# CaptainEven/DenseBox

Measured on AMD Instinct MI355X. Metric: training patches/sec (240x240), higher is better.
Workload: dtype f16; 1 GPU; full training step (fwd + fused dense loss w/ hard-negative mining + bwd + grad all-reduce + SGD) of DenseBoxLMLOC on 240x240 patches; net=DenseBoxLMLOC, batch_per_gpu=64, global_batch=64, patch=240x240, parallelism=dp1, half_neg=11, grad_finite=True

## Files before the change

densebox_amd/_lib.py:

```python
import ctypes as C
import os

_HERE = os.path.dirname(os.path.abspath(__file__))
LIB_PATH = os.environ.get('DBX_LIB') or os.path.join(_HERE, 'csrc', 'libdensebox_hip.so')

F16, BF16, F32 = 0, 1, 2
DTYPE_ID = {'f16': F16, 'bf16': BF16, 'f32': F32}
ESIZE = {F16: 2, BF16: 2, F32: 4}

EPI_BIAS, EPI_RELU, EPI_GATE, EPI_DROPMASK, EPI_ACCUM, EPI_F32_NCHW, EPI_DROPHASH = 1, 2, 4, 8, 16, 32, 64
CONV_WFRAG = 128
K_IGEMM, K_DMA, K_BAND, K_C64, K_C8, K_WS, K_P8 = 1, 2, 3, 4, 5, 6, 7


class View(C.Structure):
    _fields_ = [('ptr', C.c_void_p), ('n', C.c_int32), ('h', C.c_int32), ('w', C.c_int32),
                ('pad', C.c_int32), ('ld', C.c_int32), ('c_off', C.c_int32), ('c', C.c_int32)]


class ConvDesc(C.Structure):
    _fields_ = [('dtype', C.c_int32), ('kh', C.c_int32), ('kw', C.c_int32), ('cpad', C.c_int32),
                ('cin_pad', C.c_int32), ('cout_pad', C.c_int32), ('epilogue', C.c_int32), ('drop_seed', C.c_uint32)]


# ... 40 lines not shown


class CropFrame(C.Structure):
    _fields_ = [('src', C.c_void_p), ('sh', C.c_int32), ('sw', C.c_int32)]


class EvalRecord(C.Structure):
    _fields_ = [('score', C.c_double), ('lm_err', C.c_double), ('status', C.c_int32), ('frame', C.c_int32)]


class Track(C.Structure):
    _fields_ = [('box', C.c_double * 4), ('vel', C.c_double * 4), ('score', C.c_double), ('best_score', C.c_double), ('id', C.c_int32),
                ('hits', C.c_int32), ('age', C.c_int32), ('first_frame', C.c_int32), ('last_frame', C.c_int32), ('best_frame', C.c_int32)]


class TrackRecord(C.Structure):
    _fields_ = [('stream', C.c_int32), ('reserved', C.c_int32), ('t', Track)]


class Shot(C.Structure):
    _fields_ = [('key', C.c_double), ('score', C.c_double), ('sharpness', C.c_int64), ('id', C.c_int32), ('frame', C.c_int32),
                ('shots', C.c_int32), ('reserved', C.c_int32)]


class ShotRecord(C.Structure):
    _fields_ = [('stream', C.c_int32), ('slot', C.c_int32), ('shot', Shot)]


class OverlayFrame(C.Structure):
    _fields_ = [('src', C.c_void_p), ('dst', C.c_void_p), ('h', C.c_int32), ('w', C.c_int32)]


class OverlayStyle(C.Structure):
    _fields_ = [('box_color', C.c_uint8 * 4), ('text_color', C.c_uint8 * 4), ('mark_color', C.c_uint8 * 4), ('thickness', C.c_int32),
                ('radius', C.c_int32), ('font_scale', C.c_int32), ('inset_scale', C.c_int32)]


class RedactStyle(C.Structure):
    _fields_ = [('color', C.c_uint8 * 4), ('method', C.c_int32), ('shape', C.c_int32), ('cell', C.c_int32), ('radius', C.c_int32),
                ('grow', C.c_int32), ('grow_pct', C.c_int32), ('coast', C.c_int32), ('min_score', C.c_double)]


class ResizeJob(C.Structure):
    _fields_ = [('src', C.c_void_p), ('sh', C.c_int32), ('sw', C.c_int32), ('cx0', C.c_int32), ('cy0', C.c_int32),
                ('cw', C.c_int32), ('ch', C.c_int32), ('pad_l', C.c_int32), ('pad_t', C.c_int32), ('pad_r', C.c_int32),
                ('pad_b', C.c_int32), ('pad_value', C.c_int32), ('dh', C.c_int32), ('dw', C.c_int32), ('dst_off', C.c_int64)]


class Nv12Frame(C.Structure):
    _fields_ = [('y', C.c_void_p), ('uv', C.c_void_p), ('rgb', C.c_void_p), ('h', C.c_int32), ('w', C.c_int32), ('pitch_y', C.c_int32),
                ('pitch_uv', C.c_int32), ('pitch_rgb', C.c_int32), ('reserved', C.c_int32)]


class Nv12Params(C.Structure):
    _fields_ = [('standard', C.c_int32), ('range', C.c_int32), ('order', C.c_int32), ('reserved', C.c_int32)]


class ResizeJobNv12(C.Structure):
    _fields_ = [('y', C.c_void_p), ('uv', C.c_void_p), ('pitch_y', C.c_int32), ('pitch_uv', C.c_int32), ('sh', C.c_int32),
                ('sw', C.c_int32), ('cx0', C.c_int32), ('cy0', C.c_int32), ('cw', C.c_int32), ('ch', C.c_int32), ('pad_l', C.c_int32),
                ('pad_t', C.c_int32), ('pad_r', C.c_int32), ('pad_b', C.c_int32), ('pad_value', C.c_int32), ('dh', C.c_int32),
                ('dw', C.c_int32), ('dst_off', C.c_int64)]


class PatchJob(C.Structure):
    _fields_ = [('src', C.c_void_p), ('dst', C.c_void_p), ('scale_x', C.c_double), ('scale_y', C.c_double), ('row_bytes', C.c_int32),
                ('cx0', C.c_int32), ('cy0', C.c_int32), ('cw', C.c_int32), ('ch', C.c_int32), ('pad_l', C.c_int32), ('pad_t', C.c_int32),
                ('vw', C.c_int32), ('vh', C.c_int32), ('dh', C.c_int32), ('dw', C.c_int32), ('pad_value', C.c_int32),
                ('tiles_x', C.c_int32), ('frame', C.c_int32), ('kind', C.c_int32), ('reserved', C.c_int32)]


class PatchGeom(C.Structure):
    _fields_ = [('status', C.c_int32), ('x0', C.c_int32), ('y0', C.c_int32), ('x1', C.c_int32), ('y1', C.c_int32),
                ('labels', C.c_int32 * 12), ('reserved', C.c_int32)]


class PatchPlanIO(C.Structure):
    _fields_ = [(k, C.c_void_p) for k in (
        'frames', 'plates', 'plate0', 'cand', 'draws', 'state', 'jobs', 'labels', 'bbox', 'vertices', 'label', 'count', 'tally',
        'status', 'slot', 'cand_out', 'draws_out')]


class PatchAug(C.Structure):
    _fields_ = [('flags', C.c_int32), ('blur', C.c_int32), ('box_len', C.c_int32), ('sat', C.c_int32), ('contrast', C.c_int32),
                ('brightness', C.c_int32), ('curve', C.c_int32), ('noise_amp', C.c_int32), ('key_lo', C.c_int32), ('key_hi', C.c_int32),
                ('gain', C.c_int32 * 3), ('reserved', C.c_int32 * 3)]


class PatchAugCfg(C.Structure):
    _fields_ = [('p_flip', C.c_double), ('p_blur', C.c_double), ('p_curve', C.c_double), ('p_noise', C.c_double), ('kind_w', C.c_int32 * 3),
                ('box_lo', C.c_int32), ('box_hi', C.c_int32), ('sat_lo', C.c_int32), ('sat_hi', C.c_int32), ('contrast_lo', C.c_int32),
                ('contrast_hi', C.c_int32), ('brightness_lo', C.c_int32), ('brightness_hi', C.c_int32), ('gain_lo', C.c_int32),
                ('gain_hi', C.c_int32), ('noise_lo', C.c_int32), ('noise_hi', C.c_int32), ('curve_lo', C.c_int32), ('curve_hi', C.c_int32),
                ('G', C.c_int32), ('reserved', C.c_int32 * 2)]


class PatchAugIO(C.Structure):
    _fields_ = [(k, C.c_void_p) for k in ('labels_in', 'count', 'params_in', 'state', 'params', 'labels', 'bbox', 'vertices', 'label')]


class PatchWarpRec(C.Structure):
    _fields_ = [('flags', C.c_int32), ('border', C.c_int32), ('fill', C.c_int32), ('rot', C.c_int32), ('quad', C.c_int32 * 8),
                ('scale', C.c_int32), ('aspect', C.c_int32), ('shear', C.c_int32), ('reserved', C.c_int32)]


class PatchWarpCfg(C.Structure):
    _fields_ = [('p_warp', C.c_double), ('rot_lo', C.c_int32), ('rot_hi', C.c_int32), ('scale_lo', C.c_int32), ('scale_hi', C.c_int32),
                ('aspect_lo', C.c_int32), ('aspect_hi', C.c_int32), ('shear_lo', C.c_int32), ('shear_hi', C.c_int32), ('tx', C.c_int32),
                ('ty', C.c_int32), ('jitter', C.c_int32), ('margin', C.c_int32), ('border', C.c_int32), ('fill', C.c_int32), ('R', C.c_int32),
                ('reserved', C.c_int32)]


class PatchWarpIO(C.Structure):
    _fields_ = [(k, C.c_void_p) for k in ('labels_in', 'count', 'params_in', 'state', 'rot', 'params', 'labels', 'bbox', 'vertices', 'label',
                                          'fwd', 'inv')]


class MergeXform(C.Structure):
    _fields_ = [('scale', C.c_double), ('off_x', C.c_double), ('off_y', C.c_double)]


_VP, _I32, _I64, _F, _D = C.c_void_p, C.c_int32, C.c_int64, C.c_float, C.c_double
_PV, _PC = C.POINTER(View), C.POINTER(ConvDesc)

SIGNATURES = {
    'dbx_last_error': (C.c_char_p, []),
    'dbx_version': (C.c_int, []),
    'dbx_device_arch': (C.c_int, [C.c_int]),
    'dbx_conv_packed_elems': (_I64, [_PC]),
    'dbx_conv_forward': (C.c_int, [_PC, _PV, _VP, _VP, _PV, _PV, _VP, _I32, _VP]),
    'dbx_conv_plan': (C.c_int, [_PC, _PV, _PV, C.POINTER(ConvPlan)]),
    'dbx_conv_forward_split': (C.c_int, [_PC, _PV, _VP, _VP, _PV, _PV, _PV, _PV, _I32, _I32, _VP]),
    'dbx_heads_forward_fusable': (C.c_int, [_PC, _PV, _PV, C.POINTER(C.c_int32), _I32]),
    'dbx_heads_forward_fused_scratch_bytes': (_I64, [_I32, _I64]),
    'dbx_heads_forward_fused': (C.c_int, [_PC, _PV, _VP, _VP, _PV, _VP, _VP, C.POINTER(C.c_int32), _I32, _VP, _VP, _VP]),
    'dbx_heads_forward_fused_heads': (C.c_int, [_PC, _PV, _VP, _VP, _PV, _VP, _VP, C.POINTER(C.c_int32), _I32, C.POINTER(C.c_void_p), _VP, _VP]),
    'dbx_dp_unique_id': (C.c_int, [_VP]),
    'dbx_dp_init': (C.c_int, [_VP, _I32, _I32, C.POINTER(C.c_void_p)]),
    'dbx_dp_allreduce_sum_f32': (C.c_int, [_VP, _VP, _I64, _VP]),
    'dbx_dp_destroy': (C.c_int, [_VP]),
    'dbx_conv_dgrad_wgrad1_scratch_bytes': (_I64, []),
    'dbx_conv_dgrad_wgrad1_fusable': (C.c_int, [_PC, _PV, _PV, _PV]),
    'dbx_conv_dgrad_wgrad1': (C.c_int, [_PC, _PV, _VP, _PV, _PV, _I32, _VP, _VP, _VP, _I32, _VP]),
    'dbx_conv_pool_fusable': (C.c_int, [_PC, _PV, _PV]),
    'dbx_conv_forward_pool': (C.c_int, [_PC, _PV, _VP, _VP, _PV, _PV, _I32, _VP]),
    'dbx_conv_forward_pool_idx': (C.c_int, [_PC, _PV, _VP, _VP, _PV, _PV, _I32, _VP, _VP]),
    'dbx_pack_weight': (C.c_int, [_I32, _I32, _VP, _I32, _I32, _I32, _I32, _VP, _I32, _I32, _I32, _I32, _VP]),
    'dbx_fold_heads': (C.c_int, [_VP, _VP, _VP, _VP, _I32, _VP, _VP, _VP]),
    'dbx_fold_refine': (C.c_int, [_VP, _VP, _VP, _VP, _VP, _VP, _I32, _I32, _VP, _VP, _VP, _VP]),
    'dbx_refine_eval': (C.c_int, [_VP, _VP, _I32, _I32, _I32, _VP, _VP, _VP, _VP]),
    'dbx_refine_backward_scratch_bytes': (C.c_int64, [_I32, _I32, _I32]),
    'dbx_refine_backward': (C.c_int, [_VP, _VP, _VP, _I32, _I32, _I32, _VP, _VP, _VP, _VP, _VP, _VP, _I32, _VP, _VP, _VP, _VP, _VP, _VP, _VP, _VP, _VP, _VP, _VP, _VP, _VP, _VP]),
    'dbx_upsample_bilinear_nchw_f32': (C.c_int, [_VP, _I32, _I32, _I32, _VP, _I32, _I32, _VP]),
    'dbx_pack_multi': (C.c_int, [_I32, _VP, _I32, _I64, _VP]),
    'dbx_sgd_pack_step': (C.c_int, [_I32, _VP, _I32, _I64, _VP, _F, _F, _F, _I32, _VP]),
    'dbx_head2_dgrad': (C.c_int, [_I32, _PV, C.POINTER(C.c_void_p), C.POINTER(C.c_int32), _I32, _PV, _VP, _I32, _I32, C.c_uint32, _VP]),
    'dbx_head2_wgrad_scratch_bytes': (_I64, [_I32, _I32]),
    'dbx_head2_wgrad': (C.c_int, [_I32, _PV, _PV, C.POINTER(C.c_int32), _I32, C.POINTER(C.c_void_p), C.POINTER(C.c_void_p), _VP, _VP]),
    'dbx_head2_backward': (C.c_int, [_I32, _PV, _PV, C.POINTER(C.c_void_p), C.POINTER(C.c_int32), _I32, _PV, _VP, _I32, _I32, C.c_uint32,
                                     C.POINTER(C.c_void_p), C.POINTER(C.c_void_p), _VP, _VP]),
    'dbx_head2_backward_up': (C.c_int, [_I32, _PV, _PV, C.POINTER(C.c_void_p), C.POINTER(C.c_int32), _I32, _PV, _VP, _I32, _I32, C.c_uint32,
                                        C.POINTER(C.c_void_p), C.POINTER(C.c_void_p), _VP, _PV, _VP]),
    'dbx_perspective_matrix': (C.c_int, [_VP, _VP, _VP]),
    'dbx_warp_perspective_u8': (C.c_int, [_VP, _I32, _I32, _I32, _VP, _VP, _I32, _I32, _VP]),
    'dbx_warp_batch_workspace_bytes': (_I64, [_I32]),
    'dbx_warp_perspective_batch_u8': (C.c_int, [C.POINTER(WarpJob), _I32, _I32, _VP, _VP, _VP]),
    'dbx_plate_crops_batch': (C.c_int, [_VP, _I32, _I32, _VP, _I64, _I64, _VP, _I32, _I32, _I32, _VP, _VP, _VP, _VP]),
    'dbx_match_gt_batch': (C.c_int, [_VP, _I32, _I64, _VP, _VP, _I32, _I32, _VP, _I32, _VP, _VP, _I32, _D, _VP, _VP, _VP, _VP, _VP, _VP]),
    'dbx_eval_append': (C.c_int, [_VP, _I32, _I64, _VP, _VP, _I32, _I32, _VP, _VP, _VP, _VP, _I64, _VP, _VP]),
    'dbx_track_update_batch': (C.c_int, [_VP, _I32, _I64, _VP, _VP, _I32, _I32, _VP, _VP, _I32, _I32, _I32, _D, _I32, _D, _D, _D, _VP, _VP, _VP,
                                         _VP, _VP, _VP]),
    'dbx_track_append': (C.c_int, [_VP, _VP, _I32, _I32, _I32, _VP, _I64, _VP, _VP]),
    'dbx_crop_sharpness': (C.c_int, [_VP, _I64, _I32, _I32, _I32, _VP, _VP]),
    'dbx_track_gallery_update': (C.c_int, [_VP, _VP, _VP, _VP, _VP, _VP, _VP, _VP, _VP, _VP, _VP, _VP, _VP, _I32, _I32, _I32, _I32, _I32, _I32,
                                           _I32, _I32, _I64, _I32, _D, _I32, _VP]),
    'dbx_draw_overlay_batch': (C.c_int, [_VP, _I32, _I32, _I32, _I32, _VP, _I32, _I64, _VP, _VP, _I32, _VP, _VP, _VP, _I32, _I32,
                                         C.POINTER(OverlayStyle), _VP]),
    'dbx_overlay_font': (C.c_int, [_VP]),
    'dbx_overlay_label': (C.c_int, [_D, _I32, C.c_char_p, _I32]),
    'dbx_redact_batch': (C.c_int, [_VP, _I32, _I32, _I32, _I32, _VP, _I32, _I64, _VP, _VP, _I32, _VP, _I32, _I32, _I32,
                                   C.POINTER(RedactStyle), _VP]),
    'dbx_redact_host': (C.c_int, [_VP, _VP, _I32, _I32, _I32, _VP, _I32, _I32, _VP, _I32, _VP, _I32, C.POINTER(RedactStyle)]),
    'dbx_resize_batch_workspace_bytes': (_I64, [_I32]),
    'dbx_resize_cubic_batch_u8': (C.c_int, [C.POINTER(ResizeJob), _I32, _I32, _VP, _VP, _VP]),
    'dbx_nv12_to_rgb_batch': (C.c_int, [_VP, _I32, _I32, _I32, C.POINTER(Nv12Params), _VP]),
    'dbx_rgb_to_nv12_batch': (C.c_int, [_VP, _I32, _I32, _I32, C.POINTER(Nv12Params), _VP]),
    'dbx_nv12_host': (C.c_int, [C.POINTER(Nv12Frame), C.POINTER(Nv12Params), _I32]),
    'dbx_resize_batch_nv12_workspace_bytes': (_I64, [_I32]),
    'dbx_resize_cubic_batch_nv12': (C.c_int, [C.POINTER(ResizeJobNv12), _I32, C.POINTER(Nv12Params), _VP, _VP, _VP]),
    'dbx_patch_plan': (C.c_int, [C.POINTER(PatchPlanIO), _I32, _I32, _I32, _I32, _I32, _D, _D, _I32, _VP]),
    'dbx_patch_cut': (C.c_int, [_VP, _VP, _I32, _I32, _VP, _VP]),
    'dbx_patch_plan_host': (C.c_int, [_I32, _I32, _I32, _VP, _I32, _D, _D, _D, _I32, C.POINTER(PatchGeom)]),
    'dbx_patch_draw': (C.c_int, [_I64, _I64, _I32, _I32, _VP]),
    'dbx_patch_check_tables': (C.c_int, [_VP, _I32, _VP, _I32, _VP, _I32]),
    'dbx_patch_aug_plan': (C.c_int, [C.POINTER(PatchAugIO), C.POINTER(PatchAugCfg), _I32, _VP]),
    'dbx_patch_augment': (C.c_int, [_VP, _VP, _VP, _VP, _I32, _I32, _I32, _VP, _VP]),
    'dbx_patch_aug_params_host': (C.c_int, [C.POINTER(PatchAugCfg), _I64, _I64, _VP, _VP, _I32, _VP, _VP, _VP, _VP, _VP]),
    'dbx_patch_augment_host': (C.c_int, [_VP, _VP, _VP, _I32, _I32, _VP]),
    'dbx_patch_warp_plan': (C.c_int, [C.POINTER(PatchWarpIO), C.POINTER(PatchWarpCfg), _I32, _VP]),
    'dbx_patch_warp': (C.c_int, [_VP, _VP, _VP, _VP, _I32, _I32, _VP, _VP]),
    'dbx_patch_warp_params_host': (C.c_int, [C.POINTER(PatchWarpCfg), _I64, _I64, _VP, _VP, _VP, _I32, _VP, _VP, _VP, _VP, _VP, _VP, _VP]),
    'dbx_patch_warp_host': (C.c_int, [_VP, _VP, _VP, _I32, _VP]),
    'dbx_conv_wgrad_scratch_bytes': (_I64, [_I32, _PV, _PV, _I32, _I32]),
    'dbx_conv_wgrad': (C.c_int, [_I32, _PV, _PV, _I32, _I32, _I32, _I32, _I32, _VP, _VP, _VP, _I32, _VP]),
    'dbx_conv_wgrad_slice': (C.c_int, [_I32, _PV, _PV, _I32, _I32, _I32, _I32, _I32, _VP, _I32, _I32, _VP, _VP, _I32, _VP]),
    'dbx_conv_wgrad_pool_dz_ok': (C.c_int, [_I32, _PV, _PV, _I32, _I32]),
    'dbx_conv_wgrad_pool_dz': (C.c_int, [_I32, _PV, _VP, _I32, _PV, _PV, _I32, _I32, _I32, _I32, _I32, _VP, _VP, _VP, _I32, _I32, _VP]),
    'dbx_head2_backward_up_fused': (C.c_int, [_I32, _PV, _PV]),
    'dbx_head2_backward_up_plan': (C.c_int, [_I32, _PV, _PV, C.POINTER(C.c_int32), _I32, C.POINTER(Head2UpPlan)]),
    'dbx_heads1_wgrad_gen_ok': (C.c_int, [_I32, _PV, _I32]),
    'dbx_heads1_dgrad_gen': (C.c_int, [_I32, _PV, C.POINTER(C.c_void_p), C.POINTER(C.c_int32), _I32, _I32, C.c_uint32, _VP, _PV, _PV, _VP]),
    'dbx_heads1_wgrad_gen': (C.c_int, [_I32, _PV, _PV, C.POINTER(C.c_void_p), C.POINTER(C.c_int32), _I32, _I32, C.c_uint32, _I32, _VP, _I32, _I32,
                             _VP, _VP, _VP]),
    'dbx_conv_wgrad_plan': (C.c_int, [_I32, _PV, _PV, _I32, _I32, C.c_char_p, _I32, C.POINTER(C.c_int32)]),
    'dbx_nchw_to_framed': (C.c_int, [_I32, _VP, _I32, _PV, _VP]),
    'dbx_u8hwc_to_framed': (C.c_int, [_I32, _VP, _PV, C.POINTER(C.c_float), C.POINTER(C.c_float), _VP]),
    'dbx_nchw_to_framed_ch': (C.c_int, [_I32, _VP, _I32, _PV, _I32, _VP]),
    'dbx_nchw_to_framed_slots': (C.c_int, [_I32, _VP, _VP, _I32, _I32, _PV, _VP]),
    'dbx_framed_to_nchw_f32': (C.c_int, [_I32, _PV, _VP, _VP]),
    'dbx_framed_add_ch': (C.c_int, [_I32, _PV, _I32, _I32, _PV, _I32, _VP]),
    'dbx_maxpool2x2': (C.c_int, [_I32, _PV, _PV, _VP]),
    'dbx_maxpool2x2_bwd': (C.c_int, [_I32, _PV, _PV, _PV, _I32, _I32, _VP]),
    'dbx_maxpool_idx_bytes': (C.c_int64, [_I32, _I32, _I32, _I32]),
    'dbx_maxpool2x2_idx': (C.c_int, [_I32, _PV, _PV, _VP, _VP]),
    'dbx_maxpool2x2_bwd_idx': (C.c_int, [_I32, _VP, _PV, _PV, _I32, _I32, _VP]),
    'dbx_upsample_bilinear': (C.c_int, [_I32, _PV, _PV, _VP]),
    'dbx_upsample_bilinear_bwd': (C.c_int, [_I32, _PV, _PV, _PV, _VP]),
    'dbx_upsample_bilinear_bwd_plan': (C.c_int, [_I32, _PV, _PV, C.POINTER(UpsampleBwdPlan)]),
    'dbx_loss_scratch_bytes': (C.c_int64, [_I32]),
    'dbx_loss_forward_backward': (C.c_int, [C.POINTER(LossDesc), C.POINTER(LossIO), _VP, _VP]),
    'dbx_count_positives': (C.c_int, [_VP, _VP, _I32, _VP, _VP]),
    'dbx_init_score_map': (C.c_int, [_VP, _VP, _I32, _VP, _VP]),
    'dbx_init_offset_map': (C.c_int, [_VP, _VP, _I32, _I32, _VP, _VP]),
    'dbx_init_lm_heatmap': (C.c_int, [_VP, _VP, _I32, _I32, _VP, _VP]),
    'dbx_mask_by_sel': (C.c_int, [_VP, _I32, _VP, _I64, _VP, _I32, _VP]),
    'dbx_mask_gray_zone_cls': (C.c_int, [_VP, _VP, _VP, _I32, _VP]),
    'dbx_mask_gray_zone_lm': (C.c_int, [_VP, _I32, _VP, _I64, _VP]),
    'dbx_sgd_step': (C.c_int, [_VP, _VP, _I32, _I64, _F, _F, _F, _I32, _VP]),
    'dbx_grad_guard': (C.c_int, [_VP, _I64, _VP, _I32, _VP]),
    'dbx_sgd_step_guarded': (C.c_int, [_VP, _VP, _I32, _I64, _F, _F, _F, _I32, _VP, _I32, _VP]),
    'dbx_sgd_pack_step_guarded': (C.c_int, [_I32, _VP, _I32, _I64, _VP, _F, _F, _F, _I32, _VP, _I32, _VP]),
    'dbx_detect_scratch_bytes': (_I64, [_I32, _I32, _I32]),
    'dbx_detect': (C.c_int, [_VP, _VP, _VP, _VP, _I32, _I32, _I32, _D, _VP, _I32, _VP, _VP, _VP, _VP]),
    'dbx_detect_batch_scratch_bytes': (_I64, [_I32, _I32, _I32, _I32]),
    'dbx_detect_batch': (C.c_int, [_VP, _VP, _VP, _VP, _I32, _I32, _I32, _I32, _D, _VP, _I32, _VP, _VP, _VP, _VP]),
    'dbx_nms': (C.c_int, [_VP, _I32, _I32, _D, _VP, _VP, _VP]),
    'dbx_detect_thresh_batch_scratch_bytes': (_I64, [_I32, _I32, _I32, _I32]),
    'dbx_detect_thresh_batch': (C.c_int, [_VP, _VP, _VP, _VP, _I32, _I32, _I32, _F, _I32, _D, _VP, _I32, _VP, _VP, _VP, _VP, _VP]),
    'dbx_thresh_rows_batch_scratch_bytes': (_I64, [_I32, _I32, _I32, _I32]),
    'dbx_thresh_rows_batch': (C.c_int, [_VP, _VP, _VP, _VP, _I32, _I32, _I32, _F, _I32, _VP, _I32, _VP, _VP, _VP, _VP]),
    'dbx_nms_large_scratch_bytes': (_I64, [_I32]),
    'dbx_nms_large': (C.c_int, [_VP, _I32, _I32, _D, _VP, _VP, _VP]),
    'dbx_merge_nms_batch_workspace_bytes': (_I64, [_I32, _I32, _I32]),
    'dbx_merge_nms_batch': (C.c_int, [C.POINTER(C.c_void_p), C.POINTER(MergeXform), _I32, _I32, _I32, _I32, _D, _VP, _VP, _VP, _VP]),
    'dbx_merge_nms_thresh_batch_workspace_bytes': (_I64, [_I32, _I32, _I32]),
    'dbx_merge_nms_thresh_batch': (C.c_int, [C.POINTER(C.c_void_p), C.POINTER(C.c_void_p), C.POINTER(MergeXform), _I32, _I32, _I32, _I32, _D,
                                             _VP, _VP, _VP, _VP, _VP]),
}

ABI_VERSION = 13
_lib = None
MISSING = []


def lib():
    global _lib
    if _lib is None:
        if not os.path.exists(LIB_PATH):
            raise RuntimeError('libdensebox_hip.so is not built (%s). Run `python -c "import __graft_entry__ as g; '
                               'g.build()"`; densebox_amd has no fallback path.' % LIB_PATH)
        L = C.CDLL(LIB_PATH)
        for name, (res, args) in SIGNATURES.items():
            try:
                fn = getattr(L, name)
            except AttributeError:
                MISSING.append(name)
                continue
            fn.restype = res
            fn.argtypes = args
        if 'dbx_version' not in MISSING and L.dbx_version() != ABI_VERSION:
            raise RuntimeError('libdensebox_hip.so at %s has ABI version %d, this binding needs %d (struct layouts / scratch '
                               'contracts differ): rebuild it' % (LIB_PATH, L.dbx_version(), ABI_VERSION))
        _lib = L
    return _lib


def check(rc):
    if rc != 0:
        raise RuntimeError('libdensebox_hip: %s (status %d)' % (lib().dbx_last_error().decode(), rc))


def ptr(t):
    return C.c_void_p(t.data_ptr()) if t is not None else None


def stream_ptr():
    import torch
    return C.c_void_p(torch.cuda.current_stream().cuda_stream)
```

densebox_amd/csrc/aux_ops.hip:

```cpp
#include "common.hpp"
#include <mutex>

static thread_local char g_err[512] = "";
void dbx_set_error(const char* fmt, ...) {
    va_list ap;
    va_start(ap, fmt);
    vsnprintf(g_err, sizeof(g_err), fmt, ap);
    va_end(ap);
}
extern "C" const char* dbx_last_error(void) { return g_err; }
extern "C" int dbx_version(void) { return DBX_ABI_VERSION; }
extern "C" int dbx_device_arch(int device) {
    hipDeviceProp_t p;
    if (hipGetDeviceProperties(&p, device) != hipSuccess) { dbx_set_error("hipGetDeviceProperties failed"); return DBX_ERR_HIP; }
    int arch = 0;
    const char* s = p.gcnArchName;
    if (s[0] == 'g' && s[1] == 'f' && s[2] == 'x') arch = (int)strtol(s + 3, nullptr, 16) == 0x950 ? 950 : (int)strtol(s + 3, nullptr, 10);
    return arch;
}

template <typename T> struct Vec { static constexpr int N = 16 / sizeof(T); };

template <typename T> __device__ __forceinline__ void load_vec(const T* p, float (&v)[16 / sizeof(T)]) {
    const u32x4 raw = *(const u32x4*)p;
// ... 1671 lines not shown

__global__ void fold_heads_kernel(const float* __restrict__ w2, const float* __restrict__ b2, const float* __restrict__ w1,
                                  const float* __restrict__ b1, int k, float* __restrict__ w, float* __restrict__ b) {
    const int j = blockIdx.x;
    for (int c = threadIdx.x; c < 768; c += blockDim.x) {
        float acc = 0.f;
        for (int h = 0; h < 512; ++h) acc = fmaf(w2[j * 512 + h], w1[h * 768 + c], acc);
        w[j * 768 + c] = acc;
    }
    if (threadIdx.x == 0) {
        float acc = b2[j];
        for (int h = 0; h < 512; ++h) acc = fmaf(w2[j * 512 + h], b1[h], acc);
        b[j] = acc;
    }
}
extern "C" int dbx_fold_heads(const float* w2, const float* b2, const float* w1, const float* b1, int32_t k, float* w_out,
                              float* b_out, void* stream) {
    DBX_REQUIRE(w2 && b2 && w1 && b1 && w_out && b_out && k >= 1, "fold_heads: bad arguments");
    hipLaunchKernelGGL(fold_heads_kernel, dim3(k), dim3(256), 0, (hipStream_t)stream, w2, b2, w1, b1, k, w_out, b_out);
    DBX_LAUNCH_CHECK();
    return DBX_OK;
}

__global__ __launch_bounds__(256) void fold_refine_v_kernel(const float* __restrict__ w2, const float* __restrict__ w3, int cm, float* __restrict__ V) {
    const int e = blockIdx.x * 32 + (threadIdx.x >> 3), part = threadIdx.x & 7;
    float acc = 0.f;
    if (e < cm * 25) {
        const int m = e / 25, ab = e % 25;
        for (int n = part; n < cm; n += 8) acc = fmaf(w3[n], w2[((size_t)n * cm + m) * 25 + ab], acc);
    }
    acc += __shfl_xor(acc, 1); acc += __shfl_xor(acc, 2); acc += __shfl_xor(acc, 4);
    if (part == 0 && e < cm * 25) V[e] = acc;
}
__global__ __launch_bounds__(256) void fold_refine_w_kernel(const float* __restrict__ w1, const float* __restrict__ b1, const float* __restrict__ b2,
                                                            const float* __restrict__ w3, const float* __restrict__ b3, const float* __restrict__ Vg,
                                                            int ci, int cm, float* __restrict__ w, float* __restrict__ b) {
    __shared__ float V[64 * 25];
    __shared__ float w1s[64 * 9];
    __shared__ float red[5][49];
    __shared__ float bred[256];
    const int tid = threadIdx.x, c = blockIdx.x;
    for (int e = tid; e < cm * 25; e += 256) V[e] = Vg[e];
    for (int e = tid; e < cm * 9; e += 256) w1s[e] = w1[((size_t)(e / 9) * ci + c) * 9 + e % 9];
    __syncthreads();
    if (tid < 245) {
        const int uv = tid % 49, ch = tid / 49, u = uv / 7, v = uv % 7;
        const int per = (cm + 4) / 5, m0 = ch * per, m1 = m0 + per < cm ? m0 + per : cm;
        float acc = 0.f;
        for (int m = m0; m < m1; ++m)
            for (int i = 0; i < 3; ++i)
                for (int j = 0; j < 3; ++j) {
                    const int a2 = u - i, b2i = v - j;
                    if (a2 >= 0 && a2 < 5 && b2i >= 0 && b2i < 5) acc = fmaf(V[m * 25 + a2 * 5 + b2i], w1s[m * 9 + i * 3 + j], acc);
                }
        red[ch][uv] = acc;
    }
    __syncthreads();
    if (tid < 49) w[c * 49 + tid] = (((red[0][tid] + red[1][tid]) + red[2][tid]) + red[3][tid]) + red[4][tid];
    if (c == 0) {
        float part = 0.f;
        for (int m = tid; m < cm; m += 256) {
            float sv = 0.f;
            for (int ab = 0; ab < 25; ++ab) sv += V[m * 25 + ab];
            part += sv * b1[m] + w3[m] * b2[m];
        }
        bred[tid] = part;
        __syncthreads();
        if (tid == 0) {
            float acc = b3[0];
            for (int t = 0; t < 256; ++t) acc += bred[t];
            b[0] = acc;
        }
    }
}
extern "C" int dbx_fold_refine(const float* w1, const float* b1, const float* w2, const float* b2, const float* w3, const float* b3,
                               int32_t ci, int32_t cm, float* w_out, float* b_out, float* v_out, void* stream) {
    DBX_REQUIRE(w1 && b1 && w2 && b2 && w3 && b3 && w_out && b_out && v_out && ci >= 1 && cm >= 1 && cm <= 64, "fold_refine: bad arguments (mid channels <= 64)");
    hipLaunchKernelGGL(fold_refine_v_kernel, dim3((cm * 25 + 31) / 32), dim3(256), 0, (hipStream_t)stream, w2, w3, cm, v_out);
    DBX_LAUNCH_CHECK();
    hipLaunchKernelGGL(fold_refine_w_kernel, dim3(ci), dim3(256), 0, (hipStream_t)stream, w1, b1, b2, w3, b3, v_out, ci, cm, w_out, b_out);
    DBX_LAUNCH_CHECK();
    return DBX_OK;
}

__global__ __launch_bounds__(256) void refine_eval_kernel(const float* __restrict__ lm, const float* __restrict__ sc, int h, int w,
                                                          const float* __restrict__ wf, const float* __restrict__ bf, float* __restrict__ out) {
    constexpr int T = 16, PT = T + 6, CI = 5;
    __shared__ float tile[CI][PT][PT + 1];
    __shared__ float wsm[CI * 49];
    const int ph = h / 2, pw = w / 2, oh = ph - 6, ow = pw - 6;
    const int n = blockIdx.z, oy0 = blockIdx.y * T, ox0 = blockIdx.x * T;
    const int tid = threadIdx.x;
    for (int e = tid; e < CI * 49; e += 256) wsm[e] = wf[e];
    for (int e = tid; e < CI * PT * PT; e += 256) {
        const int c = e / (PT * PT), r = e % (PT * PT), py = oy0 + r / PT, px = ox0 + r % PT;
        float v = 0.f;
        if (py < ph && px < pw) {
            const float* p = (c < 4 ? lm + ((size_t)n * 4 + c) * h * w : sc + (size_t)n * h * w) + (size_t)(2 * py) * w + 2 * px;
            v = fmaxf(fmaxf(p[0], p[1]), fmaxf(p[w], p[w + 1]));
        }
        tile[c][r / PT][r % PT] = v;
    }
    __syncthreads();
    const int ty = tid / T, tx = tid % T, oy = oy0 + ty, ox = ox0 + tx;
    if (oy < oh && ox < ow) {
        float acc = bf[0];
        for (int c = 0; c < CI; ++c)
#pragma unroll
            for (int u = 0; u < 7; ++u)
#pragma unroll
                for (int v = 0; v < 7; ++v) acc = fmaf(wsm[(c * 7 + u) * 7 + v], tile[c][ty + u][tx + v], acc);
        out[((size_t)n * oh + oy) * ow + ox] = acc;
    }
}
extern "C" int dbx_refine_eval(const float* landmark_nchw, const float* score_nchw, int32_t n, int32_t h, int32_t w, const float* w_fold,
                               const float* b_fold, float* out_small, void* stream) {
    DBX_REQUIRE(landmark_nchw && score_nchw && w_fold && b_fold && out_small && n >= 1 && h / 2 >= 7 && w / 2 >= 7, "refine_eval: bad arguments (H/2, W/2 >= 7)");
    const int oh = h / 2 - 6, ow = w / 2 - 6;
    hipLaunchKernelGGL(refine_eval_kernel, dim3((ow + 15) / 16, (oh + 15) / 16, n), dim3(256), 0, (hipStream_t)stream, landmark_nchw, score_nchw, h, w,
                       w_fold, b_fold, out_small);
    DBX_LAUNCH_CHECK();
    return DBX_OK;
}

__global__ void upsample_nchw_f32_kernel(const float* __restrict__ x, int planes, int hi, int wi, float* __restrict__ y, int ho, int wo,
                                         float sy, float sx) {
    const int64_t total = (int64_t)planes * ho * wo;
    for (int64_t i = blockIdx.x * (int64_t)blockDim.x + threadIdx.x; i < total; i += (int64_t)gridDim.x * blockDim.x) {
        const int px = (int)(i % wo), py = (int)((i / wo) % ho);
        const int64_t pl = i / ((int64_t)wo * ho);
        int y0, y1, x0, x1;
        float ly0, ly1, lx0, lx1;
        bilin_coef(py, sy, hi, y0, y1, ly0, ly1);
        bilin_coef(px, sx, wi, x0, x1, lx0, lx1);
        const float* p = x + pl * hi * wi;
        {
#pragma clang fp contract(off)
            const float top = lx0 * p[y0 * wi + x0] + lx1 * p[y0 * wi + x1];
            const float bot = lx0 * p[y1 * wi + x0] + lx1 * p[y1 * wi + x1];
            y[i] = ly0 * top + ly1 * bot;
        }
    }
}
extern "C" int dbx_upsample_bilinear_nchw_f32(const float* x, int32_t planes, int32_t hi, int32_t wi, float* y, int32_t ho, int32_t wo,
                                              void* stream) {
    DBX_REQUIRE(x && y && planes >= 1 && hi >= 1 && wi >= 1 && ho >= 1 && wo >= 1, "upsample_nchw: bad arguments");
    const int64_t total = (int64_t)planes * ho * wo;
    hipLaunchKernelGGL(upsample_nchw_f32_kernel, dim3(grid_for(total)), dim3(256), 0, (hipStream_t)stream, x, planes, hi, wi, y, ho, wo,
                       ac_scale(hi, ho), ac_scale(wi, wo));
    DBX_LAUNCH_CHECK();
    return DBX_OK;
}

template <typename T>
__global__ void u8hwc_to_framed_kernel(const unsigned char* __restrict__ x, FrameGeo y, float m0, float m1, float m2, float s0,
                                       float s1, float s2) {
    constexpr int V = Vec<T>::N;
    const int cg = y.c / V;
    const int64_t total = (int64_t)y.n * y.h * y.w;
    for (int64_t i = blockIdx.x * (int64_t)blockDim.x + threadIdx.x; i < total; i += (int64_t)gridDim.x * blockDim.x) {
        const int px = (int)(i % y.w);
        const int py = (int)((i / y.w) % y.h);
        const int n = (int)(i / ((int64_t)y.w * y.h));
        const unsigned char* p = x + i * 3;
        float v[3];
        v[0] = ((float)p[0] / 255.0f - m0) / s0;
        v[1] = ((float)p[1] / 255.0f - m1) / s1;
        v[2] = ((float)p[2] / 255.0f - m2) / s2;
        T* dst = (T*)y.base + geo_pix(y, n, py, px);
        for (int g = 0; g < cg; ++g) {
            float o[V];
#pragma unroll
            for (int j = 0; j < V; ++j) { const int c = g * V + j; o[j] = c < 3 ? v[c] : 0.f; }
            store_vec<T>(dst + g * V, o);
        }
    }
}
template <typename T> static int u8hwc_to_framed_t(const uint8_t* x, const dbx_view* y, const float* mean, const float* stdv, hipStream_t s) {
    VIEW_VEC_CHECK(T, y, "u8hwc_to_framed");
    DBX_REQUIRE(y->c >= 3 && mean && stdv, "u8hwc_to_framed: need >= 3 channels and mean/std");
    const int64_t total = (int64_t)y->n * y->h * y->w;
    hipLaunchKernelGGL(u8hwc_to_framed_kernel<T>, dim3(grid_for(total)), dim3(256), 0, s, x, make_geo<T>(y), mean[0], mean[1], mean[2],
                       stdv[0], stdv[1], stdv[2]);
    DBX_LAUNCH_CHECK();
    return DBX_OK;
}
extern "C" int dbx_u8hwc_to_framed(int32_t dtype, const uint8_t* x_nhwc, const dbx_view* y, const float* mean3, const float* std3,
                                   void* stream) {
    DBX_DISPATCH_DTYPE(dtype, u8hwc_to_framed_t, x_nhwc, y, mean3, std3, (hipStream_t)stream);
}
```

densebox_amd/csrc/common.hpp:

```cpp
#pragma once
#include <hip/hip_runtime.h>
#include <stdint.h>
#include <stdio.h>
#include <stdarg.h>
#include <atomic>

#include "../../include/densebox_hip.h"

typedef float f32x4 __attribute__((ext_vector_type(4)));
typedef _Float16 f16x8 __attribute__((ext_vector_type(8)));
typedef _Float16 f16x4 __attribute__((ext_vector_type(4)));
typedef __bf16 bf16x8 __attribute__((ext_vector_type(8)));
typedef __bf16 bf16x4 __attribute__((ext_vector_type(4)));
typedef unsigned int u32x4 __attribute__((ext_vector_type(4)));
typedef unsigned int u32x2 __attribute__((ext_vector_type(2)));

void dbx_set_error(const char* fmt, ...);

#define DBX_HIP(call)                                                                         \
    do {                                                                                      \
        hipError_t e_ = (call);                                                               \
        if (e_ != hipSuccess) {                                                               \
            dbx_set_error("%s failed: %s (%s:%d)", #call, hipGetErrorString(e_), __FILE__, __LINE__); \
            return DBX_ERR_HIP;                                                               \
        }                                                                                     \
    } while (0)

#define DBX_LAUNCH_CHECK()                                                                    \
    do {                                                                                      \
        hipError_t e_ = hipGetLastError();                                                    \
        if (e_ != hipSuccess) {                                                               \
            dbx_set_error("kernel launch failed: %s (%s:%d)", hipGetErrorString(e_), __FILE__, __LINE__); \
            return DBX_ERR_HIP;                                                               \
        }                                                                                     \
    } while (0)

#define DBX_REQUIRE(cond, ...)                                                                \
    do {                                                                                      \
        if (!(cond)) {                                                                        \
            dbx_set_error(__VA_ARGS__);                                                       \
            return DBX_ERR_ARG;                                                               \
        }                                                                                     \
    } while (0)

struct DbxDevOnce {
    std::atomic<uint64_t> done{0};
    bool pending(int* dev_out) {
        int dev = 0;
        if (hipGetDevice(&dev) != hipSuccess) dev = 0;
        *dev_out = dev;
        return !((done.load(std::memory_order_acquire) >> (dev & 63)) & 1ull);
    }
    void mark(int dev) { done.fetch_or(1ull << (dev & 63), std::memory_order_release); }
};

namespace pipe { template <int N> struct IC { static constexpr int value = N; }; }

static inline int dbx_esize(int dtype) { return dtype == DBX_F32 ? 4 : 2; }

template <typename T> struct DType;
template <> struct DType<_Float16> { static constexpr int id = DBX_F16; };
template <> struct DType<__bf16> { static constexpr int id = DBX_BF16; };
template <> struct DType<float> { static constexpr int id = DBX_F32; };

template <typename T> __device__ __forceinline__ float to_f32(T v) { return (float)v; }
template <typename T> __device__ __forceinline__ T from_f32(float v) { return (T)v; }

struct FrameGeo {
    char* base;
    int n, h, w, pad;
    int hp, wp;
    int ld;
    int c;
};

template <typename T>
static inline FrameGeo make_geo(const dbx_view* v) {
    FrameGeo g;
    g.base = (char*)v->ptr + (size_t)v->c_off * sizeof(T);
    g.n = v->n; g.h = v->h; g.w = v->w; g.pad = v->pad;
    g.hp = v->h + 2 * v->pad; g.wp = v->w + 2 * v->pad;
    g.ld = v->ld; g.c = v->c;
    return g;
}

__device__ __forceinline__ size_t geo_pix(const FrameGeo& g, int n, int y, int x) {
    return ((size_t)(n * g.hp + y + g.pad) * g.wp + (x + g.pad)) * (size_t)g.ld;
}

__device__ __forceinline__ unsigned dbx_drop_hash32(unsigned seed, unsigned m, unsigned c32) {
    unsigned x = seed ^ (m * 0x9E3779B1u) ^ (c32 * 0x85EBCA77u);
    x ^= x >> 16; x *= 0x7FEB352Du; x ^= x >> 15; x *= 0x846CA68Bu; x ^= x >> 16;
    return x;
}
__device__ __forceinline__ unsigned dbx_drop_bits4(unsigned seed, unsigned m, unsigned c4) {
    return (dbx_drop_hash32(seed, m, c4 >> 3) >> ((c4 & 7u) * 4u)) & 15u;
}

typedef float f32x16 __attribute__((ext_vector_type(16)));

template <typename T> struct Mma32;
template <> struct Mma32<_Float16> {
    static __device__ __forceinline__ void run(const u32x4& a, const u32x4& b, f32x16& c) {
        c = __builtin_amdgcn_mfma_f32_32x32x16_f16(__builtin_bit_cast(f16x8, a), __builtin_bit_cast(f16x8, b), c, 0, 0, 0);
    }
};
template <> struct Mma32<__bf16> {
    static __device__ __forceinline__ void run(const u32x4& a, const u32x4& b, f32x16& c) {
        c = __builtin_amdgcn_mfma_f32_32x32x16_bf16(__builtin_bit_cast(bf16x8, a), __builtin_bit_cast(bf16x8, b), c, 0, 0, 0);
    }
};

struct GenHid {
    const char* dout;
    const float* w2[4];
    int k[4];
    int ld, slot, nh;
    int H, W, pad;
    unsigned seed; int use_hash;
};
template <typename T>
__device__ __forceinline__ u32x4 genhid_wfrag(const GenHid& gh, int hd, int ch, int lane) {
    const float* wp = gh.w2[0];
    int k = gh.k[0];
#pragma unroll
    for (int hh = 1; hh < 4; ++hh)
        if (hd == hh && gh.w2[hh]) { wp = gh.w2[hh]; k = gh.k[hh]; }
    const float sc = gh.use_hash ? 2.f : 1.f;
    u32x4 raw;
    T* e = (T*)&raw;
#pragma unroll
    for (int j = 0; j < 8; ++j) {
        const int row = j < k ? j : (k > 0 ? k - 1 : 0);
        const float v = wp[(size_t)row * 512 + ch];
        e[j] = from_f32<T>((lane < 32 && j < k) ? v * sc : 0.f);
    }
    return raw;
}
__device__ __forceinline__ int genhid_pixel(const GenHid& gh, int img, int q_in_img, int wp, float inv_wp) {
    const int fy = (int)(((float)q_in_img + 0.5f) * inv_wp);
    const int fx = q_in_img - fy * wp;
    const int y = fy - gh.pad, x = fx - gh.pad;
    return ((unsigned)y < (unsigned)gh.H && (unsigned)x < (unsigned)gh.W) ? (img * gh.H + y) * gh.W + x : -1;
}
__device__ __forceinline__ u32x4 genhid_load_dout(const GenHid& gh, int hd, int m) {
    const int mm = m < 0 ? 0 : m;
    return *(const u32x4*)(gh.dout + ((size_t)mm * gh.ld + hd * gh.slot) * 2);
}
__device__ __forceinline__ u32x4 genhid_bfrag(const u32x4& raw, int m, int lane) {
    return (m < 0 || lane >= 32) ? (u32x4){0u, 0u, 0u, 0u} : raw;
}

__host__ __device__ inline size_t dbx_frag_index(int row, int tap, int k, int cin_pad, int rows_pad, int taps) {
    const int bn = rows_pad % 256 == 0 ? 256 : 128;
    int period, step, nstep, nper;
    if (taps == 9) {
        const int KC = cin_pad / 64, ky = tap / 3, kx = tap - 3 * ky;
        period = 3 * (k / 64) + ky; step = kx * 4 + (k % 64) / 16; nstep = 12; nper = 3 * KC;
    } else {
        period = k / 128; step = (k % 128) / 16; nstep = 8; nper = cin_pad / 128;
    }
    const int lane = 32 * ((k % 16) / 8) + row % 32;
    const size_t blk = (((size_t)(row / bn) * nper + period) * nstep + step) * (bn / 32) + (row % bn) / 32;
    return (blk * 64 + lane) * 8 + k % 8;
}

__device__ __forceinline__ float dbx_sgd_update(float pv, float gr, float* buf, float lr, float mu, float wd, int first) {
#pragma clang fp contract(off)
    const float gv = gr + wd * pv;
    const float bv = first ? gv : mu * *buf + gv;
    *buf = bv;
    return pv - lr * bv;
}

#define DBX_DISPATCH_DTYPE(dtype, FN, ...)                          \
    switch (dtype) {                                                \
        case DBX_F16: return FN<_Float16>(__VA_ARGS__);             \
        case DBX_BF16: return FN<__bf16>(__VA_ARGS__);              \
        case DBX_F32: return FN<float>(__VA_ARGS__);                \
        default: dbx_set_error("bad dtype %d", (int)(dtype)); return DBX_ERR_DTYPE; \
    }
```

densebox_amd/csrc/loss.hip:

```cpp
#include "common.hpp"

#define HWD 60
#define NPIX 3600
#define LOSS_THREADS 1024

__device__ __forceinline__ int norm_idx(int v) {
    if (v < 0) { v += HWD; if (v < 0) v = 0; }
    else if (v > HWD) v = HWD;
    return v;
}
struct Span { int a, b; };
__device__ __forceinline__ Span py_slice(int start, int stop) {
    Span s; s.a = norm_idx(start); s.b = norm_idx(stop); if (s.b < s.a) s.b = s.a; return s;
}
__device__ __forceinline__ void rect_axis(float c0, float c2, double border, int& org, int& end) {
    const double centre = (double)(c0 + c2) * 0.5;
    const float w = c2 - c0;
    const float rw = 0.3f * w;
    const float half = rw * 0.5f;
    if (border == 0.0) {
        org = (int)(centre - (double)half + 0.5);
        end = (int)((double)org + (double)rw + 0.5);
    } else {
        org = (int)(centre - (double)half - border + 0.5);
        end = (int)((double)org + (double)rw + border * 2.0 + 0.5);
    }
}
struct Box { Span py, px, gzy, gzx, coy, cox; int valid; };
__device__ __forceinline__ Box make_box(const float* bb, int valid) {
    Box b; b.valid = valid;
    int ox, ex, oy, ey;
    rect_axis(bb[0], bb[2], 0.0, ox, ex); rect_axis(bb[1], bb[3], 0.0, oy, ey);
    b.px = py_slice(ox, ex + 1); b.py = py_slice(oy, ey + 1);
    rect_axis(bb[0], bb[2], 2.0, ox, ex); rect_axis(bb[1], bb[3], 2.0, oy, ey);
    b.gzx = py_slice(ox, ex); b.gzy = py_slice(oy, ey);
    b.cox = py_slice(ox + 2, ex - 2 + 1); b.coy = py_slice(oy + 2, ey - 2 + 1);
    return b;
}
__device__ __forceinline__ bool in_span(const Span& s, int v) { return v >= s.a && v < s.b; }
__device__ __forceinline__ int lm_coord(float v, int clamp) {
    int x = (int)(v + 0.5f);
    if (clamp) x = x < HWD ? x : HWD - 1;
    return x;
}
__device__ __forceinline__ int lm_pixel(int x, int y) {
    return (x >= 0 && x < HWD && y >= 0 && y < HWD) ? y * HWD + x : -1;
}

__device__ __forceinline__ int block_argmax(const float* vals, float* red_v, int* red_i) {
    const int tid = threadIdx.x;
    float bv = -2.f; int bi = 0x7fffffff;
    for (int i = tid; i < NPIX; i += LOSS_THREADS) {
        const float v = vals[i];
        if (v > bv) { bv = v; bi = i; }
    }
#pragma unroll
    for (int off = 32; off > 0; off >>= 1) {
        const float ov = __shfl_down(bv, off); const int oi = __shfl_down(bi, off);
        if (ov > bv || (ov == bv && oi < bi)) { bv = ov; bi = oi; }
    }
    if ((tid & 63) == 0) { red_v[tid >> 6] = bv; red_i[tid >> 6] = bi; }
    __syncthreads();
    if (tid == 0) {
        for (int w = 1; w < LOSS_THREADS / 64; ++w)
            if (red_v[w] > bv || (red_v[w] == bv && red_i[w] < bi)) { bv = red_v[w]; bi = red_i[w]; }
        red_i[0] = bi;
    }
    __syncthreads();
    const int r = red_i[0];
    __syncthreads();
    return r;
}

__device__ __forceinline__ double block_sum(double v, double* red) {
#pragma unroll
    for (int off = 32; off > 0; off >>= 1) v += __shfl_down(v, off);
    if ((threadIdx.x & 63) == 0) red[threadIdx.x >> 6] = v;
    __syncthreads();
    double t = 0.0;
    if (threadIdx.x == 0) for (int w = 0; w < LOSS_THREADS / 64; ++w) t += red[w];
    __syncthreads();
    return t;
}

struct LossArgs { dbx_loss_desc d; dbx_loss_io io; double* partial; unsigned char* maskbuf; };
#define LOSS_APPLY_THREADS 256
#define LOSS_APPLY_BLOCKS ((NPIX + LOSS_APPLY_THREADS - 1) / LOSS_APPLY_THREADS)

__global__ __launch_bounds__(LOSS_THREADS) void loss_kernel(const LossArgs a) {
    __shared__ float negl[NPIX];
    __shared__ unsigned char mask[NPIX];
    __shared__ unsigned char lmask[4][NPIX];
    __shared__ float red_v[LOSS_THREADS / 64];
    __shared__ int red_i[LOSS_THREADS / 64];
    __shared__ double red_d[LOSS_THREADS / 64];
    const int n = blockIdx.x, tid = threadIdx.x;
    const int kind = a.d.kind, N = a.d.n, K = a.d.half_neg;
    const dbx_loss_io& io = a.io;
    const float* bb = io.bbox + 4 * n;
    const int valid = (a.d.use_labels && io.labels) ? (io.labels[n] != 0.f) : 1;
    const Box box = make_box(bb, valid);

    const float* score = io.score + (size_t)n * NPIX;
    int npos = 0;
    for (int i = tid; i < NPIX; i += LOSS_THREADS) {
        const int y = i / HWD, x = i - y * HWD;
        const float gt = (valid && in_span(box.py, y) && in_span(box.px, x)) ? 1.f : 0.f;
        const float d = score[i] - gt;
        negl[i] = d * d * (1.f - gt);
        mask[i] = gt != 0.f;
        npos += gt != 0.f;
    }
    __syncthreads();
    if (io.pos_count) {
        const double t = block_sum((double)npos, red_d);
        if (tid == 0) io.pos_count[n] = (int)t;
    }
    if (K > 0 && K <= 48) {
        __shared__ unsigned long long wcand[(LOSS_THREADS / 64) * 48];
        const int lane = tid & 63, wv = tid >> 6;
        unsigned long long comp[4];
#pragma unroll
        for (int e = 0; e < 4; ++e) {
            const int i = tid + e * LOSS_THREADS;
            const float v = i < NPIX ? negl[i] : 0.f;
            const unsigned key = v != v ? 0u : __float_as_uint(v);
            comp[e] = i < NPIX ? ((unsigned long long)key << 32) | (unsigned)(~(unsigned)i) : 0ull;
        }
        auto wave_max = [&](unsigned long long v) {
#pragma unroll
            for (int off = 32; off > 0; off >>= 1) { const unsigned long long o = __shfl_xor(v, off); v = o > v ? o : v; }
            return v;
        };
        for (int r = 0; r < K; ++r) {
            unsigned long long best = comp[0];
#pragma unroll
            for (int e = 1; e < 4; ++e) best = comp[e] > best ? comp[e] : best;
            best = wave_max(best);
#pragma unroll
            for (int e = 0; e < 4; ++e) comp[e] = comp[e] == best ? 0ull : comp[e];
            if (lane == 0) wcand[wv * 48 + r] = best;
        }
        __syncthreads();
        if (wv == 0) {
            const int tot = (LOSS_THREADS / 64) * K;
            unsigned long long c2[12];
#pragma unroll
            for (int j = 0; j < 12; ++j) {
                const int f = lane + 64 * j;
                c2[j] = f < tot ? wcand[(f / K) * 48 + f % K] : 0ull;
            }
            for (int r = 0; r < K; ++r) {
                unsigned long long best = c2[0];
#pragma unroll
                for (int j = 1; j < 12; ++j) best = c2[j] > best ? c2[j] : best;
                best = wave_max(best);
#pragma unroll
                for (int j = 0; j < 12; ++j) c2[j] = c2[j] == best ? 0ull : c2[j];
                if (lane == 0) {
                    const int idx = (int)(~(unsigned)(best & 0xffffffffull));
                    mask[idx] = 1;
                    if (io.neg_idx) io.neg_idx[(size_t)n * 2 * K + r] = idx;
                }
            }
        }
        __syncthreads();
    } else {
        for (int k = 0; k < K; ++k) {
            const int idx = block_argmax(negl, red_v, red_i);
            if (tid == 0) {
                negl[idx] = -1.f;
                mask[idx] = 1;
                if (io.neg_idx) io.neg_idx[(size_t)n * 2 * K + k] = idx;
            }
            __syncthreads();
        }
    }
    for (int k = tid; k < K; k += LOSS_THREADS) {
        const long long r = io.rand_neg[(size_t)n * K + k];
        if (io.neg_idx) io.neg_idx[(size_t)n * 2 * K + K + k] = r;
        if (r >= 0 && r < NPIX) mask[(int)r] = 1;
    }
    __syncthreads();
    if (valid) {
        for (int i = tid; i < NPIX; i += LOSS_THREADS) {
            const int y = i / HWD, x = i - y * HWD;
            if (in_span(box.gzy, y) && in_span(box.gzx, x)) mask[i] = 0;
        }
        __syncthreads();
        for (int i = tid; i < NPIX; i += LOSS_THREADS) {
            const int y = i / HWD, x = i - y * HWD;
            if (in_span(box.coy, y) && in_span(box.cox, x)) mask[i] = 1;
        }
        __syncthreads();
    }

    int lmx[4] = {0, 0, 0, 0}, lmy[4] = {0, 0, 0, 0};
    if (kind != 0) {
        const float* vt = io.vertices + 8 * n;
        const int clamp = a.d.use_labels;
        for (int j = 0; j < 4; ++j) { lmx[j] = lm_coord(vt[2 * j], clamp); lmy[j] = lm_coord(vt[2 * j + 1], clamp); }
        for (int j = 0; j < 4; ++j) {
            const float* lm = io.lm + ((size_t)n * 4 + j) * NPIX;
            const int pidx = lm_pixel(lmx[j], lmy[j]);
            for (int i = tid; i < NPIX; i += LOSS_THREADS) {
                const float gt = (valid && i == pidx) ? 1.f : 0.f;
                const float d = lm[i] - gt;
                negl[i] = d * d * (1.f - gt);
                lmask[j][i] = gt != 0.f;
            }
            __syncthreads();
            const int hard = block_argmax(negl, red_v, red_i);
            if (tid == 0) {
                const long long r = io.lm_rand_neg[((size_t)j * N + n)];
                lmask[j][hard] = 1;
                if (r >= 0 && r < NPIX) lmask[j][(int)r] = 1;
                if (io.lm_neg_idx) { io.lm_neg_idx[((size_t)j * N + n) * 2] = hard; io.lm_neg_idx[((size_t)j * N + n) * 2 + 1] = r; }
            }
            __syncthreads();
            if (valid && pidx >= 0) {
                const Span sy = py_slice(lmy[j] - 2, lmy[j] + 3), sx = py_slice(lmx[j] - 2, lmx[j] + 3);
                for (int i = tid; i < 25; i += LOSS_THREADS) {
                    const int y = sy.a + i / 5, x = sx.a + i % 5;
                    if (y < sy.b && x < sx.b) lmask[j][y * HWD + x] = 0;
                }
                __syncthreads();
                if (tid == 0) lmask[j][pidx] = 1;
                __syncthreads();
            }
        }
    }

    unsigned char* mb = a.maskbuf + (size_t)n * 5 * NPIX;
    for (int i = tid; i < NPIX; i += LOSS_THREADS) {
        mb[i] = mask[i];
        if (kind != 0) {
#pragma unroll
            for (int j = 0; j < 4; ++j) mb[(1 + j) * NPIX + i] = lmask[j][i];
        }
    }
}

__global__ __launch_bounds__(LOSS_APPLY_THREADS) void loss_apply_kernel(const LossArgs a) {
    __shared__ double red_d[LOSS_APPLY_THREADS / 64];
    const int n = blockIdx.y, tid = threadIdx.x, i = blockIdx.x * LOSS_APPLY_THREADS + tid;
    const int kind = a.d.kind;
    const dbx_loss_io& io = a.io;
    const float* bb = io.bbox + 4 * n;
    const int valid = (a.d.use_labels && io.labels) ? (io.labels[n] != 0.f) : 1;
    const Box box = make_box(bb, valid);
    const float* score = io.score + (size_t)n * NPIX;
    const unsigned char* mb = a.maskbuf + (size_t)n * 5 * NPIX;
    int lmp[4] = {-1, -1, -1, -1};
    if (kind != 0) {
        const float* vt = io.vertices + 8 * n;
        const int clamp = a.d.use_labels;
        for (int j = 0; j < 4; ++j) lmp[j] = lm_pixel(lm_coord(vt[2 * j], clamp), lm_coord(vt[2 * j + 1], clamp));
    }
    const float l_loc = a.d.lambda_loc, l_det = (kind == 0) ? 1.f : a.d.lambda_det, l_lm = a.d.lambda_lm;
    double s_cls = 0, s_loc = 0, s_lm = 0, s_lmloc = 0, s_rf = 0;
    if (i < NPIX) {
        const int y = i / HWD, x = i - y * HWD;
        const float m = (float)mb[i];
        const float gt = (valid && in_span(box.py, y) && in_span(box.px, x)) ? 1.f : 0.f;
        if (io.mask_cls) io.mask_cls[(size_t)n * NPIX + i] = m;
        {
            const float d = score[i] - gt;
            s_cls += (double)(m * (d * d));
            if (io.d_score) io.d_score[(size_t)n * NPIX + i] = 2.f * l_det * m * d;
        }
        const float mg = m * gt;
        const float fx = (float)x, fy = (float)y;
#pragma unroll
        for (int c = 0; c < 4; ++c) {
            const float tgt = valid ? ((c & 1) ? fy : fx) - bb[c] : 0.f;
            const size_t o = ((size_t)n * 4 + c) * NPIX + i;
            const float d = io.loc[o] - tgt;
            s_loc += (double)(mg * (d * d));
            if (io.d_loc) io.d_loc[o] = 2.f * l_det * l_loc * mg * d;
        }
        if (kind != 0) {
            const float d = io.rf[(size_t)n * NPIX + i] - gt;
            s_rf += (double)(m * (d * d));
            if (io.d_rf) io.d_rf[(size_t)n * NPIX + i] = 2.f * m * d;
#pragma unroll
            for (int j = 0; j < 4; ++j) {
                const float ml = (float)mb[(1 + j) * NPIX + i];
                const float hg = (valid && i == lmp[j]) ? 1.f : 0.f;
                const size_t o = ((size_t)n * 4 + j) * NPIX + i;
                const float dl = io.lm[o] - hg;
                s_lm += (double)(ml * (dl * dl));
                if (io.d_lm) io.d_lm[o] = 2.f * l_lm * ml * dl;
                if (io.mask_lm) io.mask_lm[o] = ml;
            }
            if (kind == 2) {
                const float* vt = io.vertices + 8 * n;
#pragma unroll
                for (int c = 0; c < 8; ++c) {
                    const float tgt = valid ? ((c & 1) ? fy : fx) - vt[c] : 0.f;
                    const size_t o = ((size_t)n * 8 + c) * NPIX + i;
                    const float d = io.lmloc[o] - tgt;
                    s_lmloc += (double)(mg * (d * d));
                    if (io.d_lmloc) io.d_lmloc[o] = 2.f * mg * d;
                }
            }
        }
    }
    double mine = (double)l_det * (s_cls + (double)l_loc * s_loc) + (double)l_lm * s_lm + s_lmloc + s_rf;
#pragma unroll
    for (int off = 32; off > 0; off >>= 1) mine += __shfl_down(mine, off);
    if ((tid & 63) == 0) red_d[tid >> 6] = mine;
    __syncthreads();
    if (tid == 0) {
        double t = 0.0;
        for (int w = 0; w < LOSS_APPLY_THREADS / 64; ++w) t += red_d[w];
        a.partial[(size_t)n * LOSS_APPLY_BLOCKS + blockIdx.x] = t;
    }
}

__global__ __launch_bounds__(256) void loss_finish_kernel(const double* partial, int n, int per, float* loss) {
    __shared__ double psum[256];
    double run = 0.0;
    for (int base = 0; base < n; base += 256) {
        const int p = base + threadIdx.x;
        double t = 0.0;
        if (p < n) for (int i = 0; i < per; ++i) t += partial[(size_t)p * per + i];
        psum[threadIdx.x] = t;
        __syncthreads();
        if (threadIdx.x == 0) {
            const int cnt = n - base < 256 ? n - base : 256;
            for (int i = 0; i < cnt; ++i) run += psum[i];
        }
        __syncthreads();
    }
    if (threadIdx.x == 0) loss[0] = (float)run;
}

extern "C" int64_t dbx_loss_scratch_bytes(int32_t n) {
    return (int64_t)n * LOSS_APPLY_BLOCKS * 8 + (int64_t)n * 5 * NPIX + 64;
}
extern "C" int dbx_loss_forward_backward(const dbx_loss_desc* d, const dbx_loss_io* io, void* scratch, void* stream) {
    DBX_REQUIRE(d && io && scratch, "loss: null argument");
    DBX_REQUIRE(d->kind >= 0 && d->kind <= 2 && d->n > 0, "loss: bad kind/n");
    DBX_REQUIRE(d->half_neg >= 0 && d->half_neg <= NPIX, "loss: half_neg out of range");
    DBX_REQUIRE(io->bbox && io->score && io->loc && io->loss && (d->half_neg == 0 || io->rand_neg), "loss: missing tensors");
    if (d->kind != 0) DBX_REQUIRE(io->vertices && io->lm && io->rf && io->lm_rand_neg, "loss: landmark tensors missing");
    if (d->kind == 2) DBX_REQUIRE(io->lmloc != nullptr, "loss: lm_loc missing");
    LossArgs a; a.d = *d; a.io = *io; a.partial = (double*)scratch;
    a.maskbuf = (unsigned char*)scratch + (size_t)d->n * LOSS_APPLY_BLOCKS * sizeof(double);
    hipLaunchKernelGGL(loss_kernel, dim3(d->n), dim3(LOSS_THREADS), 0, (hipStream_t)stream, a);
    DBX_LAUNCH_CHECK();
    hipLaunchKernelGGL(loss_apply_kernel, dim3(LOSS_APPLY_BLOCKS, d->n), dim3(LOSS_APPLY_THREADS), 0, (hipStream_t)stream, a);
    DBX_LAUNCH_CHECK();
    hipLaunchKernelGGL(loss_finish_kernel, dim3(1), dim3(256), 0, (hipStream_t)stream, (const double*)scratch, d->n, LOSS_APPLY_BLOCKS, io->loss);
    DBX_LAUNCH_CHECK();
    return DBX_OK;
}

__global__ void count_positives_kernel(const float* bbox, const float* labels, int n, int* out) {
    const int i = blockIdx.x * blockDim.x + threadIdx.x;
    if (i >= n) return;
    const int valid = labels ? labels[i] != 0.f : 1;
    const Box b = make_box(bbox + 4 * i, valid);
    out[i] = valid ? (b.py.b - b.py.a) * (b.px.b - b.px.a) : 0;
}
extern "C" int dbx_count_positives(const float* bbox, const float* labels, int32_t n, int32_t* out, void* stream) {
    hipLaunchKernelGGL(count_positives_kernel, dim3((n + 63) / 64), dim3(64), 0, (hipStream_t)stream, bbox, labels, n, out);
    DBX_LAUNCH_CHECK();
    return DBX_OK;
}

__global__ void init_score_map_kernel(const float* bbox, const float* labels, float* out) {
    const int n = blockIdx.x;
    const int valid = labels ? labels[n] != 0.f : 1;
    const Box b = make_box(bbox + 4 * n, valid);
    for (int i = threadIdx.x; i < NPIX; i += blockDim.x) {
        const int y = i / HWD, x = i - y * HWD;
        out[(size_t)n * NPIX + i] = (valid && in_span(b.py, y) && in_span(b.px, x)) ? 1.f : 0.f;
    }
}
extern "C" int dbx_init_score_map(const float* bbox, const float* labels, int32_t n, float* out, void* stream) {
    hipLaunchKernelGGL(init_score_map_kernel, dim3(n), dim3(256), 0, (hipStream_t)stream, bbox, labels, out);
    DBX_LAUNCH_CHECK();
    return DBX_OK;
}

__global__ void init_offset_map_kernel(const float* coords, const float* labels, int c, float* out) {
    const int n = blockIdx.x;
    const int valid = labels ? labels[n] != 0.f : 1;
    for (int i = threadIdx.x; i < c * NPIX; i += blockDim.x) {
        const int ch = i / NPIX, p = i - ch * NPIX;
        const int y = p / HWD, x = p - y * HWD;
        out[(size_t)n * c * NPIX + i] = valid ? ((ch & 1) ? (float)y : (float)x) - coords[n * c + ch] : 0.f;
    }
}
extern "C" int dbx_init_offset_map(const float* coords, const float* labels, int32_t n, int32_t c, float* out, void* stream) {
    hipLaunchKernelGGL(init_offset_map_kernel, dim3(n), dim3(256), 0, (hipStream_t)stream, coords, labels, c, out);
    DBX_LAUNCH_CHECK();
    return DBX_OK;
}

__global__ void init_lm_heatmap_kernel(const float* vert, const float* labels, int clamp, float* out, int* err) {
    const int n = blockIdx.x;
    const int valid = labels ? labels[n] != 0.f : 1;
    for (int i = threadIdx.x; i < 4 * NPIX; i += blockDim.x) out[(size_t)n * 4 * NPIX + i] = 0.f;
    __syncthreads();
    if (threadIdx.x < 4 && valid) {
        const int j = threadIdx.x;
        int x = lm_coord(vert[8 * n + 2 * j], clamp), y = lm_coord(vert[8 * n + 2 * j + 1], clamp);
        if (x >= HWD || y >= HWD) { if (err) atomicAdd(err, 1); x = min(x, HWD - 1); y = min(y, HWD - 1); }
        if (x >= 0 && y >= 0) out[((size_t)n * 4 + j) * NPIX + y * HWD + x] = 1.f;
    }
}
extern "C" int dbx_init_lm_heatmap(const float* vertices, const float* labels, int32_t n, int32_t clamp, float* out, void* stream) {
    hipLaunchKernelGGL(init_lm_heatmap_kernel, dim3(n), dim3(256), 0, (hipStream_t)stream, vertices, labels, clamp, out, (int*)nullptr);
    DBX_LAUNCH_CHECK();
    return DBX_OK;
}

__global__ void mask_by_sel_kernel(float* mask, int n, const long long* pos, long long npos, const long long* neg, int nneg) {
    const long long total = npos + (long long)n * nneg;
    for (long long i = blockIdx.x * (long long)blockDim.x + threadIdx.x; i < total; i += (long long)gridDim.x * blockDim.x) {
        if (i < npos) {
            const long long* p = pos + 4 * i;
            mask[((size_t)p[0] + p[1]) * NPIX + p[2] * HWD + p[3]] = 1.f;
        } else {
            const long long j = i - npos;
            const long long id = neg[j];
            if (id >= 0 && id < NPIX) mask[(size_t)(j / nneg) * NPIX + id] = 1.f;
        }
    }
}
extern "C" int dbx_mask_by_sel(float* mask, int32_t n, const int64_t* pos_idx, int64_t n_pos, const int64_t* neg_idx,
                               int32_t n_neg, void* stream) {
    const long long total = n_pos + (long long)n * n_neg;
    if (total == 0) return DBX_OK;
    hipLaunchKernelGGL(mask_by_sel_kernel, dim3((unsigned)((total + 255) / 256)), dim3(256), 0, (hipStream_t)stream, mask, n,
                       (const long long*)pos_idx, (long long)n_pos, (const long long*)neg_idx, n_neg);
    DBX_LAUNCH_CHECK();
    return DBX_OK;
}

__global__ void mask_gray_zone_cls_kernel(float* mask, const float* bbox, const float* labels) {
    const int n = blockIdx.x;
    const int valid = labels ? labels[n] != 0.f : 1;
    if (!valid) return;
    const Box b = make_box(bbox + 4 * n, valid);
    for (int i = threadIdx.x; i < NPIX; i += blockDim.x) {
        const int y = i / HWD, x = i - y * HWD;
        float v = mask[(size_t)n * NPIX + i];
        if (in_span(b.gzy, y) && in_span(b.gzx, x)) v = 0.f;
        if (in_span(b.coy, y) && in_span(b.cox, x)) v = 1.f;
        mask[(size_t)n * NPIX + i] = v;
    }
}
extern "C" int dbx_mask_gray_zone_cls(float* mask, const float* bbox, const float* labels, int32_t n, void* stream) {
    hipLaunchKernelGGL(mask_gray_zone_cls_kernel, dim3(n), dim3(256), 0, (hipStream_t)stream, mask, bbox, labels);
    DBX_LAUNCH_CHECK();
    return DBX_OK;
}

__global__ void mask_gray_zone_lm_kernel(float* mask, const long long* pos, long long npos) {
    const long long p = blockIdx.x;
    if (p >= npos) return;
    const long long n = pos[4 * p];
    const int y = (int)pos[4 * p + 2], x = (int)pos[4 * p + 3];
    const Span sy = py_slice(y - 2, y + 3), sx = py_slice(x - 2, x + 3);
    const int i = threadIdx.x;
    if (i < 25) {
        const int yy = sy.a + i / 5, xx = sx.a + i % 5;
        if (yy < sy.b && xx < sx.b) mask[(size_t)n * NPIX + yy * HWD + xx] = 0.f;
    }
    __syncthreads();
    if (i == 0) mask[(size_t)n * NPIX + y * HWD + x] = 1.f;
}
extern "C" int dbx_mask_gray_zone_lm(float* mask, int32_t n, const int64_t* pos_idx, int64_t n_pos, void* stream) {
    if (n_pos == 0) return DBX_OK;
    hipLaunchKernelGGL(mask_gray_zone_lm_kernel, dim3((unsigned)n_pos), dim3(64), 0, (hipStream_t)stream, mask,
                       (const long long*)pos_idx, (long long)n_pos);
    DBX_LAUNCH_CHECK();
    return DBX_OK;
}
```

densebox_amd/csrc/refine_ops.hip:

```cpp
#include "common.hpp"

namespace {
constexpr int RCI = 5, RTAPS = 49, RG1 = RCI * RTAPS + 1;

__device__ __forceinline__ void rf_coef(int d, float scale, int in, int& i0, int& i1, float& l0, float& l1) {
#pragma clang fp contract(off)
    const float src = scale * (float)d;
    i0 = (int)src;
    if (i0 > in - 1) i0 = in - 1;
    i1 = i0 + (i0 < in - 1 ? 1 : 0);
    l1 = src - (float)i0;
    l0 = 1.f - l1;
}
inline float rf_scale(int in, int out) { return out > 1 ? (float)(in - 1) / (float)(out - 1) : 0.f; }

__global__ void refine_up_t_kernel(const float* __restrict__ d, int n, int ho, int wo, float* __restrict__ g, int hs, int ws, float sy, float sx) {
    const int64_t total = (int64_t)n * hs * ws;
    for (int64_t i = blockIdx.x * (int64_t)blockDim.x + threadIdx.x; i < total; i += (int64_t)gridDim.x * blockDim.x) {
        const int px = (int)(i % ws), py = (int)((i / ws) % hs);
        const int64_t im = i / ((int64_t)ws * hs);
        int ylo = sy > 0.f ? (int)((float)(py - 1) / sy) - 1 : 0, yhi = sy > 0.f ? (int)((float)(py + 1) / sy) + 2 : ho - 1;
        int xlo = sx > 0.f ? (int)((float)(px - 1) / sx) - 1 : 0, xhi = sx > 0.f ? (int)((float)(px + 1) / sx) + 2 : wo - 1;
        ylo = ylo < 0 ? 0 : ylo; xlo = xlo < 0 ? 0 : xlo; yhi = yhi > ho - 1 ? ho - 1 : yhi; xhi = xhi > wo - 1 ? wo - 1 : xhi;
        const float* dp = d + im * ho * wo;
        float acc = 0.f;
        for (int y = ylo; y <= yhi; ++y) {
            int y0, y1; float ly0, ly1;
            rf_coef(y, sy, hs, y0, y1, ly0, ly1);
            const float wy = (y0 == py ? ly0 : 0.f) + (y1 == py ? ly1 : 0.f);
            if (wy == 0.f) continue;
            for (int x = xlo; x <= xhi; ++x) {
                int x0, x1; float lx0, lx1;
                rf_coef(x, sx, ws, x0, x1, lx0, lx1);
                const float wx = (x0 == px ? lx0 : 0.f) + (x1 == px ? lx1 : 0.f);
                if (wx != 0.f) acc = fmaf(wy * wx, dp[y * wo + x], acc);
            }
        }
        g[i] = acc;
    }
}

constexpr int RSPLIT = 4;
__global__ __launch_bounds__(256) void refine_g1_kernel(const float* __restrict__ lm, const float* __restrict__ sc, int h, int w,
                                                        const float* __restrict__ g, float* __restrict__ partial) {
    extern __shared__ float sm[];
    const int ph = h / 2, pw = w / 2, oh = ph - 6, ow = pw - 6;
    const int n = blockIdx.x / RSPLIT, part = blockIdx.x % RSPLIT, tid = threadIdx.x;
    const int rows = (oh + RSPLIT - 1) / RSPLIT, y0 = part * rows < oh ? part * rows : oh, y1 = y0 + rows < oh ? y0 + rows : oh;
    const int xr = y1 > y0 ? y1 - y0 + 6 : 0;
    float* x5 = sm;
    float* gs = sm + RCI * (rows + 6) * pw;
    for (int e = tid; e < RCI * xr * pw; e += 256) {
        const int c = e / (xr * pw), r = e % (xr * pw), py = y0 + r / pw, px = r % pw;
        const float* p = (c < 4 ? lm + ((size_t)n * 4 + c) * h * w : sc + (size_t)n * h * w) + (size_t)(2 * py) * w + 2 * px;
        x5[e] = fmaxf(fmaxf(p[0], p[1]), fmaxf(p[w], p[w + 1]));
    }
    for (int e = tid; e < (y1 - y0) * ow; e += 256) gs[e] = g[((size_t)n * oh + y0) * ow + e];
    __syncthreads();
    if (tid < RG1) {
        float acc = 0.f;
        if (tid < RCI * RTAPS) {
            const int c = tid / RTAPS, u = (tid % RTAPS) / 7, v = tid % 7;
            const float* xc = x5 + (c * xr + u) * pw + v;
            for (int y = 0; y < y1 - y0; ++y)
                for (int x = 0; x < ow; ++x) acc = fmaf(gs[y * ow + x], xc[y * pw + x], acc);
        } else {
            for (int e = 0; e < (y1 - y0) * ow; ++e) acc += gs[e];
        }
        partial[(size_t)blockIdx.x * RG1 + tid] = acc;
    }
}

struct RefineW { const float *w1, *b1, *w2, *b2, *w3, *b3, *V; float *dw1, *db1, *dw2, *db2, *dw3, *db3; };
__global__ __launch_bounds__(256) void refine_wgrad_kernel(const float* __restrict__ partial, int nimg, int cm, RefineW a) {
    __shared__ float G1[RG1], G2[64 * 25], V[64 * 25], w1s[64 * RCI * 9], red[256];
    const int tid = threadIdx.x;
    for (int e = tid; e < cm * RCI * 9; e += 256) w1s[e] = a.w1[e];
    if (tid < RG1) {
        float acc = 0.f;
#pragma unroll 16
        for (int n = 0; n < nimg; ++n) acc += partial[(size_t)n * RG1 + tid];
        G1[tid] = acc;
    }
    const int blk = blockIdx.x;
    if (blk == cm)
        for (int e = tid; e < cm * 25; e += 256) V[e] = a.V[e];
    __syncthreads();
    const float Sg = G1[RG1 - 1];
    for (int e = tid; e < cm * 25; e += 256) {
        const int m = e / 25, aa = (e % 25) / 5, bb = e % 5;
        float acc = a.b1[m] * Sg;
        for (int c = 0; c < RCI; ++c)
            for (int i = 0; i < 3; ++i)
                for (int j = 0; j < 3; ++j) acc = fmaf(w1s[(m * RCI + c) * 9 + i * 3 + j], G1[(c * 7 + aa + i) * 7 + bb + j], acc);
        G2[e] = acc;
    }
    __syncthreads();
    if (blk < cm) {
        const int n = blk;
        const float w3n = a.w3[n];
        float part = 0.f;
        for (int e = tid; e < cm * 25; e += 256) {
            a.dw2[(size_t)n * cm * 25 + e] = w3n * G2[e];
            part = fmaf(a.w2[(size_t)n * cm * 25 + e], G2[e], part);
        }
        red[tid] = part;
        __syncthreads();
        if (tid == 0) {
            float acc = a.b2[n] * Sg;
            for (int t = 0; t < 256; ++t) acc += red[t];
            a.dw3[n] = acc;
            a.db2[n] = w3n * Sg;
        }
    } else {
        for (int e = tid; e < cm * RCI * 9; e += 256) {
            const int m = e / (RCI * 9), c = (e / 9) % RCI, i = (e % 9) / 3, j = e % 3;
            float acc = 0.f;
            for (int aa = 0; aa < 5; ++aa)
                for (int bb = 0; bb < 5; ++bb) acc = fmaf(V[m * 25 + aa * 5 + bb], G1[(c * 7 + aa + i) * 7 + bb + j], acc);
            a.dw1[e] = acc;
        }
        for (int m = tid; m < cm; m += 256) {
            float sv = 0.f;
            for (int ab = 0; ab < 25; ++ab) sv += V[m * 25 + ab];
            a.db1[m] = sv * Sg;
        }
        if (tid == 0) a.db3[0] = Sg;
    }
}

__global__ void refine_dgrad_kernel(const float* __restrict__ lm, const float* __restrict__ sc, int n, int h, int w, const float* __restrict__ g,
                                    const float* __restrict__ wf, const float* __restrict__ g_lm, const float* __restrict__ g_sc,
                                    float* __restrict__ out_lm, float* __restrict__ out_sc) {
    __shared__ float wsm[RCI * RTAPS];
    for (int e = threadIdx.x; e < RCI * RTAPS; e += blockDim.x) wsm[e] = wf[e];
    __syncthreads();
    const int ph = h / 2, pw = w / 2, oh = ph - 6, ow = pw - 6, wh = (h + 1) / 2, ww = (w + 1) / 2;
    const int64_t total = (int64_t)n * RCI * wh * ww;
    for (int64_t i = blockIdx.x * (int64_t)blockDim.x + threadIdx.x; i < total; i += (int64_t)gridDim.x * blockDim.x) {
        const int wx = (int)(i % ww), wy = (int)((i / ww) % wh), c = (int)((i / ((int64_t)ww * wh)) % RCI);
        const int im = (int)(i / ((int64_t)ww * wh * RCI));
        const size_t plane = c < 4 ? ((size_t)im * 4 + c) * h * w : (size_t)im * h * w;
        const float* xin = (c < 4 ? lm : sc) + plane;
        const float* gin = c < 4 ? (g_lm ? g_lm + plane : nullptr) : (g_sc ? g_sc + plane : nullptr);
        float* dst = (c < 4 ? out_lm : out_sc) + plane;
        float dv = 0.f;
        int arg = -1;
        if (wy < ph && wx < pw) {
            const float* gp = g + (size_t)im * oh * ow;
            for (int u = 0; u < 7; ++u) {
                const int y = wy - u;
                if (y < 0 || y >= oh) continue;
                for (int v = 0; v < 7; ++v) {
                    const int x = wx - v;
                    if (x >= 0 && x < ow) dv = fmaf(wsm[(c * 7 + u) * 7 + v], gp[y * ow + x], dv);
                }
            }
            const float* p = xin + (size_t)(2 * wy) * w + 2 * wx;
            float m = p[0]; arg = 0;
            if (p[1] > m) { m = p[1]; arg = 1; }
            if (p[w] > m) { m = p[w]; arg = 2; }
            if (p[w + 1] > m) { m = p[w + 1]; arg = 3; }
        }
#pragma unroll
        for (int k = 0; k < 4; ++k) {
            const int y = 2 * wy + (k >> 1), x = 2 * wx + (k & 1);
            if (y >= h || x >= w) continue;
            const float in = gin ? gin[(size_t)y * w + x] : 0.f;
            dst[(size_t)y * w + x] = in + (k == arg ? dv : 0.f);
        }
    }
}
}

extern "C" int64_t dbx_refine_backward_scratch_bytes(int32_t n, int32_t h, int32_t w) {
    const int64_t oh = h / 2 - 6, ow = w / 2 - 6;
    return ((int64_t)n * oh * ow + (int64_t)n * RSPLIT * RG1 + 64) * 4;
}

extern "C" int dbx_refine_backward(const float* d_refine, const float* landmark, const float* score, int32_t n, int32_t h, int32_t w,
                                   const float* w1, const float* b1, const float* w2, const float* b2, const float* w3, const float* b3,
                                   int32_t cm, const float* w_fold, const float* v_fold, const float* g_landmark, const float* g_score, float* out_landmark,
                                   float* out_score, float* dw1, float* db1, float* dw2, float* db2, float* dw3, float* db3, void* scratch,
                                   void* stream) {
    DBX_REQUIRE(d_refine && landmark && score && w1 && b1 && w2 && b2 && w3 && b3 && w_fold && v_fold && out_landmark && out_score && dw1 && db1 && dw2 &&
                    db2 && dw3 && db3 && scratch, "refine_backward: null argument");
    DBX_REQUIRE(n >= 1 && h / 2 >= 7 && w / 2 >= 7 && cm >= 1 && cm <= 64, "refine_backward: H/2, W/2 >= 7, mid channels <= 64");
    const int ph = h / 2, pw = w / 2, oh = ph - 6, ow = pw - 6;
    const int rows = (oh + RSPLIT - 1) / RSPLIT;
    const size_t lds = ((size_t)RCI * (rows + 6) * pw + (size_t)rows * ow) * 4;
    DBX_REQUIRE(lds <= 150 * 1024, "refine_backward: map too large for the per-image LDS tile (%d x %d)", h, w);
    hipStream_t s = (hipStream_t)stream;
    float* g = (float*)scratch;
    float* partial = g + (size_t)n * oh * ow;
    const int64_t tot_g = (int64_t)n * oh * ow;
    hipLaunchKernelGGL(refine_up_t_kernel, dim3((unsigned)((tot_g + 255) / 256)), dim3(256), 0, s, d_refine, n, h, w, g, oh, ow, rf_scale(oh, h), rf_scale(ow, w));
    DBX_LAUNCH_CHECK();
    static DbxDevOnce attr_once; int attr_dev = 0;
    if (attr_once.pending(&attr_dev)) {
        DBX_HIP(hipFuncSetAttribute((const void*)refine_g1_kernel, hipFuncAttributeMaxDynamicSharedMemorySize, 150 * 1024));
        attr_once.mark(attr_dev);
    }
    hipLaunchKernelGGL(refine_g1_kernel, dim3(n * RSPLIT), dim3(256), lds, s, landmark, score, h, w, g, partial);
    DBX_LAUNCH_CHECK();
    RefineW a = {w1, b1, w2, b2, w3, b3, v_fold, dw1, db1, dw2, db2, dw3, db3};
    hipLaunchKernelGGL(refine_wgrad_kernel, dim3(cm + 1), dim3(256), 0, s, partial, n * RSPLIT, cm, a);
    DBX_LAUNCH_CHECK();
    const int64_t tot_d = (int64_t)n * RCI * ((h + 1) / 2) * ((w + 1) / 2);
    hipLaunchKernelGGL(refine_dgrad_kernel, dim3((unsigned)((tot_d + 255) / 256)), dim3(256), 0, s, landmark, score, n, h, w, g, w_fold, g_landmark, g_score,
                       out_landmark, out_score);
    DBX_LAUNCH_CHECK();
    return DBX_OK;
}
```

densebox_amd/engine.py:

```python
import collections
import contextlib
import ctypes as C
import os
import weakref

import torch

from . import _lib
from ._lib import View, ConvDesc, check, ptr, stream_ptr

_BACKBONE = [('conv1_1_1', 3, 64), ('conv1_2_1', 64, 64), ('conv2_1_1', 64, 128), ('conv2_2_1', 128, 128),
             ('conv3_1_1', 128, 256), ('conv3_2_1', 256, 256), ('conv3_4_1', 256, 256),
             ('conv4_1_1', 256, 512), ('conv4_2_1', 512, 512), ('conv4_3_1', 512, 512), ('conv4_4_1', 512, 512)]

_HEADS = {
    'DenseBox': [('det', 1), ('loc', 4)],
    'DenseBoxLM': [('det', 1), ('loc', 4), ('landmark', 4)],
    'DenseBoxLMLOC': [('det', 1), ('loc', 4), ('landmark', 4), ('lmloc', 8)],
}


_FWD_IO = {'conv1_1_1': ('x0', 'a11'), 'conv1_2_1': ('a11', 'a12'), 'conv2_1_1': ('p1', 'a21'), 'conv2_2_1': ('a21', 'a22'),
           'conv3_1_1': ('p2', 'a31'), 'conv3_2_1': ('a31', 'a32'), 'conv3_4_1': ('a32', 'c34'), 'conv4_1_1': ('p3', 'a41'),
           'conv4_2_1': ('a41', 'a42'), 'conv4_3_1': ('a42', 'a43'), 'conv4_4_1': ('a43', 'a44')}
# ... 308 lines not shown
            import numpy as np
            self.wcache.clear(); self.bias_cache.clear()
            dev, es, jobs = params[0].device, _lib.ESIZE[dt], []
            for im in lay:
                out = self._buffer(im, dev)
                ps = [self._param(nm) for nm in im.srcs]
                (self.bias_cache if im.mode == 2 else self.wcache)[im.key] = (tuple((p._version, p.data_ptr()) for p in ps), out)
                ktot = (im.kh * im.kw * im.cin_pad * es + 127) // 128 * 128 // es
                for p, (row_off, k_off) in zip(ps, im.place):
                    if im.mode == 2:
                        jobs.append(PackJob(p.data_ptr(), out.data_ptr(), p.numel(), 1, 1, 2, 0, 0, row_off, 0, 0))
                    else:
                        jobs.append(PackJob(p.data_ptr(), out.data_ptr(), p.shape[0], p.shape[1], im.kh * im.kw, im.mode,
                                            im.rows_pad if im.mode >= 4 else ktot, im.cin_pad, row_off, k_off, im.rows_pad))
            self._table_keys = {im.key for im in lay}
            rec = np.zeros(len(jobs), dtype=[(f, '<u8' if f in ('src', 'dst') else '<i8' if f == 'ktot' else '<i4') for f in PackJob._fields])
            assert rec.dtype.itemsize == 56
            for i, j in enumerate(jobs):
                rec[i] = tuple(j)
            tab = (torch.from_numpy(rec.view(np.uint8).copy()).to(dev), len(jobs), max(j.co * j.ci * j.taps for j in jobs), jobs)
            self._tables = {tkey: tab}
            self._sgd_tables = {}
        check(self.L.dbx_pack_multi(dt, ptr(tab[0]), tab[1], tab[2], stream_ptr()))
        self._wsig = sig
        if train:
            self._last_prep = (dt, tkey, lay)
            register_params(self, params)

    def conv_plan(self, dt, x, y, kh, kw, cpad, cin_pad, cout_pad, epi):
        key = (dt, x.n, x.h, x.w, x.pad, x.ld, x.c_off, x.c, y.pad, y.ld, y.c_off, y.c, kh, kw, cpad, cin_pad, cout_pad,
               epi & ~_lib.CONV_WFRAG)
        ent = self._plans_conv.get(key)
        if ent is None:
            d = ConvDesc(dt, kh, kw, cpad, cin_pad, cout_pad, epi & ~_lib.CONV_WFRAG, 0)
            out = _lib.ConvPlan()
            check(self.L.dbx_conv_plan(C.byref(d), C.byref(x), C.byref(y), C.byref(out)))
            ent = (out.kernel, out.name.decode(), bool(out.w_frag))
            self._plans_conv[key] = ent
        return ent

    def _heads_fused(self, P, dt):
        heads = _HEADS[self.kind]
        nh = len(heads)
        if not P.train or dt == _lib.F32 or os.environ.get('DBX_HEADS_FUSED', '1') == '0':
            return 0
        d = ConvDesc(dt, 1, 1, 0, 768, 512 * nh, _lib.EPI_BIAS | _lib.EPI_DROPHASH, 0)
        ks = (C.c_int32 * nh)(*[k for _, k in heads])
        return int(self.L.dbx_heads_forward_fusable(C.byref(d), C.byref(P.B['fusion'].view()), C.byref(P.B['hid'].view()), ks, nh))

    def _frag_heads(self, P, dt, which):
        B, nh = P.B, len(_HEADS[self.kind])
        if which == 'f':
            return self.conv_plan(dt, B['fusion'].view(), B['hid'].view(), 1, 1, 0, 768, 512 * nh, _lib.EPI_BIAS | _lib.EPI_DROPHASH)[2]
        if dt == _lib.F32:
            return False
        if which == 'ba':
            return 'd_g44' in B and self.conv_plan(dt, B['d_g44'].view(), B['d_a44'].view(), 1, 1, 0, 512 * nh, 512, _lib.EPI_GATE)[2]
        if which == 'bc':
            if P.heads_gen:
                return True
            return 'd_hid' in B and self.conv_plan(dt, B['d_hid'].view(), B['d_c34'].view(), 1, 1, 0, 512 * nh, 256, _lib.EPI_GATE)[2]
        if 'd_hid' not in B or 'd_ups' not in B:
            return False
        dv = B['d_ups'].view()
        both = View(dv.ptr, dv.n, dv.h, dv.w, dv.pad, 768, 0, 768)
        return self.conv_plan(dt, B['d_hid'].view(), both, 1, 1, 0, 512 * nh, 768, 0)[2]

    def sgd_pack_step(self, live, ptrs, lr, momentum, weight_decay, first, guard=None, step_id=0):
        prep = getattr(self, '_last_prep', None)
        if prep is None or self._wsig is None or os.environ.get('DBX_SGD_PACK', '1') == '0':
            return False
        dt, tkey, lay = prep
        tab = self._tables.get(tkey)
        params = [p for _, p in self.net.named_parameters()]
        if tab is None or self._wsig[0] != dt or not self._wsig[1] or self._wsig[3] != lay:
            return False
        if tuple((p._version, p.data_ptr()) for p in params) != self._wsig[2]:
            return False
        mine = {id(p) for p in params}
        if any(id(p) not in mine for p in live):
            return False
        pidx = {p.data_ptr(): i for i, p in enumerate(live)}
        skey = (tkey, tuple(pidx))
        st = self._sgd_tables.get(skey)
        if st is False:
            return False
        if st is None:
            import numpy as np
            by_src = {}
            for j in tab[3]:
                by_src.setdefault(j.src, []).append(j)
            es = _lib.ESIZE[dt]
            recs = []
            for src, js in by_src.items():
                if src not in pidx:
                    continue
                j0 = js[0]
                if len(js) > 4 or any((j.co, j.ci, j.taps) != (j0.co, j0.ci, j0.taps) for j in js):
                    self._sgd_tables[skey] = False
                    return False
                tiled = es == 2 and j0.taps <= 25 and all(
                    j.mode != 2 and (j.ci if j.mode in (0, 4) else j.co) % 8 == 0 and j.k_off % 8 == 0 and j.cin_pad % 8 == 0 for j in js)
                recs.append((src, pidx[src], j0.co, j0.ci, j0.taps, len(js), int(tiled), js))
            for p in live:
                if p.data_ptr() not in by_src:
                    recs.append((p.data_ptr(), pidx[p.data_ptr()], p.numel(), 1, 1, 0, 0, []))
            dst_t = [('dst', '<u8'), ('ktot', '<i8'), ('mode', '<i4'), ('cin_pad', '<i4'), ('row_off', '<i4'), ('k_off', '<i4'),
                     ('rows_lim', '<i4'), ('pad', '<i4')]
            rec = np.zeros(len(recs), dtype=[('p', '<u8'), ('pidx', '<i4'), ('co', '<i4'), ('ci', '<i4'), ('taps', '<i4'), ('ndst', '<i4'),
                                             ('tiled', '<i4'), ('d', dst_t, (4,))])
            assert rec.dtype.itemsize == 192
            for i, (src, pi, co, ci, taps, nd, tiled, js) in enumerate(recs):
                rec[i]['p'], rec[i]['pidx'], rec[i]['co'], rec[i]['ci'], rec[i]['taps'] = src, pi, co, ci, taps
                rec[i]['ndst'], rec[i]['tiled'] = nd, tiled
                for k, j in enumerate(js):
                    rec[i]['d'][k] = (j.dst, j.ktot, j.mode, j.cin_pad, j.row_off, j.k_off, j.rows_lim, 0)
            st = (torch.from_numpy(rec.view(np.uint8).copy()).to(params[0].device), len(recs), max(r[2] * r[3] * r[4] for r in recs))
            if len(self._sgd_tables) >= 8:
                self._sgd_tables.pop(next(iter(self._sgd_tables)))
            self._sgd_tables[skey] = st
        check(self.L.dbx_sgd_pack_step_guarded(dt, ptr(st[0]), st[1], st[2], ptr(ptrs), lr, momentum, weight_decay, 1 if first else 0,
                                               ptr(guard), step_id, stream_ptr()))
        torch.autograd.graph.increment_version(live)
        self._wsig = (dt, True, tuple((p._version, p.data_ptr()) for p in params), lay)
        return True

    def _w_heads_folded(self, dt):
        heads = _HEADS[self.kind]
        names = []
        for s_, _ in heads:
            names += ['conv5_1_%s.weight' % s_, 'conv5_1_%s.bias' % s_, 'conv5_2_%s.weight' % s_, 'conv5_2_%s.bias' % s_]
        ps = [self._param(n) for n in names]
        ver = tuple((p._version, p.data_ptr()) for p in ps)
        ent = self.wcache.get(('folded', dt))
        if ent is not None and ent[0] == ver:
            return ent[1]
        dev = ps[0].device
        ktot = sum(k for _, k in heads)
        wf = torch.empty((ktot, 768, 1, 1), dtype=torch.float32, device=dev)
        bf = torch.zeros(64, dtype=torch.float32, device=dev)
        o = 0
        for i, (s_, k) in enumerate(heads):
            w1, b1, w2, b2 = ps[4 * i:4 * i + 4]
            check(self.L.dbx_fold_heads(ptr(w2.detach()), ptr(b2.detach()), ptr(w1.detach()), ptr(b1.detach()), k,
                                        C.c_void_p(wf.data_ptr() + o * 768 * 4), C.c_void_p(bf.data_ptr() + o * 4),
                                        stream_ptr()))
            o += k
        wp = self._pack(dt, 0, wf, 64, 768, 1, 1)
        wpa = self._pack(dt, 0, wf[:, :512].contiguous(), 64, 512, 1, 1)
        wpc = self._pack(dt, 0, wf[:, 512:].contiguous(), 64, 256, 1, 1)
        self.wcache[('folded', dt)] = (ver, (wp, bf, ktot, wpa, wpc))
        return wp, bf, ktot, wpa, wpc

    def _w_refine_folded(self):
        names = ['conv6_1_det.weight', 'conv6_1_det.bias', 'conv6_2_det.weight', 'conv6_2_det.bias', 'conv6_3_det.weight', 'conv6_3_det.bias']
        ps = [self._param(nm) for nm in names]
        ver = tuple((p._version, p.data_ptr()) for p in ps)
        ent = self.wcache.get(('refold',))
        if ent is not None and ent[0] == ver:
            return ent[1]
        dev = ps[0].device
        ci, cm = ps[0].shape[1], ps[0].shape[0]
        assert ci == 5 and cm <= 64 and tuple(ps[0].shape[2:]) == (3, 3) and tuple(ps[2].shape[2:]) == (5, 5)
        if ent is not None and ent[1][0].device == dev:
            wf, bf, vf = ent[1]
        else:
            wf = torch.empty((1, ci, 7, 7), dtype=torch.float32, device=dev)
            bf = torch.empty(1, dtype=torch.float32, device=dev)
            vf = torch.empty((cm, 5, 5), dtype=torch.float32, device=dev)
        check(self.L.dbx_fold_refine(*[ptr(p.detach().float().contiguous()) for p in ps], ci, cm, ptr(wf), ptr(bf), ptr(vf), stream_ptr()))
        self.wcache[('refold',)] = (ver, (wf, bf, vf))
        return wf, bf, vf

    @staticmethod
    def _view(P, name):
        return P.B['fusion'].view(512, 256) if name == 'c34' else P.B[name].view()

    def _frag(self, P, dt, stem, which):
        cin, cout = _CH[stem]
        if which == 'f':
            src, dst = _FWD_IO[stem]
            return self.conv_plan(dt, self._view(P, src), self._view(P, dst), 3, 3, 1, P.cin0 if cin == 3 else cin, max(64, cout),
                                  _lib.EPI_BIAS | _lib.EPI_RELU)[2]
        dz, dx = _BWD_IO.get(stem, (None, None))
        if dz not in P.B:
            return False
        gated = stem not in ('conv2_1_1', 'conv3_1_1', 'conv4_1_1')
        return self.conv_plan(dt, self._view(P, dz), self._view(P, dx), 3, 3, 1, cout, max(64, cin), _lib.EPI_GATE if gated else 0)[2]

    def _next_drop_seed(self):
        st = getattr(self, '_seed_state', None)
        if st is None or st[0] != torch.initial_seed():
            base = (torch.initial_seed() * 0x9E3779B97F4A7C15 + 0x5eed) & 0xffffffffffffffff
            st = [torch.initial_seed(), (base ^ (base >> 32)) & 0xffffffff]
            self._seed_state = st
        st[1] = (st[1] * 1664525 + 1013904223) & 0xffffffff
        x = (st[1] ^ (int(getattr(self, 'sample_offset', 0)) * 0x85EBCA6B)) & 0xffffffff
        return x

    def captured_refs(self):
        return (list(self.plans.values()), getattr(self, 'last_plan', None), dict(self.wcache), dict(self.bias_cache),
                dict(self._tables))

    def plan(self, n, h, w, dt, device, train):
        key = (n, h, w, dt, train, Plan.env_flags())
        p = self.plans.get(key)
        if p is None:
            p = Plan(self.kind, n, h, w, dt, device, train)
            self.plans = {key: p}
        return p

    def _timed(self, name, flops):
        return _NOT_TIMED if self.profile is None else _Timed(self.profile, name, flops)

    def _conv(self, dt, x, y, wpk, bias, kh, kw, cpad, cin_pad, cout_pad, epi, gate=None, dropmask=None, dm_ld=0,
              alg_ci=None, drop_seed=0):
        d = ConvDesc(dt, kh, kw, cpad, cin_pad, cout_pad, epi, drop_seed)
        with self._timed(lambda: self.conv_plan(dt, x, y, kh, kw, cpad, cin_pad, cout_pad, epi)[1],
                         2.0 * y.n * y.h * y.w * kh * kw * (alg_ci if alg_ci is not None else cin_pad) * y.c):
            check(self.L.dbx_conv_forward(C.byref(d), C.byref(x), ptr(wpk), ptr(bias), C.byref(y),
                                          C.byref(gate) if gate is not None else None,
                                          C.c_void_p(dropmask) if dropmask else None, dm_ld, stream_ptr()))

    def forward(self, X):
        net = self.net
        train = net.training and torch.is_grad_enabled()
        params = [p for _, p in net.named_parameters()]
        if train and any(p.requires_grad for p in params):
            from .autograd import NetFunction
            outs = NetFunction.apply(self, X, *params)
            names = self.output_names()
            return dict(zip(names, outs))
        return self.forward_raw(X, train=net.training)

    def output_names(self):
        return [s for s, _ in _HEADS[self.kind]] + ([] if self.kind == 'DenseBox' else ['refine'])

    def forward_raw(self, X, train):
        u8 = X.dtype == torch.uint8
        if u8:
            assert X.dim() == 4 and X.size(3) == 3, 'uint8 input must be [N,H,W,3] (HWC, RGB)'
            n, h, w, _ = X.shape
        else:
            assert X.dim() == 4 and X.size(1) == 3, 'input must be [N,3,H,W]'
            n, _, h, w = X.shape
        L, kind = self.L, self.kind
        dt = _lib.DTYPE_ID[self.net.resolved_dtype(train)]
        assert h >= 8 and w >= 8, 'input smaller than the /8 stride'
        if kind != 'DenseBox':
            assert h // 8 >= 7 and w // 8 >= 7, 'refine branch (3x3 + 5x5 un-padded convs) needs H/8, W/8 >= 7'
        dev = X.device
        P = self.plan(n, h, w, dt, dev, train)
        self.last_plan = P
        B = P.B
        s = stream_ptr()
        self._prepare_weights(dt, train, P)
        if u8:
            from .data import IMAGENET_MEAN, IMAGENET_STD
            Xc = X.detach().contiguous()
            check(L.dbx_u8hwc_to_framed(dt, ptr(Xc), C.byref(B['x0'].view()), (C.c_float * 3)(*IMAGENET_MEAN),
                                        (C.c_float * 3)(*IMAGENET_STD), s))
        else:
            Xf = X.detach().to(torch.float32).contiguous()
            check(L.dbx_nchw_to_framed(dt, ptr(Xf), 3, C.byref(B['x0'].view()), s))
        RELU = _lib.EPI_BIAS | _lib.EPI_RELU

        def hook(*names):
            if self.act_hook is not None:
                for nm in names:
                    self.act_hook(nm, P)
        hook('x0')

        def conv3(stem, src, dst, cin, cout, dst_view=None):
            cin_pad = P.cin0 if cin == 3 else cin
            wp, wfrag = self._fetch(P, (stem, 'f'))
            self._conv(dt, B[src].view(), dst_view if dst_view is not None else B[dst].view(), wp,
                       self._fetch(P, (stem, 'bias'))[0], 3, 3, 1, cin_pad, max(64, cout), RELU | wfrag, alg_ci=cin)

        PI = P.pool_idx

        def pool(xv, yv, key):
            if PI is not None:
                check(L.dbx_maxpool2x2_idx(dt, C.byref(xv), C.byref(yv), ptr(PI[key]), s))
            else:
                check(L.dbx_maxpool2x2(dt, C.byref(xv), C.byref(yv), s))

        def conv3_pool(stem, src, yv, pv, c, key, keep_full):
            if not P.pool_fused[stem]:
                if stem == 'conv1_2_1' and P.a12_alias:
                    raise RuntimeError('conv1_2 + pool1 not fusable on a plan without a full-resolution conv1_2 map')
                conv3(stem, src, None, c, c, dst_view=yv)
                pool(yv, pv, key)
                return
            d = ConvDesc(dt, 3, 3, 1, c, c, RELU, 0)
            xv = B[src].view()
            with self._timed(lambda: self.conv_plan(dt, xv, yv, 3, 3, 1, c, c, RELU)[1], 2.0 * yv.n * yv.h * yv.w * 9 * c * c):
                check(L.dbx_conv_forward_pool_idx(C.byref(d), C.byref(xv), ptr(self._fetch(P, (stem, 'f'))[0]), ptr(self._fetch(P, (stem, 'bias'))[0]),
                                                  C.byref(yv), C.byref(pv), 1 if keep_full else 0, ptr(PI[key]) if PI else None, s))

        conv3('conv1_1_1', 'x0', 'a11', 3, 64)
        hook('a11')
        conv3_pool('conv1_2_1', 'a11', B['a12'].view(), B['p1'].view(), 64, 'a12', train and PI is None)
        hook('p1')
        conv3('conv2_1_1', 'p1', 'a21', 64, 128)
        hook('a21')
        conv3_pool('conv2_2_1', 'a21', B['a22'].view(), B['p2'].view(), 128, 'a22', train and PI is None)
        hook('p2')
        conv3('conv3_1_1', 'p2', 'a31', 128, 256)
        hook('a31')
        conv3('conv3_2_1', 'a31', 'a32', 256, 256)
        hook('a32')
        c34 = B['fusion'].view(512, 256)
        conv3_pool('conv3_4_1', 'a32', c34, B['p3'].view(), 256, 'fusion', True)
        hook('c34', 'p3')
        conv3('conv4_1_1', 'p3', 'a41', 256, 512)
        hook('a41')
        conv3('conv4_2_1', 'a41', 'a42', 512, 512)
        hook('a42')
        conv3('conv4_3_1', 'a42', 'a43', 512, 512)
        hook('a43')
        conv3('conv4_4_1', 'a43', 'a44', 512, 512)
        hook('a44')
        lin_eval = not train and os.environ.get('DBX_EVAL_LINEAR', '1') != '0'
        if not lin_eval:
            check(L.dbx_upsample_bilinear(dt, C.byref(B['a44'].view()), C.byref(B['fusion'].view(0, 512)), s))
            hook('ups')

        heads = _HEADS[kind]
        nh = len(heads)
        outs = {}
        h4, w4 = P.h4, P.w4
        if not train:
            wp, bf, ktot, wpa, wpc = self._w_heads_folded(dt)
            big = torch.empty((n, ktot, h4, w4), dtype=torch.float32, device=dev)
            yv = View(C.c_void_p(big.data_ptr()), n, h4, w4, 0, ktot, 0, ktot)
            if lin_eval:
                h8, w8 = B['a44'].h, B['a44'].w
                ga = torch.empty((n, ktot, h8, w8), dtype=torch.float32, device=dev)
                gv = View(C.c_void_p(ga.data_ptr()), n, h8, w8, 0, ktot, 0, ktot)
                self._conv(dt, B['a44'].view(), gv, wpa, None, 1, 1, 0, 512, 64, _lib.EPI_F32_NCHW)
                check(L.dbx_upsample_bilinear_nchw_f32(ptr(ga), n * ktot, h8, w8, ptr(big), h4, w4, s))
                self._conv(dt, B['fusion'].view(512, 256), yv, wpc, bf, 1, 1, 0, 256, 64, _lib.EPI_BIAS | _lib.EPI_F32_NCHW | _lib.EPI_ACCUM)
            else:
                self._conv(dt, B['fusion'].view(), yv, wp, bf, 1, 1, 0, 768, 64, _lib.EPI_BIAS | _lib.EPI_F32_NCHW)
            o = 0
            for stem, k in heads:
                outs[stem] = big[:, o:o + k].contiguous()
                o += k
        else:
            epi = _lib.EPI_BIAS
            dm = None
            P.drop_active = bool(self._dropout_p() > 0.0)
            P.drop_hash = P.drop_active and self.net.dropout_masks is None
            if P.drop_hash:
                P.drop_seed = self._next_drop_seed()
                epi |= _lib.EPI_DROPHASH
            elif P.drop_active:
                dm = self._fill_dropout(P, heads)
                epi |= _lib.EPI_DROPMASK
            w1, w1frag = self._fetch(P, ('heads1', 'f'), plain=dm is not None)
            ktot = sum(k for _, k in heads)
            big = None
            b1, b2 = self._fetch(P, ('heads1', 'bias'))[0], self._fetch(P, ('heads2', 'bias'))[0]
            fused = P.manifest.get(('heads2', 'fused')) if P.drop_hash else None
            if fused is not None and fused.mode == 4 and not w1frag:
                fused = None
            if fused is not None:
                need = L.dbx_heads_forward_fused_scratch_bytes(nh, n * h4 * w4)
                if getattr(self, '_hf_scratch', None) is None or self._hf_scratch.numel() < need:
                    self._hf_scratch = torch.empty(int(need), dtype=torch.uint8, device=dev)
                w2f, w2frag = self._fetch(P, ('heads2', 'fused'))
                if not w2frag:
                    w1 = self._fetch(P, ('heads1', 'f'), plain=True)[0]
                d = ConvDesc(dt, 1, 1, 0, 768, 512 * nh, epi | w2frag, P.drop_seed)
                for stem, k in heads:
                    outs[stem] = torch.empty((n, k, h4, w4), dtype=torch.float32, device=dev)
                with self._timed(('conv3x3_ws_kernel<%s,1,1,2>' if w2frag else 'conv3x3_p8_kernel<%s,1,1>') % _TNAME[dt],
                                 2.0 * n * h4 * w4 * (768 * 512 * nh + 512 * ktot)):
                    check(L.dbx_heads_forward_fused_heads(C.byref(d), C.byref(B['fusion'].view()), ptr(w1), ptr(b1), C.byref(B['hid'].view()),
                                                          ptr(w2f), ptr(b2), (C.c_int32 * nh)(*[k for _, k in heads]), nh,
                                                          (C.c_void_p * nh)(*[outs[stem].data_ptr() for stem, _ in heads]), ptr(self._hf_scratch), s))
            else:
                self._conv(dt, B['fusion'].view(), B['hid'].view(), w1, b1, 1, 1, 0, 768, 512 * nh, epi | w1frag,
                           dropmask=dm, dm_ld=512 * nh, drop_seed=P.drop_seed if P.drop_hash else 0)
                big = torch.empty((n, ktot, h4, w4), dtype=torch.float32, device=dev)
                yv = View(C.c_void_p(big.data_ptr()), n, h4, w4, 0, ktot, 0, ktot)
                self._conv(dt, B['hid'].view(), yv, self._fetch(P, ('heads2', 'f'))[0], b2, 1, 1, 0,
                           512 * nh, 64, _lib.EPI_BIAS | _lib.EPI_F32_NCHW, alg_ci=512)
            o = 0
            for stem, k in heads:
                if big is not None:
                    outs[stem] = big[:, o:o + k].contiguous()
                o += k
        P.refine_fwd = None
        rf_convs = ('conv6_1_det', 'f') in P.manifest
        if kind != 'DenseBox' and not rf_convs:
            wf7, bf7, vf7 = self._w_refine_folded()
            lmk, det = outs['landmark'], outs['det']
            if not lmk.is_contiguous():
                lmk = lmk.contiguous()
            if not det.is_contiguous():
                det = det.contiguous()
            small = torch.empty((n, 1, h4 // 2 - 6, w4 // 2 - 6), dtype=torch.float32, device=dev)
            check(L.dbx_refine_eval(ptr(lmk), ptr(det), n, h4, w4, ptr(wf7), ptr(bf7), ptr(small), s))
            o = torch.empty((n, 1, h4, w4), dtype=torch.float32, device=dev)
            check(L.dbx_upsample_bilinear_nchw_f32(ptr(small), n, h4 // 2 - 6, w4 // 2 - 6, ptr(o), h4, w4, s))
            outs['refine'] = o
            if train:
                P.refine_fwd = (lmk, det, wf7, vf7)
        elif kind != 'DenseBox':
            rdt = P.rdt
            w61, w62, w63 = (self._fetch(P, (st, 'f'))[0] for st in ('conv6_1_det', 'conv6_2_det', 'conv6_3_det'))
            rin = B['rf_in'].view()
            check(L.dbx_nchw_to_framed_ch(rdt, ptr(outs['landmark']), 4, C.byref(rin), 0, s))
            check(L.dbx_nchw_to_framed_ch(rdt, ptr(outs['det']), 1, C.byref(rin), 4, s))
            check(L.dbx_maxpool2x2(rdt, C.byref(rin), C.byref(B['rf_p'].view()), s))
            self._conv(rdt, B['rf_p'].view(), B['rf_1'].view(), w61,
                       self._fetch(P, ('conv6_1_det', 'bias'))[0], 3, 3, 0, P.crf, 64, _lib.EPI_BIAS, alg_ci=5)
            self._conv(rdt, B['rf_1'].view(), B['rf_2'].view(), w62,
                       self._fetch(P, ('conv6_2_det', 'bias'))[0], 5, 5, 0, 64, 64, _lib.EPI_BIAS)
            check(L.dbx_upsample_bilinear(rdt, C.byref(B['rf_2'].view()), C.byref(B['rf_u'].view()), s))
            o = torch.empty((n, 1, h4, w4), dtype=torch.float32, device=dev)
            yv = View(C.c_void_p(o.data_ptr()), n, h4, w4, 0, 1, 0, 1)
            self._conv(rdt, B['rf_u'].view(), yv, w63,
                       self._fetch(P, ('conv6_3_det', 'bias'))[0], 1, 1, 0, 64, 64, _lib.EPI_BIAS | _lib.EPI_F32_NCHW)
            outs['refine'] = o
        return outs

    def _dropout_p(self):
        drops = [m for m in self.net.modules() if isinstance(m, torch.nn.Dropout)]
        p = drops[0].p if drops else 0.0
        if p not in (0.0, 0.5):
            raise RuntimeError('densebox_amd: the head Dropout supports p=0.5 (reference) or p=0, got %r' % p)
        return p

    def _fill_dropout(self, P, heads):
        nh = len(heads)
        inj = self.net.dropout_masks
        dev = P.ws.device
        m = torch.empty((P.n, P.h4, P.w4, nh, 512), dtype=torch.uint8, device=dev)
        for i, (stem, _) in enumerate(heads):
            m[:, :, :, i, :] = inj[stem].to(dev).permute(0, 2, 3, 1).to(torch.uint8)
        P.mask_buf = m
        return m.data_ptr()

    def read_activation(self, name, c_off=0, c=None):
        P = self.last_plan
        b = P.B[name]
        v = b.view(c_off, c)
        out = torch.empty((b.n, v.c, b.h, b.w), dtype=torch.float32, device=P.ws.device)
        check(self.L.dbx_framed_to_nchw_f32(P.dtype_id, C.byref(v), ptr(out), stream_ptr()))
        return out

    def _lin_bwd(self, dt):
        return (dt != _lib.F32 or os.environ.get('DBX_F32_LIN', '0') == '1') and os.environ.get('DBX_LIN_BWD', '1') != '0'

    def _d_hid(self, P):
        b = P.B.get('d_hid')
        if b is None:
            hb = P.B['hid']
            b = Buf('d_hid', hb.n, hb.h, hb.w, hb.c, 1, hb.dtype_id)
            P._d_hid_store = torch.zeros(2 * b.guard + _align(b.bytes) + 256, dtype=torch.uint8, device=P.ws.device)
            b.base = _align(P._d_hid_store.data_ptr() + b.guard)
            P.B['d_hid'] = b
        return b

    def _wgrad(self, dt, dz, x, kh, kw, cpad, co, ci, dw, db, accumulate=0, ci_total=None, ci_off=0, gen=None, pool=None):
        need = self.L.dbx_conv_wgrad_scratch_bytes(dt, C.byref(dz), C.byref(x), kh, kw)
        if getattr(self, '_wg_scratch', None) is None or self._wg_scratch.numel() < need:
            self._wg_scratch = torch.empty(int(need * 1.25) + 1024, dtype=torch.uint8, device=dw.device)

        def name():
            buf = C.create_string_buffer(64)
            check(self.L.dbx_conv_wgrad_plan(dt, C.byref(dz), C.byref(x), kh, kw, buf, 64, None))
            nm = buf.value.decode()
            if gen is not None:
                nm = nm.replace('>', ',gen>')
            if pool is not None:
                nm = nm.replace('>', ',pool+dz>' if pool[3] else ',pool>')
            return nm
        with self._timed(name, 2.0 * dz.n * dz.h * dz.w * kh * kw * ci * co):
            if pool is not None:
                dyv, nib, nch, write_dz = pool
                check(self.L.dbx_conv_wgrad_pool_dz(dt, C.byref(dyv), ptr(nib), nch, C.byref(dz), C.byref(x), kh, kw, cpad, co, ci, ptr(dw), ptr(db),
                                                    ptr(self._wg_scratch), accumulate, write_dz, stream_ptr()))
            elif gen is not None:
                dov, w2p, ks, nh, use_hash, seed = gen
                check(self.L.dbx_heads1_wgrad_gen(dt, C.byref(dov), C.byref(x), w2p, ks, nh, use_hash, seed, ci, ptr(dw), ci_total, ci_off, ptr(db),
                                                  ptr(self._wg_scratch), stream_ptr()))
            elif ci_total is None:
                check(self.L.dbx_conv_wgrad(dt, C.byref(dz), C.byref(x), kh, kw, cpad, co, ci, ptr(dw), ptr(db),
                                            ptr(self._wg_scratch), accumulate, stream_ptr()))
            else:
                check(self.L.dbx_conv_wgrad_slice(dt, C.byref(dz), C.byref(x), kh, kw, cpad, co, ci, ptr(dw), ci_total, ci_off, ptr(db),
                                                  ptr(self._wg_scratch), accumulate, stream_ptr()))

    def backward_raw(self, grad_outs):
        L, kind = self.L, self.kind
        P = self.last_plan
        assert P is not None and P.train, 'backward needs a preceding training-mode forward'
        B, dt, n = P.B, P.dtype_id, P.n
        M = self._manifest(P)
        s = stream_ptr()
        dev = P.ws.device
        heads = _HEADS[kind]
        nh = len(heads)
        h4, w4 = P.h4, P.w4
        G = {}

        sink = self.grad_sink

        def new_grad(name):
            p = self._param(name)
            g = sink.grad_view(name) if sink is not None else torch.empty_like(p, dtype=torch.float32)
            G[name] = g
            return g

        def gout(name, k):
            g = grad_outs.get(name)
            if g is None:
                return torch.zeros((n, k, h4, w4), dtype=torch.float32, device=dev)
            return g.to(torch.float32).contiguous()

        main = torch.cuda.current_stream()
        side = None
        multi = sink is not None and getattr(sink, 'world', 1) > 1
        if self.profile is None and not multi and os.environ.get('DBX_SIDE_STREAM', '0') == '1':
            if getattr(self, '_side', None) is None:
                self._side = torch.cuda.Stream(device=dev)
            side = self._side

        def on_side(fn):
            if side is None:
                return fn()
            ev = torch.cuda.Event()
            ev.record(main)
            side.wait_event(ev)
            with torch.cuda.stream(side):
                return fn()

        def conv_bwd(stem, dz, x, kh, kw, cpad, co, ci):
            dw, db = new_grad(stem + '.weight'), new_grad(stem + '.bias')
            pool = None
            if stem == 'conv1_2_1' and pool12:
                pool = (B['d_p1'].view(), P.pool_idx['a12'], 64, 1 if pool12 == 1 else 0)

            def run():
                self._wgrad(dt, dz, x, kh, kw, cpad, co, ci, dw, db, pool=pool)
                if sink is not None:
                    sink.ready([stem + '.weight', stem + '.bias'])
            on_side(run)

        def dgrad(stem, src, dst, kh, kw, cpad, rows_pad, cin_pad, gate=None, epi=0, dropmask=None):
            wp, wfrag = self._fetch(P, (stem, 'b'))
            e = epi | (_lib.EPI_GATE if gate is not None else 0) | wfrag
            self._conv(dt, src, dst, wp, None, kh, kw, cpad, cin_pad, rows_pad, e, gate=gate, dropmask=dropmask,
                       dm_ld=512 * nh)

        override = {}
        if kind != 'DenseBox' and P.refine_fwd is not None:
            lmk, det, wf7, vf7 = P.refine_fwd
            pn = ['conv6_1_det.weight', 'conv6_1_det.bias', 'conv6_2_det.weight', 'conv6_2_det.bias', 'conv6_3_det.weight', 'conv6_3_det.bias']
            ps = [self._param(nm).detach() for nm in pn]
            gs = [new_grad(nm) for nm in pn]

            def f32c(t):
                return None if t is None else t.to(torch.float32).contiguous()
            g_lm, g_det = f32c(grad_outs.get('landmark')), f32c(grad_outs.get('det'))
            o_lm = torch.empty((n, 4, h4, w4), dtype=torch.float32, device=dev)
            o_det = torch.empty((n, 1, h4, w4), dtype=torch.float32, device=dev)
            need = L.dbx_refine_backward_scratch_bytes(n, h4, w4)
            if getattr(self, '_rf_scratch', None) is None or self._rf_scratch.numel() < need:
                self._rf_scratch = torch.empty(int(need), dtype=torch.uint8, device=dev)
            d_rf = gout('refine', 1)
            check(L.dbx_refine_backward(ptr(d_rf), ptr(lmk), ptr(det), n, h4, w4, *[ptr(p) for p in ps], ps[0].shape[0], ptr(wf7), ptr(vf7),
                                        ptr(g_lm), ptr(g_det), ptr(o_lm), ptr(o_det), *[ptr(g_) for g_ in gs], ptr(self._rf_scratch), s))
            if sink is not None:
                sink.ready(pn)
            override = {'landmark': o_lm, 'det': o_det}
        elif kind != 'DenseBox' and ('conv6_1_det', 'b') not in M:
            raise RuntimeError('densebox_amd: backward of the refine branch without its forward state (no training-mode forward on this plan)')
        elif kind != 'DenseBox':
            d_rfo = B['d_rfo'].view()
            check(L.dbx_nchw_to_framed(dt, ptr(gout('refine', 1)), 1, C.byref(d_rfo), s))
            conv_bwd('conv6_3_det', d_rfo, B['rf_u'].view(), 1, 1, 0, 1, 64)
            dgrad('conv6_3_det', d_rfo, B['d_rf_u'].view(), 1, 1, 0, 64, P.crf)
            check(L.dbx_upsample_bilinear_bwd(dt, C.byref(B['d_rf_u'].view()), C.byref(B['d_rf_2'].view()), None, s))
            conv_bwd('conv6_2_det', B['d_rf_2'].view(), B['rf_1'].view(), 5, 5, 0, 64, 64)
            dgrad('conv6_2_det', B['d_rf_2'].view(), B['d_rf_1'].view(), 5, 5, 4, 64, 64)
            conv_bwd('conv6_1_det', B['d_rf_1'].view(), B['rf_p'].view(), 3, 3, 0, 64, 5)
            dgrad('conv6_1_det', B['d_rf_1'].view(), B['d_rf_p'].view(), 3, 3, 2, 64, 64)
            check(L.dbx_maxpool2x2_bwd(dt, C.byref(B['rf_in'].view()), C.byref(B['d_rf_p'].view()),
                                       C.byref(B['d_rf_in'].view()), 0, 0, s))

        slot = {}
        srcs = []
        for i, (stem, k) in enumerate(heads):
            slot[stem] = B['d_out'].view(P.crf * i, P.crf)
            src = override.get(stem)
            srcs.append(src if src is not None else gout(stem, k))
        if override or kind == 'DenseBox':
            check(L.dbx_nchw_to_framed_slots(dt, (C.c_void_p * nh)(*[t.data_ptr() for t in srcs]), (C.c_int32 * nh)(*[k for _, k in heads]), nh, P.crf,
                                             C.byref(B['d_out'].view()), s))
        else:
            for (stem, k), t in zip(heads, srcs):
                check(L.dbx_nchw_to_framed(dt, ptr(t), k, C.byref(slot[stem]), s))
        if kind != 'DenseBox' and not override:
            check(L.dbx_framed_add_ch(dt, C.byref(B['d_rf_in'].view()), 0, 4, C.byref(slot['landmark']), 0, s))
            check(L.dbx_framed_add_ch(dt, C.byref(B['d_rf_in'].view()), 4, 1, C.byref(slot['det']), 0, s))

        hv = B['hid'].view()
        need = L.dbx_head2_wgrad_scratch_bytes(nh, hv.n * hv.h)
        if getattr(self, '_h2_scratch', None) is None or self._h2_scratch.numel() < need:
            self._h2_scratch = torch.empty(int(need), dtype=torch.uint8, device=dev)
        dw2 = [new_grad('conv5_2_%s.weight' % st) for st, _ in heads]
        db2 = [new_grad('conv5_2_%s.bias' % st) for st, _ in heads]
        w2s = [self._param('conv5_2_%s.weight' % st).detach() for st, _ in heads]
        ks = (C.c_int32 * nh)(*[k for _, k in heads])
        h2_names = ['conv5_2_%s.weight' % st for st, _ in heads] + ['conv5_2_%s.bias' % st for st, _ in heads]
        mask_p = C.c_void_p(P.mask_buf.data_ptr()) if (P.drop_active and not P.drop_hash) else None
        hash_on, hash_seed = (1 if P.drop_hash else 0), (P.drop_seed if P.drop_hash else 0)
        lin = ('heads1', 'bwd_a') in M
        up_done = False
        gen = bool(getattr(P, 'heads_gen', False) and lin and side is None and mask_p is None)
        if gen and dt != _lib.F32:
            dhid_v = View(None, hv.n, hv.h, hv.w, 1, 512 * nh, 0, 512 * nh)
        else:
            dhid_v = self._d_hid(P).view()
        w2p = (C.c_void_p * nh)(*[w.data_ptr() for w in w2s])
        with self._timed(lambda: ('head2_backward_up_kernel<%s>' if up_done else 'head2_wgrad_kernel<%s>') % _TNAME[dt],
                         2.0 * hv.n * hv.h * hv.w * 512 * sum(k for _, k in heads) * (1 if side is not None else 2)):
            if side is not None:
                def run_h2():
                    check(L.dbx_head2_wgrad(dt, C.byref(B['d_out'].view()), C.byref(hv), ks, nh,
                                            (C.c_void_p * nh)(*[t.data_ptr() for t in dw2]), (C.c_void_p * nh)(*[t.data_ptr() for t in db2]),
                                            ptr(self._h2_scratch), stream_ptr()))
                    if sink is not None:
                        sink.ready(h2_names)
                on_side(run_h2)
                check(L.dbx_head2_dgrad(dt, C.byref(B['d_out'].view()), (C.c_void_p * nh)(*[w.data_ptr() for w in w2s]), ks, nh,
                                        C.byref(dhid_v), mask_p, 512 * nh, hash_on, hash_seed, s))
            elif lin:
                check(L.dbx_head2_backward_up(dt, C.byref(B['d_out'].view()), C.byref(hv), (C.c_void_p * nh)(*[w.data_ptr() for w in w2s]), ks, nh,
                                              C.byref(dhid_v), mask_p, 512 * nh, hash_on, hash_seed,
                                              (C.c_void_p * nh)(*[t.data_ptr() for t in dw2]), (C.c_void_p * nh)(*[t.data_ptr() for t in db2]),
                                              ptr(self._h2_scratch), C.byref(B['d_g44'].view()), s))
                up_done = True
                if gen and dt == _lib.F32:
                    bh = P.B['d_hid']
                    P.ws[bh.off:bh.off + bh.bytes].view(torch.float32).fill_(float('nan'))
            else:
                check(L.dbx_head2_backward(dt, C.byref(B['d_out'].view()), C.byref(hv), (C.c_void_p * nh)(*[w.data_ptr() for w in w2s]), ks, nh,
                                           C.byref(dhid_v), mask_p, 512 * nh, hash_on, hash_seed,
                                           (C.c_void_p * nh)(*[t.data_ptr() for t in dw2]), (C.c_void_p * nh)(*[t.data_ptr() for t in db2]),
                                           ptr(self._h2_scratch), s))
                if sink is not None:
                    sink.ready(h2_names)
        w1n = ['conv5_1_%s.weight' % st for st, _ in heads]
        b1n = ['conv5_1_%s.bias' % st for st, _ in heads]
        if sink is not None:
            dw1, db1 = sink.region(w1n).view(512 * nh, 768, 1, 1), sink.region(b1n)
        else:
            dw1 = torch.empty((512 * nh, 768, 1, 1), dtype=torch.float32, device=dev)
            db1 = torch.empty((512 * nh,), dtype=torch.float32, device=dev)
        c34 = B['fusion'].view(512, 256)
        if lin and not up_done:
            check(L.dbx_upsample_bilinear_bwd(dt, C.byref(dhid_v), C.byref(B['d_g44'].view()), None, s))

        def run_h1():
            if lin:
                self._wgrad(dt, B['d_g44'].view(), B['a44'].view(), 1, 1, 0, 512 * nh, 512, dw1, None, ci_total=768, ci_off=0)
                if gen:
                    self._wgrad(dt, dhid_v, c34, 1, 1, 0, 512 * nh, 256, dw1, db1, ci_total=768, ci_off=512,
                                gen=(B['d_out'].view(), w2p, ks, nh, hash_on, hash_seed))
                else:
                    self._wgrad(dt, dhid_v, c34, 1, 1, 0, 512 * nh, 256, dw1, db1, ci_total=768, ci_off=512)
            else:
                self._wgrad(dt, dhid_v, B['fusion'].view(), 1, 1, 0, 512 * nh, 768, dw1, db1)
            if sink is not None:
                sink.ready(w1n + b1n)
        on_side(run_h1)
        for i, (stem, _) in enumerate(heads):
            G['conv5_1_%s.weight' % stem] = dw1[512 * i:512 * (i + 1)]
            G['conv5_1_%s.bias' % stem] = db1[512 * i:512 * (i + 1)]
        if lin:
            wa, fa = self._fetch(P, ('heads1', 'bwd_a'))
            self._conv(dt, B['d_g44'].view(), B['d_a44'].view(), wa, None, 1, 1, 0, 512 * nh, 512, _lib.EPI_GATE | fa, gate=B['a44'].view())
            if gen:
                wc = self._fetch(P, ('heads1', 'bwd_c'))[0]
                with self._timed('heads1_dgrad_gen_kernel<%s>' % _TNAME[dt], 2.0 * hv.n * hv.h * hv.w * 512 * nh * (256 + 8)):
                    check(L.dbx_heads1_dgrad_gen(dt, C.byref(B['d_out'].view()), w2p, ks, nh, hash_on, hash_seed,
                                                 ptr(wc), C.byref(B['d_c34'].view()), C.byref(c34), s))
            else:
                plain = P.heads_gen and M[('heads1', 'bwd_c')].mode >= 4 and \
                    not self.conv_plan(dt, dhid_v, B['d_c34'].view(), 1, 1, 0, 512 * nh, 256, _lib.EPI_GATE)[2]
                wc, fc = self._fetch(P, ('heads1', 'bwd_c'), plain=plain)
                self._conv(dt, dhid_v, B['d_c34'].view(), wc, None, 1, 1, 0, 512 * nh, 256, _lib.EPI_GATE | fc, gate=c34)
        else:
            w1t, bfrag = self._fetch(P, ('heads1', 'bwd'))
            if dt != _lib.F32:
                d = ConvDesc(dt, 1, 1, 0, 512 * nh, 768, bfrag, 0)
                dv = B['d_ups'].view()
                both = View(dv.ptr, dv.n, dv.h, dv.w, dv.pad, 768, 0, 768)
                with self._timed((lambda: self.conv_plan(dt, dhid_v, both, 1, 1, 0, 512 * nh, 768, 0)[1]) if bfrag else
                                 'conv_igemm_dma_kernel<%s,256,256>' % _TNAME[dt], 2.0 * hv.n * hv.h * hv.w * 512 * nh * 768):
                    check(L.dbx_conv_forward_split(C.byref(d), C.byref(dhid_v), ptr(w1t), None, C.byref(B['d_ups'].view()), None,
                                                   C.byref(B['d_c34'].view()), C.byref(c34), 512, _lib.EPI_GATE, s))
            else:
                row_bytes = 512 * nh * _lib.ESIZE[dt]
                self._conv(dt, dhid_v, B['d_ups'].view(), w1t, None, 1, 1, 0, 512 * nh, 512, 0)
                self._conv(dt, dhid_v, B['d_c34'].view(), w1t[512 * row_bytes:], None, 1, 1, 0, 512 * nh, 256,
                           _lib.EPI_GATE, gate=c34)
            check(L.dbx_upsample_bilinear_bwd(dt, C.byref(B['d_ups'].view()), C.byref(B['d_a44'].view()),
                                              C.byref(B['a44'].view()), s))

        chain = [
            ('conv4_4_1', 'd_a44', 'a43', 512, 512, 'd_a43', 'a43'),
            ('conv4_3_1', 'd_a43', 'a42', 512, 512, 'd_a42', 'a42'),
            ('conv4_2_1', 'd_a42', 'a41', 512, 512, 'd_a41', 'a41'),
            ('conv4_1_1', 'd_a41', 'p3', 256, 512, 'd_p3', None),
            ('pool', 'fusion', 'd_p3', 'd_c34', 1),
            ('conv3_4_1', 'd_c34', 'a32', 256, 256, 'd_a32', 'a32'),
            ('conv3_2_1', 'd_a32', 'a31', 256, 256, 'd_a31', 'a31'),
            ('conv3_1_1', 'd_a31', 'p2', 128, 256, 'd_p2', None),
            ('pool', 'a22', 'd_p2', 'd_a22', 0),
            ('conv2_2_1', 'd_a22', 'a21', 128, 128, 'd_a21', 'a21'),
            ('conv2_1_1', 'd_a21', 'p1', 64, 128, 'd_p1', None),
            ('pool', 'a12', 'd_p1', 'd_a12', 0),
            ('conv1_2_1', 'd_a12', 'a11', 64, 64, 'd_a11', 'a11'),
            ('conv1_1_1', 'd_a11', 'x0', 3, 64, None, None),
        ]
        fused11 = False
        pool12 = 0
        if P.pool_idx is not None and os.environ.get('DBX_POOL_WGRAD', '1') != '0' and \
                L.dbx_conv_wgrad_pool_dz_ok(dt, C.byref(B['d_a12'].view()), C.byref(B['a11'].view()), 3, 3):
            pool12 = 2 if (os.environ.get('DBX_POOL_WGRAD') == '2' or side is not None) else 1
        for item in chain:
            if item[0] == 'conv1_1_1' and fused11:
                continue
            if item[0] == 'conv1_2_1':
                stem, dzn, xn, cin, cout, dxn, gaten = item
                d12 = ConvDesc(dt, 3, 3, 1, 64, 64, _lib.EPI_GATE, 0)
                dzv, gv, x0v = B[dzn].view(), B[gaten].view(), B['x0'].view()
                if side is None and os.environ.get('DBX_FUSE_WG1', '1') != '0' and L.dbx_conv_dgrad_wgrad1_fusable(C.byref(d12), C.byref(dzv), C.byref(gv), C.byref(x0v)):
                    conv_bwd(stem, dzv, B[xn].view(), 3, 3, 1, cout, cin)
                    need = L.dbx_conv_dgrad_wgrad1_scratch_bytes()
                    if getattr(self, '_wg1_scratch', None) is None or self._wg1_scratch.numel() < need:
                        self._wg1_scratch = torch.empty(int(need), dtype=torch.uint8, device=dev)
                    dw1, db1 = new_grad('conv1_1_1.weight'), new_grad('conv1_1_1.bias')
                    w12 = self._fetch(P, (stem, 'b'), plain=True)[0]
                    with self._timed(lambda: self.conv_plan(dt, dzv, B[dxn].view(), 3, 3, 1, 64, 64, _lib.EPI_GATE)[1],
                                     2.0 * dzv.n * dzv.h * dzv.w * 9 * 64 * (64 + 3)):
                        check(L.dbx_conv_dgrad_wgrad1(C.byref(d12), C.byref(dzv), ptr(w12), C.byref(gv), C.byref(x0v), 3, ptr(dw1), ptr(db1),
                                                      ptr(self._wg1_scratch), 0, s))
# ... 25 lines not shown
```

densebox_amd/loss.py:

```python
import ctypes as C

import numpy as np
import torch

from . import _lib, labels as LB
from ._lib import LossDesc, LossIO, check, ptr, stream_ptr

_KIND_ID = {'DenseBox': 0, 'DenseBoxLM': 1, 'DenseBoxLMLOC': 2}


class _LossFn(torch.autograd.Function):
    @staticmethod
    def forward(ctx, loss, n_out, *outs_and_grads):
        outs, grads = outs_and_grads[:n_out], outs_and_grads[n_out:]
        ctx.grads = grads
        return loss.clone()

    @staticmethod
    def backward(ctx, g):
        return (None, None) + tuple(d * g for d in ctx.grads) + (None,) * len(ctx.grads)


def densebox_loss(kind, outputs, bbox, vertices=None, labels=None, rand_neg_indices=None, lm_rand_neg_indices=None,
                  lambda_loc=3.0, lambda_det=1.0, lambda_lm=0.5, batch_global=None, positive_num_global=None,
                  return_debug=False, rng=None):
    kid = _KIND_ID[kind]
    if kind == 'DenseBox':
        score, loc = outputs
        lm = rf = lmloc = None
    elif kind == 'DenseBoxLM':
        score, loc, lm, rf = outputs
        lmloc = None
    else:
        score, rf, loc, lm, lmloc = outputs
    dev = score.device
    n = score.size(0)
    use_labels = kind == 'DenseBoxLMLOC'
    if kid != 0:
        LB.check_landmarks(vertices, labels if use_labels else None, clamp=use_labels)
    assert tuple(score.shape[1:]) == (1, 60, 60), 'the dense loss is defined on the 60x60 training grid'
    P = int(LB.positive_count(bbox, labels if use_labels else None).sum()) if positive_num_global is None \
        else int(positive_num_global)
    _, half = LB.neg_counts(P, n if batch_global is None else batch_global)
    rs = rng if rng is not None else np.random
    if rand_neg_indices is None:
        rand_neg_indices = np.stack([rs.choice(3600, half, replace=False) for _ in range(n)]) if half else \
            np.zeros((n, 0), np.int64)
    if kid != 0 and lm_rand_neg_indices is None:
        lm_rand_neg_indices = np.stack([np.stack([rs.choice(3600, 1, replace=False) for _ in range(n)])
                                        for _ in range(4)])
    rn = LB._dev(rand_neg_indices, dev, torch.int64).reshape(n, half)
    lrn = LB._dev(lm_rand_neg_indices, dev, torch.int64).reshape(4, n, 1) if kid != 0 else None
    bb = LB._dev(bbox, dev)
    vt = LB._dev(vertices, dev) if kid != 0 else None
    lb = LB._dev(labels, dev) if use_labels else None

    def c32(t):
        return None if t is None else t.detach().to(torch.float32).contiguous()
    o = [c32(t) for t in (score, loc, lm, rf, lmloc)]
    g = [None if t is None else torch.empty_like(t) for t in o]
    loss = torch.empty(1, dtype=torch.float32, device=dev)
    scratch = torch.empty((_lib.lib().dbx_loss_scratch_bytes(n) + 7) // 8, dtype=torch.float64, device=dev)
    dbg = {}
    if return_debug:
        dbg['mask_cls'] = torch.empty((n, 1, 60, 60), dtype=torch.float32, device=dev)
        dbg['neg_idx'] = torch.empty((n, 2 * half), dtype=torch.int64, device=dev)
        dbg['pos_count'] = torch.empty(n, dtype=torch.int32, device=dev)
        if kid != 0:
            dbg['mask_lm'] = torch.empty((n, 4, 60, 60), dtype=torch.float32, device=dev)
            dbg['lm_neg_idx'] = torch.empty((4, n, 2), dtype=torch.int64, device=dev)
    d = LossDesc(kid, n, half, lambda_loc, lambda_det, lambda_lm, 1 if use_labels else 0)
    io = LossIO()
    for name, t in (('bbox', bb), ('vertices', vt), ('labels', lb), ('rand_neg', rn), ('lm_rand_neg', lrn),
                    ('score', o[0]), ('loc', o[1]), ('lm', o[2]), ('rf', o[3]), ('lmloc', o[4]),
                    ('d_score', g[0]), ('d_loc', g[1]), ('d_lm', g[2]), ('d_rf', g[3]), ('d_lmloc', g[4]),
                    ('loss', loss), ('mask_cls', dbg.get('mask_cls')), ('mask_lm', dbg.get('mask_lm')),
                    ('neg_idx', dbg.get('neg_idx')), ('lm_neg_idx', dbg.get('lm_neg_idx')),
                    ('pos_count', dbg.get('pos_count'))):
        setattr(io, name, t.data_ptr() if t is not None else None)
    check(_lib.lib().dbx_loss_forward_backward(C.byref(d), C.byref(io), ptr(scratch), stream_ptr()))
    live = [(t, gg) for t, gg in zip((score, loc, lm, rf, lmloc), g) if t is not None]
    out = _LossFn.apply(loss[0], len(live), *[t for t, _ in live], *[gg for _, gg in live])
    out._dbx_direct = ([t for t, _ in live], [gg for _, gg in live])
    if return_debug:
        dbg['half'] = half
        dbg['grads'] = {k: gg for k, gg in zip(('score', 'loc', 'lm', 'rf', 'lmloc'), g) if gg is not None}
        return out, dbg
    return out
```

include/densebox_hip.h:

```cpp
#ifndef DENSEBOX_HIP_H
#define DENSEBOX_HIP_H

#include <stdint.h>

#ifdef __cplusplus
extern "C" {
#endif

enum dbx_status {
    DBX_OK = 0,
    DBX_ERR_ARG = -1,
    DBX_ERR_HIP = -2,
    DBX_ERR_DTYPE = -3
};

enum dbx_dtype { DBX_F16 = 0, DBX_BF16 = 1, DBX_F32 = 2 };

const char* dbx_last_error(void);
#define DBX_ABI_VERSION 13
int dbx_version(void);
int dbx_device_arch(int device);

typedef struct dbx_view {
    void*   ptr;
    int32_t n, h, w;
    int32_t pad;
    int32_t ld;
    int32_t c_off;
    int32_t c;
} dbx_view;

enum dbx_epilogue {
    DBX_EPI_BIAS     = 1,
    DBX_EPI_RELU     = 2,
    DBX_EPI_GATE     = 4,
    DBX_EPI_DROPMASK = 8,
    DBX_EPI_ACCUM    = 16,
    DBX_EPI_F32_NCHW = 32,
    DBX_EPI_DROPHASH = 64,
    DBX_CONV_WFRAG   = 128
};

typedef struct dbx_conv_desc {
    int32_t dtype;
    int32_t kh, kw;
    int32_t cpad;
    int32_t cin_pad;
    int32_t cout_pad;
    int32_t epilogue;
    uint32_t drop_seed;
} dbx_conv_desc;

int64_t dbx_conv_packed_elems(const dbx_conv_desc* d);
int dbx_conv_forward(const dbx_conv_desc* d, const dbx_view* x, const void* w_packed, const float* bias,
                     const dbx_view* y, const dbx_view* gate, const uint8_t* dropmask, int32_t dropmask_ld,
                     void* stream);
enum dbx_conv_kernel { DBX_K_IGEMM = 1, DBX_K_DMA = 2, DBX_K_BAND = 3, DBX_K_C64 = 4, DBX_K_C8 = 5, DBX_K_WS = 6, DBX_K_P8 = 7 };
typedef struct dbx_conv_plan_t {
    int32_t kernel;
    int32_t tile_m, tile_n;
    int32_t w_frag;
    char    name[64];
} dbx_conv_plan_t;
int dbx_conv_plan(const dbx_conv_desc* d, const dbx_view* x, const dbx_view* y, dbx_conv_plan_t* out);

int dbx_heads_forward_fusable(const dbx_conv_desc* d, const dbx_view* x, const dbx_view* hid, const int32_t* k, int32_t nh);
int64_t dbx_heads_forward_fused_scratch_bytes(int32_t nh, int64_t pixels);
int dbx_heads_forward_fused(const dbx_conv_desc* d, const dbx_view* x, const void* w1_frag, const float* bias1, const dbx_view* hid,
                            const void* w2_frag, const float* bias2, const int32_t* k, int32_t nh, float* out_nchw, void* scratch,
                            void* stream);
int dbx_heads_forward_fused_heads(const dbx_conv_desc* d, const dbx_view* x, const void* w1_frag, const float* bias1, const dbx_view* hid,
                                  const void* w2_frag, const float* bias2, const int32_t* k, int32_t nh, float* const* outs, void* scratch,
                                  void* stream);

int dbx_conv_forward_split(const dbx_conv_desc* d, const dbx_view* x, const void* w_packed, const float* bias,
                           const dbx_view* y, const dbx_view* gate, const dbx_view* y2, const dbx_view* gate2,
                           int32_t split_c, int32_t epilogue2, void* stream);

int dbx_conv_pool_fusable(const dbx_conv_desc* d, const dbx_view* x, const dbx_view* y);
int dbx_conv_forward_pool(const dbx_conv_desc* d, const dbx_view* x, const void* w_packed, const float* bias,
                          const dbx_view* y, const dbx_view* ypool, int32_t write_full, void* stream);
int dbx_conv_forward_pool_idx(const dbx_conv_desc* d, const dbx_view* x, const void* w_packed, const float* bias,
                              const dbx_view* y, const dbx_view* ypool, int32_t write_full, void* idx, void* stream);

int dbx_pack_weight(int32_t dtype, int32_t mode, const float* w_oihw, int32_t co, int32_t ci, int32_t kh, int32_t kw,
                    void* w_packed, int32_t rows_pad, int32_t cin_pad, int32_t row_off, int32_t k_off, void* stream);

int dbx_pack_multi(int32_t dtype, const void* jobs, int32_t count, int64_t max_elems, void* stream);

int dbx_sgd_pack_step(int32_t dtype, const void* jobs, int32_t count, int64_t max_elems, float* const* ptrs, float lr, float momentum,
                      float weight_decay, int32_t first_step, void* stream);

int dbx_head2_dgrad(int32_t dtype, const dbx_view* d_out, const float* const* w2, const int32_t* k, int32_t nh,
                    const dbx_view* d_hid, const uint8_t* dropmask, int32_t dropmask_ld, int32_t use_hash, uint32_t drop_seed,
                    void* stream);
int64_t dbx_head2_wgrad_scratch_bytes(int32_t nh, int32_t rows);
int dbx_head2_wgrad(int32_t dtype, const dbx_view* d_out, const dbx_view* hid, const int32_t* k, int32_t nh,
                    float* const* dw, float* const* db, void* scratch, void* stream);
int dbx_head2_backward(int32_t dtype, const dbx_view* d_out, const dbx_view* hid, const float* const* w2, const int32_t* k,
                       int32_t nh, const dbx_view* d_hid, const uint8_t* dropmask, int32_t dropmask_ld, int32_t use_hash,
                       uint32_t drop_seed, float* const* dw, float* const* db, void* scratch, void* stream);
int dbx_head2_backward_up(int32_t dtype, const dbx_view* d_out, const dbx_view* hid, const float* const* w2, const int32_t* k,
                          int32_t nh, const dbx_view* d_hid, const uint8_t* dropmask, int32_t dropmask_ld, int32_t use_hash,
                          uint32_t drop_seed, float* const* dw, float* const* db, void* scratch, const dbx_view* d_g44, void* stream);
int dbx_conv_wgrad_pool_dz_ok(int32_t dtype, const dbx_view* dz, const dbx_view* x, int32_t kh, int32_t kw);
int dbx_conv_wgrad_pool_dz(int32_t dtype, const dbx_view* dy, const void* idx, int32_t idx_channels, const dbx_view* dz, const dbx_view* x,
                           int32_t kh, int32_t kw, int32_t cpad, int32_t co, int32_t ci, float* dw_oihw, float* db, void* scratch,
                           int32_t accumulate, int32_t write_dz, void* stream);
int dbx_head2_backward_up_fused(int32_t dtype, const dbx_view* hid, const dbx_view* d_g44);
typedef struct dbx_head2_up_half { int32_t px_lo, px_n, own_lo, own_hi, ix_lo, ix_n; } dbx_head2_up_half;
typedef struct dbx_head2_up_launch { int32_t head0, heads, kj, groups, blocks; } dbx_head2_up_launch;
typedef struct dbx_head2_up_plan_t {
    int32_t fused, halves;
    dbx_head2_up_half half[2];
    int32_t launches;
    dbx_head2_up_launch launch[4];
} dbx_head2_up_plan_t;
int dbx_head2_backward_up_plan(int32_t dtype, const dbx_view* hid, const dbx_view* d_g44, const int32_t* k, int32_t nh,
                               dbx_head2_up_plan_t* out);
int dbx_heads1_wgrad_gen_ok(int32_t dtype, const dbx_view* x, int32_t nh);
int dbx_heads1_wgrad_gen(int32_t dtype, const dbx_view* d_out, const dbx_view* x, const float* const* w2, const int32_t* k, int32_t nh,
                         int32_t use_hash, uint32_t drop_seed, int32_t ci, float* dw_oihw, int32_t dw_ci_total, int32_t dw_ci_off,
                         float* db, void* scratch, void* stream);
int dbx_heads1_dgrad_gen(int32_t dtype, const dbx_view* d_out, const float* const* w2, const int32_t* k, int32_t nh, int32_t use_hash,
                         uint32_t drop_seed, const void* w1t_frag, const dbx_view* y, const dbx_view* gate, void* stream);

int dbx_fold_heads(const float* w2, const float* b2, const float* w1, const float* b1, int32_t k, float* w_out,
                   float* b_out, void* stream);
int dbx_fold_refine(const float* w1, const float* b1, const float* w2, const float* b2, const float* w3, const float* b3,
                    int32_t ci, int32_t cm, float* w_out, float* b_out, float* v_out, void* stream);
int dbx_refine_eval(const float* landmark_nchw, const float* score_nchw, int32_t n, int32_t h, int32_t w, const float* w_fold,
                    const float* b_fold, float* out_small, void* stream);
int dbx_upsample_bilinear_nchw_f32(const float* x, int32_t planes, int32_t hi, int32_t wi, float* y, int32_t ho, int32_t wo,
                                   void* stream);
int64_t dbx_refine_backward_scratch_bytes(int32_t n, int32_t h, int32_t w);
int dbx_refine_backward(const float* d_refine, const float* landmark, const float* score, int32_t n, int32_t h, int32_t w,
                        const float* w1, const float* b1, const float* w2, const float* b2, const float* w3, const float* b3,
                        int32_t cm, const float* w_fold, const float* v_fold, const float* g_landmark, const float* g_score, float* out_landmark,
                        float* out_score, float* dw1, float* db1, float* dw2, float* db2, float* dw3, float* db3, void* scratch,
                        void* stream);

int64_t dbx_conv_wgrad_scratch_bytes(int32_t dtype, const dbx_view* dz, const dbx_view* x, int32_t kh, int32_t kw);
int dbx_conv_wgrad(int32_t dtype, const dbx_view* dz, const dbx_view* x, int32_t kh, int32_t kw, int32_t cpad,
                   int32_t co, int32_t ci, float* dw_oihw, float* db, void* scratch, int32_t accumulate, void* stream);
int dbx_conv_wgrad_slice(int32_t dtype, const dbx_view* dz, const dbx_view* x, int32_t kh, int32_t kw, int32_t cpad,
                         int32_t co, int32_t ci, float* dw_oihw, int32_t dw_ci_total, int32_t dw_ci_off, float* db, void* scratch,
                         int32_t accumulate, void* stream);
int dbx_conv_wgrad_plan(int32_t dtype, const dbx_view* dz, const dbx_view* x, int32_t kh, int32_t kw, char* name, int32_t name_len,
                        int32_t* splits);

int64_t dbx_conv_dgrad_wgrad1_scratch_bytes(void);
int dbx_conv_dgrad_wgrad1_fusable(const dbx_conv_desc* d, const dbx_view* dz, const dbx_view* gate, const dbx_view* x0);
int dbx_conv_dgrad_wgrad1(const dbx_conv_desc* d, const dbx_view* dz, const void* w_packed, const dbx_view* gate, const dbx_view* x0,
                          int32_t ci, float* dw_oihw, float* db, void* scratch, int32_t accumulate, void* stream);

int dbx_nchw_to_framed(int32_t dtype, const float* x_nchw, int32_t c_src, const dbx_view* y, void* stream);
int dbx_u8hwc_to_framed(int32_t dtype, const uint8_t* x_nhwc, const dbx_view* y, const float* mean3, const float* std3,
                        void* stream);
int dbx_nchw_to_framed_ch(int32_t dtype, const float* x_nchw, int32_t c_src, const dbx_view* y, int32_t c_dst_off,
                          void* stream);
int dbx_nchw_to_framed_slots(int32_t dtype, const float* const* x_nchw, const int32_t* k, int32_t nslots, int32_t slot,
                             const dbx_view* y, void* stream);
int dbx_framed_to_nchw_f32(int32_t dtype, const dbx_view* x, float* y_nchw, void* stream);
int dbx_framed_add_ch(int32_t dtype, const dbx_view* src, int32_t c_src_off, int32_t n_ch, const dbx_view* dst,
                      int32_t c_dst_off, void* stream);
int dbx_maxpool2x2(int32_t dtype, const dbx_view* x, const dbx_view* y, void* stream);
int dbx_maxpool2x2_bwd(int32_t dtype, const dbx_view* x, const dbx_view* dy, const dbx_view* dx,
                       int32_t accumulate, int32_t relu_gate, void* stream);
int64_t dbx_maxpool_idx_bytes(int32_t n, int32_t h, int32_t w, int32_t c);
int dbx_maxpool2x2_idx(int32_t dtype, const dbx_view* x, const dbx_view* y, void* idx, void* stream);
int dbx_maxpool2x2_bwd_idx(int32_t dtype, const void* idx, const dbx_view* dy, const dbx_view* dx,
                           int32_t accumulate, int32_t relu_gate, void* stream);
int dbx_upsample_bilinear(int32_t dtype, const dbx_view* x, const dbx_view* y, void* stream);
int dbx_upsample_bilinear_bwd(int32_t dtype, const dbx_view* dy, const dbx_view* dx, const dbx_view* gate, void* stream);
typedef struct dbx_upsample_bwd_plan_t { int32_t kernel, nseg, workgroups, lds_bytes; } dbx_upsample_bwd_plan_t;
int dbx_upsample_bilinear_bwd_plan(int32_t dtype, const dbx_view* dy, const dbx_view* dx, dbx_upsample_bwd_plan_t* out);

typedef struct dbx_loss_desc {
    int32_t kind;
    int32_t n;
    int32_t half_neg;
    float   lambda_loc, lambda_det, lambda_lm;
    int32_t use_labels;
} dbx_loss_desc;

typedef struct dbx_loss_io {
    const float* bbox;
    const float* vertices;
    const float* labels;
    const int64_t* rand_neg;
    const int64_t* lm_rand_neg;
    const float* score;  const float* loc;  const float* lm;  const float* rf;  const float* lmloc;
    float* d_score; float* d_loc; float* d_lm; float* d_rf; float* d_lmloc;
    float* loss;
    float* mask_cls;
    float* mask_lm;
    int64_t* neg_idx;
    int64_t* lm_neg_idx;
    int32_t* pos_count;
} dbx_loss_io;

int64_t dbx_loss_scratch_bytes(int32_t n);
int dbx_loss_forward_backward(const dbx_loss_desc* d, const dbx_loss_io* io, void* scratch, void* stream);
int dbx_count_positives(const float* bbox, const float* labels, int32_t n, int32_t* count_per_sample, void* stream);

int dbx_init_score_map(const float* bbox, const float* labels, int32_t n, float* out, void* stream);
int dbx_init_offset_map(const float* coords, const float* labels, int32_t n, int32_t c, float* out, void* stream);
int dbx_init_lm_heatmap(const float* vertices, const float* labels, int32_t n, int32_t clamp, float* out, void* stream);
int dbx_mask_by_sel(float* mask, int32_t n, const int64_t* pos_idx, int64_t n_pos, const int64_t* neg_idx, int32_t n_neg, void* stream);
int dbx_mask_gray_zone_cls(float* mask, const float* bbox, const float* labels, int32_t n, void* stream);
int dbx_mask_gray_zone_lm(float* mask, int32_t n, const int64_t* pos_idx, int64_t n_pos, void* stream);

int dbx_sgd_step(float* const* ptrs, const int64_t* sizes, int32_t count, int64_t max_size,
                 float lr, float momentum, float weight_decay, int32_t first_step, void* stream);
int dbx_grad_guard(const float* grads, int64_t n, int32_t* guard, int32_t step_id, void* stream);
int dbx_sgd_step_guarded(float* const* ptrs, const int64_t* sizes, int32_t count, int64_t max_size, float lr, float momentum,
                         float weight_decay, int32_t first_step, int32_t* guard, int32_t step_id, void* stream);
int dbx_sgd_pack_step_guarded(int32_t dtype, const void* jobs, int32_t count, int64_t max_elems, float* const* ptrs, float lr, float momentum,
                              float weight_decay, int32_t first_step, int32_t* guard, int32_t step_id, void* stream);

int dbx_detect(const float* score, const float* loc, const float* lm_heat, const float* lm_loc,
               int32_t rows, int32_t cols, int32_t K, double nms_thresh,
               double* dets, int32_t det_cols, int64_t* topk_idx, int32_t* keep, void* scratch, void* stream);
int64_t dbx_detect_scratch_bytes(int32_t rows, int32_t cols, int32_t K);
int64_t dbx_detect_batch_scratch_bytes(int32_t batch, int32_t rows, int32_t cols, int32_t K);
int dbx_detect_batch(const float* score, const float* loc, const float* lm_heat, const float* lm_loc,
                     int32_t batch, int32_t rows, int32_t cols, int32_t K, double nms_thresh,
                     double* dets, int32_t det_cols, int64_t* topk_idx, int32_t* keep, void* scratch, void* stream);
int dbx_nms(const double* dets, int32_t n, int32_t det_cols, double nms_thresh, int32_t* keep, void* scratch, void* stream);

int64_t dbx_detect_thresh_batch_scratch_bytes(int32_t batch, int32_t rows, int32_t cols, int32_t max_dets);
int dbx_detect_thresh_batch(const float* score, const float* loc, const float* lm_heat, const float* lm_loc,
                            int32_t batch, int32_t rows, int32_t cols, float score_thresh, int32_t max_dets, double nms_thresh,
                            double* dets, int32_t det_cols, int64_t* topk_idx, int32_t* keep, int32_t* counts, void* scratch,
                            void* stream);
int64_t dbx_thresh_rows_batch_scratch_bytes(int32_t batch, int32_t rows, int32_t cols, int32_t max_dets);
int dbx_thresh_rows_batch(const float* score, const float* loc, const float* lm_heat, const float* lm_loc,
                          int32_t batch, int32_t rows, int32_t cols, float score_thresh, int32_t max_dets,
                          double* dets, int32_t det_cols, int64_t* topk_idx, int32_t* counts, void* scratch, void* stream);
int64_t dbx_nms_large_scratch_bytes(int32_t n);
int dbx_nms_large(const double* dets, int32_t n, int32_t det_cols, double nms_thresh, int32_t* keep, void* scratch, void* stream);

typedef struct dbx_merge_xform { double scale, off_x, off_y; } dbx_merge_xform;
int64_t dbx_merge_nms_batch_workspace_bytes(int32_t levels, int32_t batch, int32_t K);
int dbx_merge_nms_batch(const double* const* level_dets, const dbx_merge_xform* xform, int32_t levels, int32_t batch, int32_t K,
                        int32_t det_cols, double nms_thresh, double* out_dets, int32_t* out_keep, void* workspace, void* stream);

int64_t dbx_merge_nms_thresh_batch_workspace_bytes(int32_t levels, int32_t batch, int32_t max_dets);
int dbx_merge_nms_thresh_batch(const double* const* level_dets, const int32_t* const* level_counts, const dbx_merge_xform* xform,
                               int32_t levels, int32_t batch, int32_t max_dets, int32_t det_cols, double nms_thresh,
                               double* out_dets, int32_t* out_keep, int32_t* out_counts, void* workspace, void* stream);

int dbx_perspective_matrix(const float* src_xy, const float* dst_xy, double* m9);
int dbx_warp_perspective_u8(const uint8_t* src, int32_t sh, int32_t sw, int32_t c, const double* m9, uint8_t* dst,
                            int32_t dh, int32_t dw, void* stream);
typedef struct dbx_warp_job {
    const uint8_t* src;
    int32_t sh, sw;
    double m9[9];
    int32_t dh, dw;
    int32_t x0, y0, oh, ow;
    int64_t dst_off;
} dbx_warp_job;
int64_t dbx_warp_batch_workspace_bytes(int32_t njobs);
int dbx_warp_perspective_batch_u8(const dbx_warp_job* jobs, int32_t njobs, int32_t c, uint8_t* dst, void* workspace, void* stream);

typedef struct dbx_crop_frame {
    const uint8_t* src;
    int32_t sh, sw;
} dbx_crop_frame;
int dbx_plate_crops_batch(const dbx_crop_frame* frames, int32_t nframes, int32_t c, const double* quads, int64_t row_stride,
                          int64_t frame_stride, const int32_t* sel, int32_t slots, int32_t ow, int32_t oh, uint8_t* dst, int32_t* ok,
                          double* m9_out, void* stream);

typedef struct dbx_eval_record {
    double  score;
    double  lm_err;
    int32_t status;
    int32_t frame;
} dbx_eval_record;
int dbx_match_gt_batch(const double* dets, int32_t det_cols, int64_t det_rows, const int32_t* keep, const int32_t* prefix,
                       int32_t batch, int32_t slots, const double* gt, int32_t gt_cols, const int32_t* gt_counts,
                       const uint8_t* gt_ignore, int32_t max_gt, double iou_thresh, int32_t* status, int32_t* gt_index,
                       double* iou, double* lm_err, int32_t* tally, void* stream);
int dbx_eval_append(const double* dets, int32_t det_cols, int64_t det_rows, const int32_t* keep, const int32_t* prefix,
                    int32_t batch, int32_t slots, const int32_t* status, const double* lm_err, const int32_t* tally,
                    dbx_eval_record* records, int64_t capacity, int64_t* state, void* stream);

typedef struct dbx_track {
    double  box[4];
    double  vel[4];
    double  score;
    double  best_score;
    int32_t id;
    int32_t hits;
    int32_t age;
    int32_t first_frame;
    int32_t last_frame;
    int32_t best_frame;
} dbx_track;
typedef struct dbx_track_record {
    int32_t   stream;
    int32_t   reserved;
    dbx_track t;
} dbx_track_record;
int dbx_track_update_batch(const double* dets, int32_t det_cols, int64_t det_rows, const int32_t* keep, const int32_t* prefix,
                           int32_t batch, int32_t slots, int32_t* headers, dbx_track* tracks, int32_t streams, int32_t stream0,
                           int32_t max_tracks, double iou_thresh, int32_t max_age, double alpha, double beta, double birth_score,
                           int32_t* track_id, int32_t* track_slot, int32_t* track_hits, dbx_track* retired, int32_t* tally, void* stream);
int dbx_track_append(const dbx_track* retired, const int32_t* tally, int32_t batch, int32_t max_tracks, int32_t stream0,
                     dbx_track_record* records, int64_t capacity, int64_t* state, void* stream);

typedef struct dbx_shot {
    double  key;
    double  score;
    int64_t sharpness;
    int32_t id;
    int32_t frame;
    int32_t shots;
    int32_t reserved;
} dbx_shot;
typedef struct dbx_shot_record {
    int32_t  stream;
    int32_t  slot;
    dbx_shot shot;
} dbx_shot_record;
int dbx_crop_sharpness(const uint8_t* crops, int64_t n, int32_t oh, int32_t ow, int32_t c, int64_t* out, void* stream);
int dbx_track_gallery_update(const dbx_track* tracks, const int32_t* headers, const int32_t* track_slot, const uint8_t* crops,
                             const int32_t* ok, const dbx_track* retired, const int32_t* tally, const int64_t* append_state,
                             dbx_shot* shots, uint8_t* shot_crops, dbx_shot_record* arena, uint8_t* arena_crops, int64_t* gstate,
                             int32_t batch, int32_t slots, int32_t streams, int32_t stream0, int32_t max_tracks, int32_t oh, int32_t ow,
                             int32_t c, int64_t capacity, int32_t policy, double min_score, int32_t commit, void* stream);

typedef struct dbx_overlay_frame {
    const uint8_t* src;
    uint8_t* dst;
    int32_t h, w;
} dbx_overlay_frame;
typedef struct dbx_overlay_style {
    uint8_t box_color[4], text_color[4], mark_color[4];
    int32_t thickness;
    int32_t radius;
    int32_t font_scale;
    int32_t inset_scale;
} dbx_overlay_style;
int dbx_draw_overlay_batch(const dbx_overlay_frame* frames, int32_t batch, int32_t c, int32_t max_h, int32_t max_w,
                           const double* dets, int32_t det_cols, int64_t det_rows, const int32_t* keep, const int32_t* prefix,
                           int32_t slots, const int32_t* track_id, const uint8_t* crops, const int32_t* ok, int32_t ow, int32_t oh,
                           const dbx_overlay_style* style, void* stream);
int dbx_overlay_font(uint8_t* out);
int dbx_overlay_label(double score, int32_t track_id, char* out, int32_t out_len);

typedef struct dbx_redact_style {
    uint8_t color[4];
    int32_t method;
    int32_t shape;
// ... 187 lines not shown
```

Before: 7783 patches/s.

## Chain loss kernels, split mining per head, fuse refine upsample and slot packing

Splits hard-negative mining into per-sample, per-head blocks: one class head plus four landmark heads, giving 5x more blocks. It folds the loss reduction into the apply kernel using a last-block ticket, which removes the separate finish launch and the loss clone. It also adds a refine eval kernel that fuses maxpool, 7x7 conv and bilinear upsample. The refine backward now writes the framed gradient slots directly, skipping the separate nchw_to_framed_slots pass. The gain is fewer launches and passes, paid for with atomic and ticket coherence logic and more code paths.

```diff
diff --git a/densebox_amd/_lib.py b/densebox_amd/_lib.py
--- a/densebox_amd/_lib.py
+++ b/densebox_amd/_lib.py
@@ -216,6 +216,10 @@
     'dbx_refine_backward_scratch_bytes': (C.c_int64, [_I32, _I32, _I32]),
     'dbx_refine_backward': (C.c_int, [_VP, _VP, _VP, _I32, _I32, _I32, _VP, _VP, _VP, _VP, _VP, _VP, _I32, _VP, _VP, _VP, _VP, _VP, _VP, _VP, _VP, _VP, _VP, _VP, _VP, _VP, _VP]),
     'dbx_upsample_bilinear_nchw_f32': (C.c_int, [_VP, _I32, _I32, _I32, _VP, _I32, _I32, _VP]),
+    'dbx_refine_eval_up': (C.c_int, [_VP, _VP, _I32, _I32, _I32, _VP, _VP, _VP, _VP]),
+    'dbx_refine_backward_slots_scratch_bytes': (C.c_int64, [_I32, _I32, _I32]),
+    'dbx_refine_backward_slots': (C.c_int, [_VP, _VP, _VP, _I32, _I32, _I32, _VP, _VP, _VP, _VP, _VP, _VP, _I32, _VP, _VP, _VP, _VP, _VP, _VP, _VP, _VP, _VP, _VP,
+                                            _VP, _VP, _VP, _I32, _VP, _VP, _I32, _I32, _I32, _I32, _PV, _VP]),
     'dbx_pack_multi': (C.c_int, [_I32, _VP, _I32, _I64, _VP]),
     'dbx_sgd_pack_step': (C.c_int, [_I32, _VP, _I32, _I64, _VP, _F, _F, _F, _I32, _VP]),
     'dbx_head2_dgrad': (C.c_int, [_I32, _PV, C.POINTER(C.c_void_p), C.POINTER(C.c_int32), _I32, _PV, _VP, _I32, _I32, C.c_uint32, _VP]),
@@ -293,6 +297,8 @@
     'dbx_upsample_bilinear_bwd_plan': (C.c_int, [_I32, _PV, _PV, C.POINTER(UpsampleBwdPlan)]),
     'dbx_loss_scratch_bytes': (C.c_int64, [_I32]),
     'dbx_loss_forward_backward': (C.c_int, [C.POINTER(LossDesc), C.POINTER(LossIO), _VP, _VP]),
+    'dbx_loss_chain_scratch_bytes': (C.c_int64, [_I32]),
+    'dbx_loss_forward_backward_chain': (C.c_int, [C.POINTER(LossDesc), C.POINTER(LossIO), _VP, _VP]),
     'dbx_count_positives': (C.c_int, [_VP, _VP, _I32, _VP, _VP]),
     'dbx_init_score_map': (C.c_int, [_VP, _VP, _I32, _VP, _VP]),
     'dbx_init_offset_map': (C.c_int, [_VP, _VP, _I32, _I32, _VP, _VP]),
diff --git a/densebox_amd/csrc/aux_ops.hip b/densebox_amd/csrc/aux_ops.hip
--- a/densebox_amd/csrc/aux_ops.hip
+++ b/densebox_amd/csrc/aux_ops.hip
@@ -1847,6 +1847,72 @@
     return DBX_OK;
 }
 
+__global__ __launch_bounds__(256) void refine_eval_up_kernel(const float* __restrict__ lm, const float* __restrict__ sc, int h, int w,
+                                                             const float* __restrict__ wf, const float* __restrict__ bf, float* __restrict__ out,
+                                                             float sy, float sx) {
+    constexpr int TO = 32, ST = 18, PT = ST + 6, CI = 5;
+    __shared__ float tile[CI][PT][PT + 1];
+    __shared__ float small[ST][ST + 1];
+    __shared__ float wsm[CI * 49];
+    const int ph = h / 2, pw = w / 2, oh = ph - 6, ow = pw - 6;
+    const int n = blockIdx.z, Y0 = blockIdx.y * TO, X0 = blockIdx.x * TO, tid = threadIdx.x;
+    const int Y1 = Y0 + TO < h ? Y0 + TO : h, X1 = X0 + TO < w ? X0 + TO : w;
+    int sy0, sy1, sx0, sx1, t0, t1;
+    float f0, f1;
+    bilin_coef(Y0, sy, oh, sy0, t1, f0, f1);
+    bilin_coef(Y1 - 1, sy, oh, t0, sy1, f0, f1);
+    bilin_coef(X0, sx, ow, sx0, t1, f0, f1);
+    bilin_coef(X1 - 1, sx, ow, t0, sx1, f0, f1);
+    const int sh = sy1 - sy0 + 1, sw = sx1 - sx0 + 1;
+    for (int e = tid; e < CI * 49; e += 256) wsm[e] = wf[e];
+    for (int e = tid; e < CI * PT * PT; e += 256) {
+        const int c = e / (PT * PT), r = e % (PT * PT), ry = r / PT, rx = r % PT, py = sy0 + ry, px = sx0 + rx;
+        float v = 0.f;
+        if (ry < sh + 6 && rx < sw + 6 && py < ph && px < pw) {
+            const float* p = (c < 4 ? lm + ((size_t)n * 4 + c) * h * w : sc + (size_t)n * h * w) + (size_t)(2 * py) * w + 2 * px;
+            v = fmaxf(fmaxf(p[0], p[1]), fmaxf(p[w], p[w + 1]));
+        }
+        tile[c][ry][rx] = v;
+    }
+    __syncthreads();
+    for (int e = tid; e < sh * sw; e += 256) {
+        const int ty = e / sw, tx = e % sw;
+        float acc = bf[0];
+        for (int c = 0; c < CI; ++c)
+#pragma unroll
+            for (int u = 0; u < 7; ++u)
+#pragma unroll
+                for (int v = 0; v < 7; ++v) acc = fmaf(wsm[(c * 7 + u) * 7 + v], tile[c][ty + u][tx + v], acc);
+        small[ty][tx] = acc;
+    }
+    __syncthreads();
+    const int tw = X1 - X0;
+    for (int e = tid; e < (Y1 - Y0) * tw; e += 256) {
+        const int py = Y0 + e / tw, px = X0 + e % tw;
+        int y0, y1, x0, x1;
+        float ly0, ly1, lx0, lx1;
+        bilin_coef(py, sy, oh, y0, y1, ly0, ly1);
+        bilin_coef(px, sx, ow, x0, x1, lx0, lx1);
+        y0 -= sy0; y1 -= sy0; x0 -= sx0; x1 -= sx0;
+        {
+#pragma clang fp contract(off)
+            const float top = lx0 * small[y0][x0] + lx1 * small[y0][x1];
+            const float bot = lx0 * small[y1][x0] + lx1 * small[y1][x1];
+            out[((size_t)n * h + py) * w + px] = ly0 * top + ly1 * bot;
+        }
+    }
+}
+extern "C" int dbx_refine_eval_up(const float* landmark_nchw, const float* score_nchw, int32_t n, int32_t h, int32_t w, const float* w_fold,
+                                  const float* b_fold, float* out, void* stream) {
+    DBX_REQUIRE(landmark_nchw && score_nchw && w_fold && b_fold && out && n >= 1 && n <= 65535 && h / 2 >= 7 && w / 2 >= 7,
+                "refine_eval_up: bad arguments (H/2, W/2 >= 7)");
+    const int oh = h / 2 - 6, ow = w / 2 - 6;
+    hipLaunchKernelGGL(refine_eval_up_kernel, dim3((w + 31) / 32, (h + 31) / 32, n), dim3(256), 0, (hipStream_t)stream, landmark_nchw, score_nchw, h, w,
+                       w_fold, b_fold, out, ac_scale(oh, h), ac_scale(ow, w));
+    DBX_LAUNCH_CHECK();
+    return DBX_OK;
+}
+
 template <typename T>
 __global__ void u8hwc_to_framed_kernel(const unsigned char* __restrict__ x, FrameGeo y, float m0, float m1, float m2, float s0,
                                        float s1, float s2) {
diff --git a/densebox_amd/csrc/common.hpp b/densebox_amd/csrc/common.hpp
--- a/densebox_amd/csrc/common.hpp
+++ b/densebox_amd/csrc/common.hpp
@@ -173,6 +173,19 @@
     return pv - lr * bv;
 }
 
+__device__ __forceinline__ bool dbx_last_block_coherent(unsigned* ticket, unsigned total, int* flag) {
+    asm volatile("s_waitcnt vmcnt(0)" ::: "memory");
+    __syncthreads();
+    if (threadIdx.x == 0) {
+        const unsigned t = __hip_atomic_fetch_add(ticket, 1u, __ATOMIC_RELAXED, __HIP_MEMORY_SCOPE_AGENT);
+        const int last = t == total - 1u;
+        if (last) __hip_atomic_store(ticket, 0u, __ATOMIC_RELAXED, __HIP_MEMORY_SCOPE_AGENT);
+        *flag = last;
+    }
+    __syncthreads();
+    return *flag != 0;
+}
+
 #define DBX_DISPATCH_DTYPE(dtype, FN, ...)                          \
     switch (dtype) {                                                \
         case DBX_F16: return FN<_Float16>(__VA_ARGS__);             \
diff --git a/densebox_amd/csrc/loss.hip b/densebox_amd/csrc/loss.hip
--- a/densebox_amd/csrc/loss.hip
+++ b/densebox_amd/csrc/loss.hip
@@ -87,20 +87,10 @@
 #define LOSS_APPLY_THREADS 256
 #define LOSS_APPLY_BLOCKS ((NPIX + LOSS_APPLY_THREADS - 1) / LOSS_APPLY_THREADS)
 
-__global__ __launch_bounds__(LOSS_THREADS) void loss_kernel(const LossArgs a) {
-    __shared__ float negl[NPIX];
-    __shared__ unsigned char mask[NPIX];
-    __shared__ unsigned char lmask[4][NPIX];
-    __shared__ float red_v[LOSS_THREADS / 64];
-    __shared__ int red_i[LOSS_THREADS / 64];
-    __shared__ double red_d[LOSS_THREADS / 64];
-    const int n = blockIdx.x, tid = threadIdx.x;
-    const int kind = a.d.kind, N = a.d.n, K = a.d.half_neg;
+__device__ __forceinline__ void mine_cls(const LossArgs& a, int n, int valid, const Box& box, float* negl, unsigned char* mask,
+                                         float* red_v, int* red_i, double* red_d) {
+    const int tid = threadIdx.x, K = a.d.half_neg;
     const dbx_loss_io& io = a.io;
-    const float* bb = io.bbox + 4 * n;
-    const int valid = (a.d.use_labels && io.labels) ? (io.labels[n] != 0.f) : 1;
-    const Box box = make_box(bb, valid);
-
     const float* score = io.score + (size_t)n * NPIX;
     int npos = 0;
     for (int i = tid; i < NPIX; i += LOSS_THREADS) {
@@ -194,42 +184,58 @@
         }
         __syncthreads();
     }
-
-    int lmx[4] = {0, 0, 0, 0}, lmy[4] = {0, 0, 0, 0};
-    if (kind != 0) {
-        const float* vt = io.vertices + 8 * n;
-        const int clamp = a.d.use_labels;
-        for (int j = 0; j < 4; ++j) { lmx[j] = lm_coord(vt[2 * j], clamp); lmy[j] = lm_coord(vt[2 * j + 1], clamp); }
-        for (int j = 0; j < 4; ++j) {
-            const float* lm = io.lm + ((size_t)n * 4 + j) * NPIX;
-            const int pidx = lm_pixel(lmx[j], lmy[j]);
-            for (int i = tid; i < NPIX; i += LOSS_THREADS) {
-                const float gt = (valid && i == pidx) ? 1.f : 0.f;
-                const float d = lm[i] - gt;
-                negl[i] = d * d * (1.f - gt);
-                lmask[j][i] = gt != 0.f;
-            }
-            __syncthreads();
-            const int hard = block_argmax(negl, red_v, red_i);
-            if (tid == 0) {
-                const long long r = io.lm_rand_neg[((size_t)j * N + n)];
-                lmask[j][hard] = 1;
-                if (r >= 0 && r < NPIX) lmask[j][(int)r] = 1;
-                if (io.lm_neg_idx) { io.lm_neg_idx[((size_t)j * N + n) * 2] = hard; io.lm_neg_idx[((size_t)j * N + n) * 2 + 1] = r; }
-            }
-            __syncthreads();
-            if (valid && pidx >= 0) {
-                const Span sy = py_slice(lmy[j] - 2, lmy[j] + 3), sx = py_slice(lmx[j] - 2, lmx[j] + 3);
-                for (int i = tid; i < 25; i += LOSS_THREADS) {
-                    const int y = sy.a + i / 5, x = sx.a + i % 5;
-                    if (y < sy.b && x < sx.b) lmask[j][y * HWD + x] = 0;
-                }
-                __syncthreads();
-                if (tid == 0) lmask[j][pidx] = 1;
-                __syncthreads();
-            }
-        }
-    }
+}
+
+__device__ __forceinline__ void mine_lm(const LossArgs& a, int n, int j, int valid, float* negl, unsigned char* lmask, float* red_v, int* red_i) {
+    const int tid = threadIdx.x, N = a.d.n;
+    const dbx_loss_io& io = a.io;
+    const float* vt = io.vertices + 8 * n;
+    const int clamp = a.d.use_labels;
+    const int lmx = lm_coord(vt[2 * j], clamp), lmy = lm_coord(vt[2 * j + 1], clamp);
+    const float* lm = io.lm + ((size_t)n * 4 + j) * NPIX;
+    const int pidx = lm_pixel(lmx, lmy);
+    for (int i = tid; i < NPIX; i += LOSS_THREADS) {
+        const float gt = (valid && i == pidx) ? 1.f : 0.f;
+        const float d = lm[i] - gt;
+        negl[i] = d * d * (1.f - gt);
+        lmask[i] = gt != 0.f;
+    }
+    __syncthreads();
+    const int hard = block_argmax(negl, red_v, red_i);
+    if (tid == 0) {
+        const long long r = io.lm_rand_neg[((size_t)j * N + n)];
+        lmask[hard] = 1;
+        if (r >= 0 && r < NPIX) lmask[(int)r] = 1;
+        if (io.lm_neg_idx) { io.lm_neg_idx[((size_t)j * N + n) * 2] = hard; io.lm_neg_idx[((size_t)j * N + n) * 2 + 1] = r; }
+    }
+    __syncthreads();
+    if (valid && pidx >= 0) {
+        const Span sy = py_slice(lmy - 2, lmy + 3), sx = py_slice(lmx - 2, lmx + 3);
+        for (int i = tid; i < 25; i += LOSS_THREADS) {
+            const int y = sy.a + i / 5, x = sx.a + i % 5;
+            if (y < sy.b && x < sx.b) lmask[y * HWD + x] = 0;
+        }
+        __syncthreads();
+        if (tid == 0) lmask[pidx] = 1;
+        __syncthreads();
+    }
+}
+
+__global__ __launch_bounds__(LOSS_THREADS) void loss_kernel(const LossArgs a) {
+    __shared__ float negl[NPIX];
+    __shared__ unsigned char mask[NPIX];
+    __shared__ unsigned char lmask[4][NPIX];
+    __shared__ float red_v[LOSS_THREADS / 64];
+    __shared__ int red_i[LOSS_THREADS / 64];
+    __shared__ double red_d[LOSS_THREADS / 64];
+    const int n = blockIdx.x, tid = threadIdx.x;
+    const int kind = a.d.kind;
+    const dbx_loss_io& io = a.io;
+    const int valid = (a.d.use_labels && io.labels) ? (io.labels[n] != 0.f) : 1;
+    const Box box = make_box(io.bbox + 4 * n, valid);
+    mine_cls(a, n, valid, box, negl, mask, red_v, red_i, red_d);
+    if (kind != 0)
+        for (int j = 0; j < 4; ++j) mine_lm(a, n, j, valid, negl, lmask[j], red_v, red_i);
 
     unsigned char* mb = a.maskbuf + (size_t)n * 5 * NPIX;
     for (int i = tid; i < NPIX; i += LOSS_THREADS) {
@@ -241,7 +247,29 @@
     }
 }
 
-__global__ __launch_bounds__(LOSS_APPLY_THREADS) void loss_apply_kernel(const LossArgs a) {
+__global__ __launch_bounds__(LOSS_THREADS) void loss_mine_kernel(const LossArgs a, unsigned* ticket) {
+    __shared__ float negl[NPIX];
+    __shared__ unsigned char mask[NPIX];
+    __shared__ float red_v[LOSS_THREADS / 64];
+    __shared__ int red_i[LOSS_THREADS / 64];
+    __shared__ double red_d[LOSS_THREADS / 64];
+    const int task = blockIdx.x, n = blockIdx.y, tid = threadIdx.x;
+    const dbx_loss_io& io = a.io;
+    if (task == 0 && n == 0 && tid == 0) *ticket = 0u;
+    const int valid = (a.d.use_labels && io.labels) ? (io.labels[n] != 0.f) : 1;
+    if (task == 0) {
+        const Box box = make_box(io.bbox + 4 * n, valid);
+        mine_cls(a, n, valid, box, negl, mask, red_v, red_i, red_d);
+    } else {
+        mine_lm(a, n, task - 1, valid, negl, mask, red_v, red_i);
+    }
+    unsigned char* mb = a.maskbuf + ((size_t)n * 5 + task) * NPIX;
+    for (int i = tid; i < NPIX; i += LOSS_THREADS) mb[i] = mask[i];
+}
+
+template <bool COHERENT> __device__ __forceinline__ void loss_finish_sum(double* partial, int n, int per, float* loss, double* psum);
+template <bool FINISH>
+__global__ __launch_bounds__(LOSS_APPLY_THREADS) void loss_apply_kernel(const LossArgs a, unsigned* ticket) {
     __shared__ double red_d[LOSS_APPLY_THREADS / 64];
     const int n = blockIdx.y, tid = threadIdx.x, i = blockIdx.x * LOSS_APPLY_THREADS + tid;
     const int kind = a.d.kind;
@@ -314,17 +342,24 @@
     if (tid == 0) {
         double t = 0.0;
         for (int w = 0; w < LOSS_APPLY_THREADS / 64; ++w) t += red_d[w];
-        a.partial[(size_t)n * LOSS_APPLY_BLOCKS + blockIdx.x] = t;
-    }
-}
-
-__global__ __launch_bounds__(256) void loss_finish_kernel(const double* partial, int n, int per, float* loss) {
-    __shared__ double psum[256];
+        if constexpr (FINISH) __hip_atomic_store(&a.partial[(size_t)n * LOSS_APPLY_BLOCKS + blockIdx.x], t, __ATOMIC_RELAXED, __HIP_MEMORY_SCOPE_AGENT);
+        else a.partial[(size_t)n * LOSS_APPLY_BLOCKS + blockIdx.x] = t;
+    }
+    if constexpr (FINISH) {
+        __shared__ double psum[LOSS_APPLY_THREADS];
+        __shared__ int last;
+        if (dbx_last_block_coherent(ticket, gridDim.x * gridDim.y, &last)) loss_finish_sum<true>(a.partial, a.d.n, LOSS_APPLY_BLOCKS, io.loss, psum);
+    }
+}
+
+template <bool COHERENT> __device__ __forceinline__ void loss_finish_sum(double* partial, int n, int per, float* loss, double* psum) {
     double run = 0.0;
     for (int base = 0; base < n; base += 256) {
         const int p = base + threadIdx.x;
         double t = 0.0;
-        if (p < n) for (int i = 0; i < per; ++i) t += partial[(size_t)p * per + i];
+        if (p < n)
+            for (int i = 0; i < per; ++i)
+                t += COHERENT ? __hip_atomic_load(&partial[(size_t)p * per + i], __ATOMIC_RELAXED, __HIP_MEMORY_SCOPE_AGENT) : partial[(size_t)p * per + i];
         psum[threadIdx.x] = t;
         __syncthreads();
         if (threadIdx.x == 0) {
@@ -335,24 +370,49 @@
     }
     if (threadIdx.x == 0) loss[0] = (float)run;
 }
+__global__ __launch_bounds__(256) void loss_finish_kernel(const double* partial, int n, int per, float* loss) {
+    __shared__ double psum[256];
+    loss_finish_sum<false>((double*)partial, n, per, loss, psum);
+}
+static_assert(LOSS_APPLY_THREADS == 256, "loss_finish_sum walks the patches in groups of 256 = one per thread");
 
 extern "C" int64_t dbx_loss_scratch_bytes(int32_t n) {
     return (int64_t)n * LOSS_APPLY_BLOCKS * 8 + (int64_t)n * 5 * NPIX + 64;
 }
-extern "C" int dbx_loss_forward_backward(const dbx_loss_desc* d, const dbx_loss_io* io, void* scratch, void* stream) {
+static int loss_check(const dbx_loss_desc* d, const dbx_loss_io* io, void* scratch) {
     DBX_REQUIRE(d && io && scratch, "loss: null argument");
     DBX_REQUIRE(d->kind >= 0 && d->kind <= 2 && d->n > 0, "loss: bad kind/n");
     DBX_REQUIRE(d->half_neg >= 0 && d->half_neg <= NPIX, "loss: half_neg out of range");
     DBX_REQUIRE(io->bbox && io->score && io->loc && io->loss && (d->half_neg == 0 || io->rand_neg), "loss: missing tensors");
     if (d->kind != 0) DBX_REQUIRE(io->vertices && io->lm && io->rf && io->lm_rand_neg, "loss: landmark tensors missing");
     if (d->kind == 2) DBX_REQUIRE(io->lmloc != nullptr, "loss: lm_loc missing");
+    return DBX_OK;
+}
+extern "C" int dbx_loss_forward_backward(const dbx_loss_desc* d, const dbx_loss_io* io, void* scratch, void* stream) {
+    const int rc = loss_check(d, io, scratch);
+    if (rc != DBX_OK) return rc;
     LossArgs a; a.d = *d; a.io = *io; a.partial = (double*)scratch;
     a.maskbuf = (unsigned char*)scratch + (size_t)d->n * LOSS_APPLY_BLOCKS * sizeof(double);
     hipLaunchKernelGGL(loss_kernel, dim3(d->n), dim3(LOSS_THREADS), 0, (hipStream_t)stream, a);
     DBX_LAUNCH_CHECK();
-    hipLaunchKernelGGL(loss_apply_kernel, dim3(LOSS_APPLY_BLOCKS, d->n), dim3(LOSS_APPLY_THREADS), 0, (hipStream_t)stream, a);
+    hipLaunchKernelGGL(loss_apply_kernel<false>, dim3(LOSS_APPLY_BLOCKS, d->n), dim3(LOSS_APPLY_THREADS), 0, (hipStream_t)stream, a, (unsigned*)nullptr);
     DBX_LAUNCH_CHECK();
     hipLaunchKernelGGL(loss_finish_kernel, dim3(1), dim3(256), 0, (hipStream_t)stream, (const double*)scratch, d->n, LOSS_APPLY_BLOCKS, io->loss);
+    DBX_LAUNCH_CHECK();
+    return DBX_OK;
+}
+
+extern "C" int64_t dbx_loss_chain_scratch_bytes(int32_t n) { return dbx_loss_scratch_bytes(n) + 64; }
+extern "C" int dbx_loss_forward_backward_chain(const dbx_loss_desc* d, const dbx_loss_io* io, void* scratch, void* stream) {
+    const int rc = loss_check(d, io, scratch);
+    if (rc != DBX_OK) return rc;
+    LossArgs a; a.d = *d; a.io = *io; a.partial = (double*)scratch;
+    a.maskbuf = (unsigned char*)scratch + (size_t)d->n * LOSS_APPLY_BLOCKS * sizeof(double);
+    unsigned* ticket = (unsigned*)((char*)scratch + (dbx_loss_scratch_bytes(d->n) / 64) * 64);
+    DBX_REQUIRE(d->n <= 65535, "loss: at most 65535 patches per call");
+    hipLaunchKernelGGL(loss_mine_kernel, dim3(d->kind != 0 ? 5 : 1, d->n), dim3(LOSS_THREADS), 0, (hipStream_t)stream, a, ticket);
+    DBX_LAUNCH_CHECK();
+    hipLaunchKernelGGL(loss_apply_kernel<true>, dim3(LOSS_APPLY_BLOCKS, d->n), dim3(LOSS_APPLY_THREADS), 0, (hipStream_t)stream, a, ticket);
     DBX_LAUNCH_CHECK();
     return DBX_OK;
 }
diff --git a/densebox_amd/csrc/refine_ops.hip b/densebox_amd/csrc/refine_ops.hip
--- a/densebox_amd/csrc/refine_ops.hip
+++ b/densebox_amd/csrc/refine_ops.hip
@@ -14,35 +14,39 @@
 }
 inline float rf_scale(int in, int out) { return out > 1 ? (float)(in - 1) / (float)(out - 1) : 0.f; }
 
+__device__ __forceinline__ float refine_up_t_at(const float* __restrict__ dp, int ho, int wo, int py, int px, int hs, int ws, float sy, float sx) {
+    int ylo = sy > 0.f ? (int)((float)(py - 1) / sy) - 1 : 0, yhi = sy > 0.f ? (int)((float)(py + 1) / sy) + 2 : ho - 1;
+    int xlo = sx > 0.f ? (int)((float)(px - 1) / sx) - 1 : 0, xhi = sx > 0.f ? (int)((float)(px + 1) / sx) + 2 : wo - 1;
+    ylo = ylo < 0 ? 0 : ylo; xlo = xlo < 0 ? 0 : xlo; yhi = yhi > ho - 1 ? ho - 1 : yhi; xhi = xhi > wo - 1 ? wo - 1 : xhi;
+    float acc = 0.f;
+    for (int y = ylo; y <= yhi; ++y) {
+        int y0, y1; float ly0, ly1;
+        rf_coef(y, sy, hs, y0, y1, ly0, ly1);
+        const float wy = (y0 == py ? ly0 : 0.f) + (y1 == py ? ly1 : 0.f);
+        if (wy == 0.f) continue;
+        for (int x = xlo; x <= xhi; ++x) {
+            int x0, x1; float lx0, lx1;
+            rf_coef(x, sx, ws, x0, x1, lx0, lx1);
+            const float wx = (x0 == px ? lx0 : 0.f) + (x1 == px ? lx1 : 0.f);
+            if (wx != 0.f) acc = fmaf(wy * wx, dp[y * wo + x], acc);
+        }
+    }
+    return acc;
+}
 __global__ void refine_up_t_kernel(const float* __restrict__ d, int n, int ho, int wo, float* __restrict__ g, int hs, int ws, float sy, float sx) {
     const int64_t total = (int64_t)n * hs * ws;
     for (int64_t i = blockIdx.x * (int64_t)blockDim.x + threadIdx.x; i < total; i += (int64_t)gridDim.x * blockDim.x) {
         const int px = (int)(i % ws), py = (int)((i / ws) % hs);
         const int64_t im = i / ((int64_t)ws * hs);
-        int ylo = sy > 0.f ? (int)((float)(py - 1) / sy) - 1 : 0, yhi = sy > 0.f ? (int)((float)(py + 1) / sy) + 2 : ho - 1;
-        int xlo = sx > 0.f ? (int)((float)(px - 1) / sx) - 1 : 0, xhi = sx > 0.f ? (int)((float)(px + 1) / sx) + 2 : wo - 1;
-        ylo = ylo < 0 ? 0 : ylo; xlo = xlo < 0 ? 0 : xlo; yhi = yhi > ho - 1 ? ho - 1 : yhi; xhi = xhi > wo - 1 ? wo - 1 : xhi;
-        const float* dp = d + im * ho * wo;
-        float acc = 0.f;
-        for (int y = ylo; y <= yhi; ++y) {
-            int y0, y1; float ly0, ly1;
-            rf_coef(y, sy, hs, y0, y1, ly0, ly1);
-            const float wy = (y0 == py ? ly0 : 0.f) + (y1 == py ? ly1 : 0.f);
-            if (wy == 0.f) continue;
-            for (int x = xlo; x <= xhi; ++x) {
-                int x0, x1; float lx0, lx1;
-                rf_coef(x, sx, ws, x0, x1, lx0, lx1);
-                const float wx = (x0 == px ? lx0 : 0.f) + (x1 == px ? lx1 : 0.f);
-                if (wx != 0.f) acc = fmaf(wy * wx, dp[y * wo + x], acc);
-            }
-        }
-        g[i] = acc;
+        g[i] = refine_up_t_at(d + im * ho * wo, ho, wo, py, px, hs, ws, sy, sx);
     }
 }
 
 constexpr int RSPLIT = 4;
+template <bool UPT>
 __global__ __launch_bounds__(256) void refine_g1_kernel(const float* __restrict__ lm, const float* __restrict__ sc, int h, int w,
-                                                        const float* __restrict__ g, float* __restrict__ partial) {
+                                                        float* __restrict__ g, float* __restrict__ partial, const float* __restrict__ d,
+                                                        float sy, float sx) {
     extern __shared__ float sm[];
     const int ph = h / 2, pw = w / 2, oh = ph - 6, ow = pw - 6;
     const int n = blockIdx.x / RSPLIT, part = blockIdx.x % RSPLIT, tid = threadIdx.x;
@@ -55,7 +59,16 @@
         const float* p = (c < 4 ? lm + ((size_t)n * 4 + c) * h * w : sc + (size_t)n * h * w) + (size_t)(2 * py) * w + 2 * px;
         x5[e] = fmaxf(fmaxf(p[0], p[1]), fmaxf(p[w], p[w + 1]));
     }
-    for (int e = tid; e < (y1 - y0) * ow; e += 256) gs[e] = g[((size_t)n * oh + y0) * ow + e];
+    if constexpr (UPT) {
+        const float* dp = d + (size_t)n * h * w;
+        for (int e = tid; e < (y1 - y0) * ow; e += 256) {
+            const float v = refine_up_t_at(dp, h, w, y0 + e / ow, e % ow, oh, ow, sy, sx);
+            gs[e] = v;
+            g[((size_t)n * oh + y0) * ow + e] = v;
+        }
+    } else {
+        for (int e = tid; e < (y1 - y0) * ow; e += 256) gs[e] = g[((size_t)n * oh + y0) * ow + e];
+    }
     __syncthreads();
     if (tid < RG1) {
         float acc = 0.f;
@@ -72,17 +85,37 @@
 }
 
 struct RefineW { const float *w1, *b1, *w2, *b2, *w3, *b3, *V; float *dw1, *db1, *dw2, *db2, *dw3, *db3; };
-__global__ __launch_bounds__(256) void refine_wgrad_kernel(const float* __restrict__ partial, int nimg, int cm, RefineW a) {
-    __shared__ float G1[RG1], G2[64 * 25], V[64 * 25], w1s[64 * RCI * 9], red[256];
+struct RefineWLds { float G1[RG1], G2[64 * 25], V[64 * 25], w1s[64 * RCI * 9], red[256]; };
+template <int CHUNK>
+__device__ __forceinline__ void refine_wgrad_block(const float* __restrict__ partial, int nimg, int cm, int blk, const RefineW& a, RefineWLds& L,
+                                                   float* stage) {
+    float* G1 = L.G1; float* G2 = L.G2; float* V = L.V; float* w1s = L.w1s; float* red = L.red;
     const int tid = threadIdx.x;
     for (int e = tid; e < cm * RCI * 9; e += 256) w1s[e] = a.w1[e];
-    if (tid < RG1) {
+    if constexpr (CHUNK == 0) {
+        if (tid < RG1) {
+            float acc = 0.f;
+#pragma unroll 16
+            for (int n = 0; n < nimg; ++n) acc += partial[(size_t)n * RG1 + tid];
+            G1[tid] = acc;
+        }
+    } else {
+        static_assert((CHUNK * RG1) % 4 == 0, "a chunk of partial blocks is a whole number of 16-byte words");
         float acc = 0.f;
-#pragma unroll 16
-        for (int n = 0; n < nimg; ++n) acc += partial[(size_t)n * RG1 + tid];
-        G1[tid] = acc;
-    }
-    const int blk = blockIdx.x;
+        for (int n0 = 0; n0 < nimg; n0 += CHUNK) {
+            const int cnt = nimg - n0 < CHUNK ? nimg - n0 : CHUNK;
+            const float* src = partial + (size_t)n0 * RG1;
+            const int words = cnt * RG1, vec = words / 4;
+#pragma unroll 8
+            for (int e = tid; e < vec; e += 256) ((f32x4*)stage)[e] = ((const f32x4*)src)[e];
+            for (int e = vec * 4 + tid; e < words; e += 256) stage[e] = src[e];
+            __syncthreads();
+            if (tid < RG1)
+                for (int n = 0; n < cnt; ++n) acc += stage[n * RG1 + tid];
+            __syncthreads();
+        }
+        if (tid < RG1) G1[tid] = acc;
+    }
     if (blk == cm)
         for (int e = tid; e < cm * 25; e += 256) V[e] = a.V[e];
     __syncthreads();
@@ -127,6 +160,10 @@
         }
         if (tid == 0) a.db3[0] = Sg;
     }
+}
+__global__ __launch_bounds__(256) void refine_wgrad_kernel(const float* __restrict__ partial, int nimg, int cm, RefineW a) {
+    __shared__ RefineWLds L;
+    refine_wgrad_block<0>(partial, nimg, cm, blockIdx.x, a, L, nullptr);
 }
 
 __global__ void refine_dgrad_kernel(const float* __restrict__ lm, const float* __restrict__ sc, int n, int h, int w, const float* __restrict__ g,
@@ -171,6 +208,96 @@
         }
     }
 }
+
+constexpr int RW_CHUNK = 32;
+struct RefineSlots { const float* x[4]; int k[4]; int nslots, slot, lm_slot, det_slot; FrameGeo y; };
+template <typename T>
+__device__ __forceinline__ void refine_store_group(T* p, const float (&v)[16 / sizeof(T)]) {
+    u32x4 raw;
+    T* e = (T*)&raw;
+#pragma unroll
+    for (int i = 0; i < 16 / (int)sizeof(T); ++i) e[i] = from_f32<T>(v[i]);
+    *(u32x4*)p = raw;
+}
+template <typename T>
+__global__ __launch_bounds__(256) void refine_wgrad_dgrad_slots_kernel(const float* __restrict__ partial, int nimg, int cm, RefineW a,
+                                                                       const float* __restrict__ lm, const float* __restrict__ sc, int n, int h, int w,
+                                                                       const float* __restrict__ g, const float* __restrict__ wf,
+                                                                       const float* __restrict__ g_lm, const float* __restrict__ g_sc,
+                                                                       float* __restrict__ out_lm, float* __restrict__ out_sc, RefineSlots S) {
+    constexpr int V = 16 / (int)sizeof(T);
+    __shared__ RefineWLds L;
+    __shared__ __attribute__((aligned(16))) float stage[RW_CHUNK * RG1];
+    if ((int)blockIdx.x <= cm) {
+        refine_wgrad_block<RW_CHUNK>(partial, nimg, cm, blockIdx.x, a, L, stage);
+        return;
+    }
+    float* wsm = stage;
+    for (int e = threadIdx.x; e < RCI * RTAPS; e += 256) wsm[e] = wf[e];
+    __syncthreads();
+    const int ph = h / 2, pw = w / 2, oh = ph - 6, ow = pw - 6, wh = (h + 1) / 2, ww = (w + 1) / 2;
+    const int64_t total = (int64_t)n * wh * ww;
+    const int64_t i = ((int64_t)blockIdx.x - (cm + 1)) * 256 + threadIdx.x;
+    if (i >= total) return;
+    const int wx = (int)(i % ww), wy = (int)((i / ww) % wh), im = (int)(i / ((int64_t)ww * wh));
+    float dv[RCI] = {0.f, 0.f, 0.f, 0.f, 0.f};
+    int arg[RCI] = {-1, -1, -1, -1, -1};
+    if (wy < ph && wx < pw) {
+        const float* gp = g + (size_t)im * oh * ow;
+        for (int u = 0; u < 7; ++u) {
+            const int y = wy - u;
+            if (y < 0 || y >= oh) continue;
+            for (int v = 0; v < 7; ++v) {
+                const int x = wx - v;
+                if (x >= 0 && x < ow) {
+                    const float gv = gp[y * ow + x];
+#pragma unroll
+                    for (int c = 0; c < RCI; ++c) dv[c] = fmaf(wsm[(c * 7 + u) * 7 + v], gv, dv[c]);
+                }
+            }
+        }
+#pragma unroll
+        for (int c = 0; c < RCI; ++c) {
+            const float* p = (c < 4 ? lm + ((size_t)im * 4 + c) * h * w : sc + (size_t)im * h * w) + (size_t)(2 * wy) * w + 2 * wx;
+            float m = p[0]; int ar = 0;
+            if (p[1] > m) { m = p[1]; ar = 1; }
+            if (p[w] > m) { m = p[w]; ar = 2; }
+            if (p[w + 1] > m) { m = p[w + 1]; ar = 3; }
+            arg[c] = ar;
+        }
+    }
+#pragma unroll
+    for (int k = 0; k < 4; ++k) {
+        const int y = 2 * wy + (k >> 1), x = 2 * wx + (k & 1);
+        if (y >= h || x >= w) continue;
+        float val[RCI];
+#pragma unroll
+        for (int c = 0; c < RCI; ++c) {
+            const size_t plane = c < 4 ? ((size_t)im * 4 + c) * h * w : (size_t)im * h * w;
+            const float* gin = c < 4 ? (g_lm ? g_lm + plane : nullptr) : (g_sc ? g_sc + plane : nullptr);
+            const float in = gin ? gin[(size_t)y * w + x] : 0.f;
+            val[c] = in + (k == arg[c] ? dv[c] : 0.f);
+            ((c < 4 ? out_lm : out_sc) + plane)[(size_t)y * w + x] = val[c];
+        }
+        T* row = (T*)S.y.base + geo_pix(S.y, im, y, x);
+        const int gps = S.slot / V;
+        for (int si = 0; si < S.nslots; ++si) {
+            const float* xs = si == 0 ? S.x[0] : si == 1 ? S.x[1] : si == 2 ? S.x[2] : S.x[3];
+            const int ks = si == 0 ? S.k[0] : si == 1 ? S.k[1] : si == 2 ? S.k[2] : S.k[3];
+            for (int gi = 0; gi < gps; ++gi) {
+                float v[V];
+#pragma unroll
+                for (int j = 0; j < V; ++j) {
+                    const int c = gi * V + j;
+                    if (si == S.lm_slot) v[j] = (gi == 0 && j < 4) ? val[j < 4 ? j : 0] : 0.f;
+                    else if (si == S.det_slot) v[j] = (gi == 0 && j == 0) ? val[4] : 0.f;
+                    else v[j] = (xs && c < ks) ? xs[(((int64_t)im * ks + c) * h + y) * w + x] : 0.f;
+                }
+                refine_store_group<T>(row + si * S.slot + gi * V, v);
+            }
+        }
+    }
+}
 }
 
 extern "C" int64_t dbx_refine_backward_scratch_bytes(int32_t n, int32_t h, int32_t w) {
@@ -198,10 +325,10 @@
     DBX_LAUNCH_CHECK();
     static DbxDevOnce attr_once; int attr_dev = 0;
     if (attr_once.pending(&attr_dev)) {
-        DBX_HIP(hipFuncSetAttribute((const void*)refine_g1_kernel, hipFuncAttributeMaxDynamicSharedMemorySize, 150 * 1024));
+        DBX_HIP(hipFuncSetAttribute((const void*)refine_g1_kernel<false>, hipFuncAttributeMaxDynamicSharedMemorySize, 150 * 1024));
         attr_once.mark(attr_dev);
     }
-    hipLaunchKernelGGL(refine_g1_kernel, dim3(n * RSPLIT), dim3(256), lds, s, landmark, score, h, w, g, partial);
+    hipLaunchKernelGGL(refine_g1_kernel<false>, dim3(n * RSPLIT), dim3(256), lds, s, landmark, score, h, w, g, partial, (const float*)nullptr, 0.f, 0.f);
     DBX_LAUNCH_CHECK();
     RefineW a = {w1, b1, w2, b2, w3, b3, v_fold, dw1, db1, dw2, db2, dw3, db3};
     hipLaunchKernelGGL(refine_wgrad_kernel, dim3(cm + 1), dim3(256), 0, s, partial, n * RSPLIT, cm, a);
@@ -212,3 +339,60 @@
     DBX_LAUNCH_CHECK();
     return DBX_OK;
 }
+
+extern "C" int64_t dbx_refine_backward_slots_scratch_bytes(int32_t n, int32_t h, int32_t w) {
+    const int64_t oh = h / 2 - 6, ow = w / 2 - 6;
+    return (((int64_t)n * oh * ow + 3) / 4 * 4 + (int64_t)n * RSPLIT * RG1 + 64) * 4;
+}
+template <typename T>
+static int refine_backward_slots_t(const float* d_refine, const float* landmark, const float* score, int n, int h, int w, const RefineW& a, int cm,
+                                   const float* w_fold, const float* g_landmark, const float* g_score, float* out_landmark, float* out_score,
+                                   void* scratch, const float* const* xs, const int32_t* ks, int nslots, int slot, int lm_slot, int det_slot,
+                                   const dbx_view* y, hipStream_t s) {
+    constexpr int V = 16 / (int)sizeof(T);
+    DBX_REQUIRE(((size_t)y->ptr % 16) == 0 && (y->ld * sizeof(T)) % 16 == 0 && (y->c_off * sizeof(T)) % 16 == 0, "refine_backward_slots: view must be 16-byte aligned/strided");
+    DBX_REQUIRE(nslots >= 2 && nslots <= 4 && slot % V == 0 && y->c == nslots * slot && y->n == n && y->h == h && y->w == w,
+                "refine_backward_slots: 2..4 slots of a multiple of the vector width, view of nslots * slot channels on the heads' grid");
+    DBX_REQUIRE(lm_slot >= 0 && lm_slot < nslots && det_slot >= 0 && det_slot < nslots && lm_slot != det_slot && ks[lm_slot] == 4 && ks[det_slot] == 1,
+                "refine_backward_slots: the landmark slot holds 4 channels, the det slot 1");
+    RefineSlots S;
+    for (int i = 0; i < 4; ++i) {
+        S.x[i] = i < nslots ? xs[i] : nullptr; S.k[i] = i < nslots ? ks[i] : 0;
+        if (i < nslots) DBX_REQUIRE(ks[i] >= 0 && ks[i] <= slot, "refine_backward_slots: k must fit its slot");
+    }
+    S.nslots = nslots; S.slot = slot; S.lm_slot = lm_slot; S.det_slot = det_slot; S.y = make_geo<T>(y);
+    const int ph = h / 2, pw = w / 2, oh = ph - 6, ow = pw - 6;
+    const int rows = (oh + RSPLIT - 1) / RSPLIT;
+    const size_t lds = ((size_t)RCI * (rows + 6) * pw + (size_t)rows * ow) * 4;
+    float* g = (float*)scratch;
+    float* partial = g + ((size_t)n * oh * ow + 3) / 4 * 4;
+    DBX_REQUIRE(((size_t)scratch % 16) == 0, "refine_backward_slots: scratch must be 16-byte aligned");
+    static DbxDevOnce attr_once; int attr_dev = 0;
+    if (attr_once.pending(&attr_dev)) {
+        DBX_HIP(hipFuncSetAttribute((const void*)refine_g1_kernel<true>, hipFuncAttributeMaxDynamicSharedMemorySize, 150 * 1024));
+        attr_once.mark(attr_dev);
+    }
+    hipLaunchKernelGGL(refine_g1_kernel<true>, dim3(n * RSPLIT), dim3(256), lds, s, landmark, score, h, w, g, partial, d_refine, rf_scale(oh, h), rf_scale(ow, w));
+    DBX_LAUNCH_CHECK();
+    const int64_t tot_d = (int64_t)n * ((h + 1) / 2) * ((w + 1) / 2);
+    hipLaunchKernelGGL(refine_wgrad_dgrad_slots_kernel<T>, dim3((unsigned)(cm + 1 + (tot_d + 255) / 256)), dim3(256), 0, s, partial, n * RSPLIT, cm, a,
+                       landmark, score, n, h, w, g, w_fold, g_landmark, g_score, out_landmark, out_score, S);
+    DBX_LAUNCH_CHECK();
+    return DBX_OK;
+}
+extern "C" int dbx_refine_backward_slots(const float* d_refine, const float* landmark, const float* score, int32_t n, int32_t h, int32_t w,
+                                         const float* w1, const float* b1, const float* w2, const float* b2, const float* w3, const float* b3,
+                                         int32_t cm, const float* w_fold, const float* v_fold, const float* g_landmark, const float* g_score,
+                                         float* out_landmark, float* out_score, float* dw1, float* db1, float* dw2, float* db2, float* dw3, float* db3,
+                                         void* scratch, int32_t dtype, const float* const* x_nchw, const int32_t* k, int32_t nslots, int32_t slot,
+                                         int32_t lm_slot, int32_t det_slot, const dbx_view* y, void* stream) {
+    DBX_REQUIRE(d_refine && landmark && score && w1 && b1 && w2 && b2 && w3 && b3 && w_fold && v_fold && out_landmark && out_score && dw1 && db1 && dw2 &&
+                    db2 && dw3 && db3 && scratch && x_nchw && k && y, "refine_backward_slots: null argument");
+    DBX_REQUIRE(n >= 1 && h / 2 >= 7 && w / 2 >= 7 && cm >= 1 && cm <= 64, "refine_backward_slots: H/2, W/2 >= 7, mid channels <= 64");
+    const int rows = (h / 2 - 6 + RSPLIT - 1) / RSPLIT;
+    DBX_REQUIRE(((size_t)RCI * (rows + 6) * (w / 2) + (size_t)rows * (w / 2 - 6)) * 4 <= 150 * 1024,
+                "refine_backward_slots: map too large for the per-image LDS tile (%d x %d)", h, w);
+    const RefineW a = {w1, b1, w2, b2, w3, b3, v_fold, dw1, db1, dw2, db2, dw3, db3};
+    DBX_DISPATCH_DTYPE(dtype, refine_backward_slots_t, d_refine, landmark, score, n, h, w, a, cm, w_fold, g_landmark, g_score, out_landmark, out_score,
+                       scratch, x_nchw, k, nslots, slot, lm_slot, det_slot, y, (hipStream_t)stream);
+}
diff --git a/densebox_amd/engine.py b/densebox_amd/engine.py
--- a/densebox_amd/engine.py
+++ b/densebox_amd/engine.py
@@ -484,6 +484,11 @@
         self.wcache[('folded', dt)] = (ver, (wp, bf, ktot, wpa, wpc))
         return wp, bf, ktot, wpa, wpc
 
+    def _loss_chain(self, train):
+        from .loss import loss_chain_enabled
+        return bool(train and loss_chain_enabled() and self.net.dropout_masks is None and os.environ.get('DBX_SIDE_STREAM', '0') != '1'
+                    and os.environ.get('DBX_LIN_BWD', '1') != '0')
+
     def _w_refine_folded(self):
         names = ['conv6_1_det.weight', 'conv6_1_det.bias', 'conv6_2_det.weight', 'conv6_2_det.bias', 'conv6_3_det.weight', 'conv6_3_det.bias']
         ps = [self._param(nm) for nm in names]
@@ -727,16 +732,20 @@
         P.refine_fwd = None
         rf_convs = ('conv6_1_det', 'f') in P.manifest
         if kind != 'DenseBox' and not rf_convs:
+            chain = self._loss_chain(train)
             wf7, bf7, vf7 = self._w_refine_folded()
             lmk, det = outs['landmark'], outs['det']
             if not lmk.is_contiguous():
                 lmk = lmk.contiguous()
             if not det.is_contiguous():
                 det = det.contiguous()
-            small = torch.empty((n, 1, h4 // 2 - 6, w4 // 2 - 6), dtype=torch.float32, device=dev)
-            check(L.dbx_refine_eval(ptr(lmk), ptr(det), n, h4, w4, ptr(wf7), ptr(bf7), ptr(small), s))
             o = torch.empty((n, 1, h4, w4), dtype=torch.float32, device=dev)
-            check(L.dbx_upsample_bilinear_nchw_f32(ptr(small), n, h4 // 2 - 6, w4 // 2 - 6, ptr(o), h4, w4, s))
+            if chain:
+                check(L.dbx_refine_eval_up(ptr(lmk), ptr(det), n, h4, w4, ptr(wf7), ptr(bf7), ptr(o), s))
+            else:
+                small = torch.empty((n, 1, h4 // 2 - 6, w4 // 2 - 6), dtype=torch.float32, device=dev)
+                check(L.dbx_refine_eval(ptr(lmk), ptr(det), n, h4, w4, ptr(wf7), ptr(bf7), ptr(small), s))
+                check(L.dbx_upsample_bilinear_nchw_f32(ptr(small), n, h4 // 2 - 6, w4 // 2 - 6, ptr(o), h4, w4, s))
             outs['refine'] = o
             if train:
                 P.refine_fwd = (lmk, det, wf7, vf7)
@@ -890,6 +899,7 @@
                        dm_ld=512 * nh)
 
         override = {}
+        slots_done = False
         if kind != 'DenseBox' and P.refine_fwd is not None:
             lmk, det, wf7, vf7 = P.refine_fwd
             pn = ['conv6_1_det.weight', 'conv6_1_det.bias', 'conv6_2_det.weight', 'conv6_2_det.bias', 'conv6_3_det.weight', 'conv6_3_det.bias']
@@ -905,8 +915,21 @@
             if getattr(self, '_rf_scratch', None) is None or self._rf_scratch.numel() < need:
                 self._rf_scratch = torch.empty(int(need), dtype=torch.uint8, device=dev)
             d_rf = gout('refine', 1)
-            check(L.dbx_refine_backward(ptr(d_rf), ptr(lmk), ptr(det), n, h4, w4, *[ptr(p) for p in ps], ps[0].shape[0], ptr(wf7), ptr(vf7),
-                                        ptr(g_lm), ptr(g_det), ptr(o_lm), ptr(o_det), *[ptr(g_) for g_ in gs], ptr(self._rf_scratch), s))
+            slots_done = self._loss_chain(True)
+            if slots_done:
+                need = L.dbx_refine_backward_slots_scratch_bytes(n, h4, w4)
+                if self._rf_scratch.numel() < need:
+                    self._rf_scratch = torch.empty(int(need), dtype=torch.uint8, device=dev)
+                others = [None if stem in ('landmark', 'det') else gout(stem, k) for stem, k in heads]
+                stems = [stem for stem, _ in heads]
+                check(L.dbx_refine_backward_slots(ptr(d_rf), ptr(lmk), ptr(det), n, h4, w4, *[ptr(p) for p in ps], ps[0].shape[0], ptr(wf7), ptr(vf7),
+                                                  ptr(g_lm), ptr(g_det), ptr(o_lm), ptr(o_det), *[ptr(g_) for g_ in gs], ptr(self._rf_scratch), dt,
+                                                  (C.c_void_p * nh)(*[t.data_ptr() if t is not None else None for t in others]),
+                                                  (C.c_int32 * nh)(*[k for _, k in heads]), nh, P.crf, stems.index('landmark'), stems.index('det'),
+                                                  C.byref(B['d_out'].view()), s))
+            else:
+                check(L.dbx_refine_backward(ptr(d_rf), ptr(lmk), ptr(det), n, h4, w4, *[ptr(p) for p in ps], ps[0].shape[0], ptr(wf7), ptr(vf7),
+                                            ptr(g_lm), ptr(g_det), ptr(o_lm), ptr(o_det), *[ptr(g_) for g_ in gs], ptr(self._rf_scratch), s))
             if sink is not None:
                 sink.ready(pn)
             override = {'landmark': o_lm, 'det': o_det}
@@ -930,8 +953,11 @@
         for i, (stem, k) in enumerate(heads):
             slot[stem] = B['d_out'].view(P.crf * i, P.crf)
             src = override.get(stem)
-            srcs.append(src if src is not None else gout(stem, k))
-        if override or kind == 'DenseBox':
+            if not slots_done:
+                srcs.append(src if src is not None else gout(stem, k))
+        if slots_done:
+            pass
+        elif override or kind == 'DenseBox':
             check(L.dbx_nchw_to_framed_slots(dt, (C.c_void_p * nh)(*[t.data_ptr() for t in srcs]), (C.c_int32 * nh)(*[k for _, k in heads]), nh, P.crf,
                                              C.byref(B['d_out'].view()), s))
         else:
diff --git a/densebox_amd/loss.py b/densebox_amd/loss.py
--- a/densebox_amd/loss.py
+++ b/densebox_amd/loss.py
@@ -1,4 +1,5 @@
 import ctypes as C
+import os
 
 import numpy as np
 import torch
@@ -9,12 +10,21 @@
 _KIND_ID = {'DenseBox': 0, 'DenseBoxLM': 1, 'DenseBoxLMLOC': 2}
 
 
+def loss_chain_enabled():
+    return os.environ.get('DBX_LOSS_CHAIN', '1') != '0'
+
+
+class _Fresh:
+    def __init__(self, t):
+        self.t = t
+
+
 class _LossFn(torch.autograd.Function):
     @staticmethod
     def forward(ctx, loss, n_out, *outs_and_grads):
         outs, grads = outs_and_grads[:n_out], outs_and_grads[n_out:]
         ctx.grads = grads
-        return loss.clone()
+        return loss.t if isinstance(loss, _Fresh) else loss.clone()
 
     @staticmethod
     def backward(ctx, g):
@@ -23,7 +33,7 @@
 
 def densebox_loss(kind, outputs, bbox, vertices=None, labels=None, rand_neg_indices=None, lm_rand_neg_indices=None,
                   lambda_loc=3.0, lambda_det=1.0, lambda_lm=0.5, batch_global=None, positive_num_global=None,
-                  return_debug=False, rng=None):
+                  return_debug=False, rng=None, chain=None):
     kid = _KIND_ID[kind]
     if kind == 'DenseBox':
         score, loc = outputs
@@ -59,8 +69,12 @@
         return None if t is None else t.detach().to(torch.float32).contiguous()
     o = [c32(t) for t in (score, loc, lm, rf, lmloc)]
     g = [None if t is None else torch.empty_like(t) for t in o]
-    loss = torch.empty(1, dtype=torch.float32, device=dev)
-    scratch = torch.empty((_lib.lib().dbx_loss_scratch_bytes(n) + 7) // 8, dtype=torch.float64, device=dev)
+    if chain is None:
+        chain = loss_chain_enabled()
+    L = _lib.lib()
+    loss = torch.empty((), dtype=torch.float32, device=dev) if chain else torch.empty(1, dtype=torch.float32, device=dev)
+    need = L.dbx_loss_chain_scratch_bytes(n) if chain else L.dbx_loss_scratch_bytes(n)
+    scratch = torch.empty((need + 7) // 8, dtype=torch.float64, device=dev)
     dbg = {}
     if return_debug:
         dbg['mask_cls'] = torch.empty((n, 1, 60, 60), dtype=torch.float32, device=dev)
@@ -78,9 +92,9 @@
                     ('neg_idx', dbg.get('neg_idx')), ('lm_neg_idx', dbg.get('lm_neg_idx')),
                     ('pos_count', dbg.get('pos_count'))):
         setattr(io, name, t.data_ptr() if t is not None else None)
-    check(_lib.lib().dbx_loss_forward_backward(C.byref(d), C.byref(io), ptr(scratch), stream_ptr()))
+    check((L.dbx_loss_forward_backward_chain if chain else L.dbx_loss_forward_backward)(C.byref(d), C.byref(io), ptr(scratch), stream_ptr()))
     live = [(t, gg) for t, gg in zip((score, loc, lm, rf, lmloc), g) if t is not None]
-    out = _LossFn.apply(loss[0], len(live), *[t for t, _ in live], *[gg for _, gg in live])
+    out = _LossFn.apply(_Fresh(loss) if chain else loss[0], len(live), *[t for t, _ in live], *[gg for _, gg in live])
     out._dbx_direct = ([t for t, _ in live], [gg for _, gg in live])
     if return_debug:
         dbg['half'] = half
diff --git a/include/densebox_hip.h b/include/densebox_hip.h
--- a/include/densebox_hip.h
+++ b/include/densebox_hip.h
@@ -139,6 +139,15 @@
                         int32_t cm, const float* w_fold, const float* v_fold, const float* g_landmark, const float* g_score, float* out_landmark,
                         float* out_score, float* dw1, float* db1, float* dw2, float* db2, float* dw3, float* db3, void* scratch,
                         void* stream);
+int dbx_refine_eval_up(const float* landmark_nchw, const float* score_nchw, int32_t n, int32_t h, int32_t w, const float* w_fold,
+                       const float* b_fold, float* out, void* stream);
+int64_t dbx_refine_backward_slots_scratch_bytes(int32_t n, int32_t h, int32_t w);
+int dbx_refine_backward_slots(const float* d_refine, const float* landmark, const float* score, int32_t n, int32_t h, int32_t w,
+                              const float* w1, const float* b1, const float* w2, const float* b2, const float* w3, const float* b3,
+                              int32_t cm, const float* w_fold, const float* v_fold, const float* g_landmark, const float* g_score,
+                              float* out_landmark, float* out_score, float* dw1, float* db1, float* dw2, float* db2, float* dw3, float* db3,
+                              void* scratch, int32_t dtype, const float* const* x_nchw, const int32_t* k, int32_t nslots, int32_t slot,
+                              int32_t lm_slot, int32_t det_slot, const dbx_view* y, void* stream);
 
 int64_t dbx_conv_wgrad_scratch_bytes(int32_t dtype, const dbx_view* dz, const dbx_view* x, int32_t kh, int32_t kw);
 int dbx_conv_wgrad(int32_t dtype, const dbx_view* dz, const dbx_view* x, int32_t kh, int32_t kw, int32_t cpad,
@@ -202,6 +211,8 @@
 
 int64_t dbx_loss_scratch_bytes(int32_t n);
 int dbx_loss_forward_backward(const dbx_loss_desc* d, const dbx_loss_io* io, void* scratch, void* stream);
+int64_t dbx_loss_chain_scratch_bytes(int32_t n);
+int dbx_loss_forward_backward_chain(const dbx_loss_desc* d, const dbx_loss_io* io, void* scratch, void* stream);
 int dbx_count_positives(const float* bbox, const float* labels, int32_t n, int32_t* count_per_sample, void* stream);
 
 int dbx_init_score_map(const float* bbox, const float* labels, int32_t n, float* out, void* stream);
```

New measurement: 7830 patches/s (median of 6 runs). No clear change (+0.6%).
